# scipopt/SCIP-SDP

Measured on AMD Instinct MI355X. Metric: node-SDP solves/sec, dense block n x n with m vars (IPM iters/sec in iters_per_sec), higher is better.
Workload: dtype f64

## Files before the change

### include/hipsdp_units.h

```cpp
#ifndef HIPSDP_UNITS_H
#define HIPSDP_UNITS_H

#include "hipsdp.h"

#ifdef __cplusplus
extern "C" {
#endif

HIPSDP_API int  hipsdp_dgemm_selfcheck(int device, int M, int N, int K, int layB, int batch, int splitk, int flags, double beta,
   int* used_v2, long long* ndiff);
HIPSDP_API int  hipsdp_pass_at_unit(int device, int R, long long E, const double* A, const double* coef, double sa, const double* add, int split,
   double* out, int* chunks);
HIPSDP_API int  hipsdp_dgemm_selfcheck2(int device, int M, int N, int K, int layB, int batch, int splitk, int flags, double alpha, double beta,
   int reps, int* used, long long* ndiff, double* ms_tile, double* ms_fast);
HIPSDP_API int  hipsdp_gram_plan_info(int device, int M, long long K, int nslab, int* no, int* nd, int* nitems, double* span);
HIPSDP_API int  hipsdp_gram_selfcheck(int device, int M, long long K, int reps, int* used, double* maxdiff, long long* nrepro, double* ms_tile,
   double* ms_gram);
HIPSDP_API int  hipsdp_dgemm_selfcheck3(int device, int M, int N, int K, int layB, int batch, int splitk, int flags, double alpha, double beta,
   int reps, int* used, long long* ndiff, double* maxdiff, long long* nrepro, double* ms_tile, double* ms_fast);
HIPSDP_API int  hipsdp_tri_product_unit(int device, int mode, int M, int N, int K, int layB, int batch, int flags, const double* A,
   const double* B, double* Cio, int crows, int ldc, int* used);
HIPSDP_API int  hipsdp_tri_instance_force(int mode);
HIPSDP_API int  hipsdp_schur_identity_unit(int device, int m1, int n, const double* A, double ws_gbytes, int full_storage, double* Mx,
   double* flops);
HIPSDP_API int  hipsdp_schur_dense(int device, int m1, int n, const double* A, const double* X, const double* Zinv, double* Mx,
   double ws_gbytes);
HIPSDP_API int  hipsdp_schur_w(int device, int m1, int n, const double* A, const double* X, const double* Z, double* Mx);
HIPSDP_API int  hipsdp_schur_form_unit(int device, int form, int parts, int m1, int n, const double* A, const double* P, const double* Q,
   double ws_gbytes, double* Mx, int* used);
HIPSDP_API int  hipsdp_schur_small_unit(int device, int m1, int nblk, const int* ns, const double* const* A, const double* const* X,
   const double* const* Zinv, int q, const double* Dext, const double* x, const double* z, double* Mx, double* Lm, double* diagM, int* taken);
HIPSDP_API int  hipsdp_schur_shard_time(int device, int m1, int n, int nranks, int rank, int by_columns, int reps, double ws_gbytes, double* ms);
HIPSDP_API int  hipsdp_schur_var_share_time(int device, int m1, int n, int nranks, int rank, int cw, int reps, double* ms, double* a2a_bytes);
HIPSDP_API int  hipsdp_schur_sparse_unit(int device, int n, int m, long long nnz, const int* var, const int* row, const int* col,
   const double* val, const double* X, const double* Zinv, double* Mx);
HIPSDP_API int  hipsdp_schur_sparse_unit2(int device, int n, int m, long long nnz, const int* var, const int* row, const int* col,
   const double* val, const double* X, const double* Zinv, double* Mx, int kernel, int* took);
HIPSDP_API int  hipsdp_sparse_ops_unit(int device, int n, int m, long long nnz, const int* var, const int* row, const int* col,
   const double* val, const double* V, const double* coef, const double* base, double* outA, double* outAT);
HIPSDP_API int  hipsdp_mfma_peak(int device, double ms, double* tflops, double* ghz);
HIPSDP_API int  hipsdp_potrf(int device, int n, double* A, int* fail);
HIPSDP_API int  hipsdp_potrf_ex(int device, int n, double* A, int psd, int v1, double* dinv, int* regmask, int* fail);
HIPSDP_API int  hipsdp_potrs(int device, int n, const double* A, int nrhs, double* rhs);
HIPSDP_API int  hipsdp_potrs_seq(int device, int n, const double* A, int psd, int ncalls, const int* nrhs, const int* mode, double* rhs,
   int* regmask, int* fail);
HIPSDP_API int  hipsdp_potrf_small_unit(int device, int n, int pair, const double* base, const double* dir, double alpha, int set_flag,
   int want_gram, double* L, double* dinv, double* Mout, double* Linv, double* Gram, int* flag);
HIPSDP_API long long hipsdp_potrf_dinv_len(int n);
HIPSDP_API int  hipsdp_potrf_pair_unit(int device, int n, int pair, double* A, double* dinv, int* fail);
HIPSDP_API int  hipsdp_trial_pair_unit(int device, int n, int fused, int first, double alpha, double* io);
HIPSDP_API int  hipsdp_tail_after_solve2_unit(int device, int m, int fused, const double* rhs2, const double* u1, double* u2, double* wt,
   double* e2, double* e1);
HIPSDP_API int  hipsdp_tail_unpack3_unit(int device, int n, int fused, const double* pk, double* out);
HIPSDP_API int  hipsdp_tail_dz_unit(int device, int n, int fused, const double* pk, const double* P2, const double* Rd, double dtau, double eta,
   double* dZ);
HIPSDP_API int  hipsdp_tail_dirmat_unit(int device, int n, int fused, double s1, const double* Zinv, const double* X, const double* GZ, double* H,
   double* pk);
HIPSDP_API int  hipsdp_tail_sc_len(void);
HIPSDP_API int  hipsdp_tail_dir_unit(int device, int m, int n, int fused, const double* B, const double* H, const double* rhs2, const double* rp,
   const double* b, const double* u1, const double* u2, const double* par, double* sc, double* dy, double* dyt);
HIPSDP_API int  hipsdp_tail_dots_unit(int device, int m, int n, int fused, const double* a, const double* v, double* out);
HIPSDP_API int  hipsdp_trtri(int device, int n, const double* A, double* Linv);
HIPSDP_API int  hipsdp_lambda_min(int device, int n, const double* W, int steps, double* theta, double* resid);
HIPSDP_API int  hipsdp_lambda_min_scaled(int device, int n, const double* L, const double* D, int steps, double* theta, double* resid);
HIPSDP_API int  hipsdp_solve1_fits(int m, int q, int nblk, const int* ns);
HIPSDP_API int  hipsdp_solve1_class(int m, int nblk, const int* ns);
HIPSDP_API unsigned long long hipsdp_gram_gen_next(unsigned long long* counter);
HIPSDP_API int  hipsdp_gram_key_match_unit(int m_a, int nblk_a, const int* n_a, const int* form_a, const unsigned long long* gen_a,
   const long long* ws_a, int m_b, int nblk_b, const int* n_b, const int* form_b, const unsigned long long* gen_b, const long long* ws_b);
HIPSDP_API int  hipsdp_syev_many_unit(int device, int count, const int* ns, const double* A, double* lam, double* V, int* launches);
HIPSDP_API int  hipsdp_sparsecuts_unit(int device, int count, const int* ns, const double* Z, const double* v0, const double* maxeig,
   const int* sizes, const hipsdp_sparsecut_opts* opts, int* ncuts, double* eigvals, double* vecs, int* iters, int* flags);
HIPSDP_API int  hipsdp_sparsecuts_large_unit(int device, int n, const double* Z, const double* v0, double maxeig, int size,
   const hipsdp_sparsecut_opts* opts, int* ncuts, double* eigvals, double* vecs, int* iters, int* flags);
HIPSDP_API int  hipsdp_tridiag_unit(int device, int n, const double* A, double* d, double* e, double* Vrefl, double* tau);
HIPSDP_API int  hipsdp_tvec_unit(int device, int n, const double* d, const double* e, double* lam, double* Z);
HIPSDP_API int  hipsdp_sparse_dump_unit(hipsdp_solver* solver, int block, long long* counts, int* voff, int* vrow, int* vcol, double* vval,
   int* poff, int* prow, int* pcol, int* pvar, double* pval, int* foff, int* frow, int* fcol, double* fval, int* soff, int* srow, int* sent);
HIPSDP_API int  hipsdp_onevar_unit(int device, int n, int count, const double* Z, const double* A, const double* shift, const int* kind,
   const double* lb, const double* ub, double feastol, int maxevals, int* status, double* optval, double* lmin, double* grad, int* evals);
HIPSDP_API int  hipsdp_onevar_all_unit(int device, int count, const int* n, const double* Z, const double* A, const double* shift,
   const int* kind, const double* lb, const double* ub, double feastol, int maxevals, int mid_cap,
   int* status, double* optval, double* lmin, double* grad, int* evals);
HIPSDP_API int  hipsdp_onevar_large_unit(int device, int count, const int* n, const double* Z, const double* A, const double* shift,
   const int* kind, const double* lb, const double* ub, double feastol, int maxevals, int wg_cap, int chunk,
   int* status, double* optval, double* lmin, double* grad, int* evals, int* rounds);
HIPSDP_API int  hipsdp_objs_fanout_unit(int device, int count, int m, int q, int nblk, const int* ns, const double* B, const double* b_own,
   int have_start, const double* y, const double* x, const double* z, const double* XZ, int gap, double guard, long long* lane_len,
   long long* offs, double* lanes, int* launches);
HIPSDP_API int  hipsdp_small_dir_block_unit(int device, int n, double c, double s1, const double* X, const double* R, const double* E,
   const double* Zinv, int recorded, double* out, int* pending);
HIPSDP_API int  hipsdp_small_lp_rows_unit(int device, int q, int m1, const double* Dext, const double* v, int mode, double eta, double sigmu,
   const double* x, const double* z, const double* rd, const double* elp, int recorded, double* out1, double* out2, int* pending);
HIPSDP_API int  hipsdp_small_apply_A_unit(int device, int m1, int nblk, const int* n2, const double* A, const double* V, int q,
   const double* Dext, const double* vlp, int epi, double scal, const double* vin, int recorded, double* out, double* vout, int* pending);
HIPSDP_API int  hipsdp_small_elementwise_unit(int device, int n, const int* nn, const double* par, int use_elp, const double* in,
   const double* xs, int recorded, double* o_lp, double* o_mul, double* o_ext, double* ys, int* pending);
HIPSDP_API int  hipsdp_small_gemv_t_unit(int device, int R, long long E, long long lda, const double* A, const double* coef, double sa,
   int add_mode, const double* add, int recorded, double* out, int* pending);
HIPSDP_API int  hipsdp_reductions_unit(int device, int kind, int count, const int* len, const int* slot, const int* accumulate,
   const double* a, const double* b, const double* c, int nslots, const double* preset, int recorded, double* out, int* pending);
HIPSDP_API int  hipsdp_small_solve_unit(int device, int m, const double* M, int form, int nrhs, long long ld, double* rhs, double* u2,
   double* wt, int* pending, int* fail);
HIPSDP_API int  hipsdp_gemv_t3_unit(int device, int R, long long E, long long lda, const double* A, const double* c, int fused, double* out,
   int* took);
// ... 9 lines not shown
```

### scip-sdp_amd/binding.py

```python
import ctypes as C
import os
import numpy as np

_HERE = os.path.dirname(os.path.abspath(__file__))
LIBPATH = os.environ.get("HIPSDP_LIB", os.path.join(_HERE, "lib", "libhipsdp.so"))

STATUS_NAMES = {0: "optimal", 1: "dual_infeasible", 2: "dual_unbounded", 3: "both_infeasible", 4: "iterlimit",
                5: "numeric", 6: "timelimit", 7: "objlimit", -1: "unsolved"}


class Params(C.Structure):
    _fields_ = [("gaptol", C.c_double), ("feastol", C.c_double), ("infeastol", C.c_double), ("objlimit", C.c_double),
                ("timelimit", C.c_double), ("gamma", C.c_double), ("ws_gbytes", C.c_double), ("maxiter", C.c_int),
                ("verbose", C.c_int), ("lanczos_steps", C.c_int), ("settings", C.c_int), ("pabstol", C.c_double), ("preoptgap", C.c_double)]


class Info(C.Structure):
    _fields_ = [("status", C.c_int), ("iterations", C.c_int), ("pobj", C.c_double), ("dobj", C.c_double),
                ("pinf", C.c_double), ("dinf", C.c_double), ("dabs", C.c_double), ("gap", C.c_double), ("mu", C.c_double),
                ("tau", C.c_double), ("kappa", C.c_double), ("solve_seconds", C.c_double), ("schur_seconds", C.c_double),
                ("schur_flops", C.c_double), ("schur_calls", C.c_int), ("chol_fail", C.c_int), ("warm_started", C.c_int),
                ("settings_used", C.c_int), ("schur_flops_executed", C.c_double)]


# ... 866 lines not shown
    A = _f64(A)
    m1, n = A.shape[0], A.shape[1]
    P = _f64(P); Q = _f64(Q)
    assert A.shape == (m1, n, n) and P.shape == (n, n) and Q.shape == (n, n)
    Mx = np.zeros((m1, m1))
    used = (C.c_int * 3)(0, 0, 0)
    _chk(ulib().hipsdp_schur_form_unit(device, form, parts, m1, n, _dp(A), _dp(P), _dp(Q), C.c_double(ws_gbytes), _dp(Mx), used),
         "hipsdp_schur_form_unit")
    return Mx, tuple(used)


def schur_small_unit(As, Xs, Zinvs, Dext=None, x=None, z=None, fill=0.0, device=0):
    As = [_f64(a) for a in As]; Xs = [_f64(a) for a in Xs]; Zinvs = [_f64(a) for a in Zinvs]
    nblk, m1 = len(As), As[0].shape[0]
    ns = np.array([a.shape[1] for a in As], dtype=np.int32)
    for k in range(nblk):
        assert As[k].shape == (m1, ns[k], ns[k]) and Xs[k].shape == (ns[k], ns[k]) and Zinvs[k].shape == (ns[k], ns[k])
    q = 0 if Dext is None else int(np.shape(Dext)[0])
    if q > 0:
        Dext = _f64(Dext); x = _f64(x); z = _f64(z)
        assert Dext.shape == (q, m1) and x.shape == (q,) and z.shape == (q,)
    arr = C.POINTER(C.c_double) * nblk
    pA, pX, pZ = arr(*[_dp(a) for a in As]), arr(*[_dp(a) for a in Xs]), arr(*[_dp(a) for a in Zinvs])
    m = m1 - 1
    Mx = np.full((m1, m1), fill)
    Lm = np.full(max(m * m, 1), fill)
    dg = np.full(max(m, 1), fill)
    taken = C.c_int(-1)
    _chk(ulib().hipsdp_schur_small_unit(device, m1, nblk, _ip(ns), pA, pX, pZ, q, _dp(Dext) if q else None, _dp(x) if q else None,
                                        _dp(z) if q else None, _dp(Mx), _dp(Lm), _dp(dg), C.byref(taken)), "hipsdp_schur_small_unit")
    return taken.value, Mx, Lm[:m * m].reshape(m, m), dg[:m]


def gram_plan_info(M, K, nslab=64, device=0):
    no, nd, ni = C.c_int(0), C.c_int(0), C.c_int(0)
    sp = C.c_double(0.0)
    rc = ulib().hipsdp_gram_plan_info(device, M, C.c_longlong(K), nslab, C.byref(no), C.byref(nd), C.byref(ni), C.byref(sp))
    return (no.value, nd.value, ni.value, sp.value) if rc == 0 else None


def dgemm_selfcheck(M, N, K, layB=1, batch=1, splitk=1, flags=0, beta=0.0, device=0):
    used = C.c_int(0)
    nd = C.c_longlong(0)
    _chk(ulib().hipsdp_dgemm_selfcheck(device, M, N, K, layB, batch, splitk, flags, C.c_double(beta), C.byref(used), C.byref(nd)),
         "hipsdp_dgemm_selfcheck")
    return used.value, nd.value


def dgemm_selfcheck2(M, N, K, layB=1, batch=1, splitk=1, flags=0, alpha=1.0, beta=0.0, reps=0, device=0):
    used = C.c_int(0)
    nd = C.c_longlong(0)
    t0, t1 = C.c_double(0.0), C.c_double(0.0)
    _chk(ulib().hipsdp_dgemm_selfcheck2(device, M, N, K, layB, batch, splitk, flags, C.c_double(alpha), C.c_double(beta), reps,
                                       C.byref(used), C.byref(nd), C.byref(t0), C.byref(t1)), "hipsdp_dgemm_selfcheck2")
    return used.value, nd.value, t0.value, t1.value


def dgemm_selfcheck3(M, N, K, layB=1, batch=1, splitk=1, flags=0, alpha=1.0, beta=0.0, reps=0, device=0):
    used = C.c_int(0)
    nd, nr = C.c_longlong(0), C.c_longlong(0)
    md, t0, t1 = C.c_double(0.0), C.c_double(0.0), C.c_double(0.0)
    _chk(ulib().hipsdp_dgemm_selfcheck3(device, M, N, K, layB, batch, splitk, flags, C.c_double(alpha), C.c_double(beta), reps,
                                       C.byref(used), C.byref(nd), C.byref(md), C.byref(nr), C.byref(t0), C.byref(t1)), "hipsdp_dgemm_selfcheck3")
    return used.value, nd.value, md.value, nr.value, t0.value, t1.value


def tri_product_unit(A, B, flags, mode, layB=1, sentinel=None, pad_rows=0, pad_cols=0, device=0):
    A = _f64(A); B = _f64(B)
    M, K = A.shape
    batch = B.shape[0]
    N = B.shape[2] if layB == 1 else B.shape[1]
    assert B.shape == ((batch, K, N) if layB == 1 else (batch, N, K))
    Cio = np.full((batch, M + pad_rows, N + pad_cols), np.nan if sentinel is None else sentinel)
    used = (C.c_int * 2)(0, 0)
    _chk(ulib().hipsdp_tri_product_unit(device, mode, M, N, K, layB, batch, flags, _dp(A), _dp(B), _dp(Cio), M + pad_rows, N + pad_cols, used),
         "hipsdp_tri_product_unit")
    return Cio, tuple(used)


def tri_instance_force(mode):
    return ulib().hipsdp_tri_instance_force(mode)


def gram_selfcheck(M, K, reps=0, device=0):
    used = C.c_int(0)
    nr = C.c_longlong(0)
    md, t0, t1 = C.c_double(0.0), C.c_double(0.0), C.c_double(0.0)
    _chk(ulib().hipsdp_gram_selfcheck(device, M, C.c_longlong(K), reps, C.byref(used), C.byref(md), C.byref(nr), C.byref(t0), C.byref(t1)),
         "hipsdp_gram_selfcheck")
    return used.value, md.value, nr.value, t0.value, t1.value


def schur_identity_unit(A, Mx=None, ws_gbytes=0.0, full_storage=False, device=0):
    A = _f64(A)
    m1, n = A.shape[0], A.shape[1]
    Mx = np.zeros((m1, m1)) if Mx is None else _f64(Mx).copy()
    fl = C.c_double(0.0)
    _chk(ulib().hipsdp_schur_identity_unit(device, m1, n, _dp(A), C.c_double(ws_gbytes), int(full_storage), _dp(Mx), C.byref(fl)),
         "hipsdp_schur_identity_unit")
    return Mx, fl.value


def potrf(A, device=0):
    L = _f64(A).copy()
    fail = C.c_int(0)
    _chk(ulib().hipsdp_potrf(device, L.shape[0], _dp(L), C.byref(fail)), "hipsdp_potrf")
    return np.tril(L), fail.value


def potrf_ex(A, psd=False, v1=False, device=0):
    L = _f64(A).copy()
    n = L.shape[0]
    dinv = np.zeros(((n + 63) // 64) * 4096)
    mask = np.zeros(n, dtype=np.int32)
    fail = C.c_int(0)
    _chk(ulib().hipsdp_potrf_ex(device, n, _dp(L), int(psd), int(v1), _dp(dinv), _ip(mask), C.byref(fail)), "hipsdp_potrf_ex")
    return L, dinv, mask, fail.value


def potrs(A, rhs, device=0):
    A = _f64(A)
    r = _f64(rhs).copy()
    r2 = r.reshape(-1, A.shape[0])
    _chk(ulib().hipsdp_potrs(device, A.shape[0], _dp(A), r2.shape[0], _dp(r2)), "hipsdp_potrs")
    return r2.reshape(r.shape)


def potrs_seq(A, calls, psd=False, device=0):
    A = _f64(A)
    n = A.shape[0]
    nc = len(calls)
    slab = np.zeros((max(nc, 1), 4, n))
    nrhs = np.zeros(max(nc, 1), dtype=np.int32)
    mode = np.zeros(max(nc, 1), dtype=np.int32)
    for c, (md, r) in enumerate(calls):
        r = _f64(r).reshape(-1, n)
        nrhs[c], mode[c] = r.shape[0], md
        slab[c, :min(r.shape[0], 4)] = r[:4]
    mask = np.zeros(n, dtype=np.int32)
    fail = C.c_int(0)
    _chk(ulib().hipsdp_potrs_seq(device, n, _dp(A), int(psd), nc, _ip(nrhs), _ip(mode), _dp(slab), _ip(mask), C.byref(fail)),
         "hipsdp_potrs_seq")
    return [slab[c, :nrhs[c]].copy() for c in range(nc)], mask, fail.value


def potrf_small_unit(base, dir=None, alpha=0.0, pair=False, set_flag=False, want_gram=False, device=0):
    base = _f64(base)
    n = base.shape[-1]
    npb = 2 if pair else 1
    assert base.size == npb * n * n
    d = None if dir is None else _f64(dir)
    assert d is None or d.size == base.size
    shp = (2, n, n) if pair else (n, n)
    out = {"L": np.zeros(shp), "dinv": np.zeros((2, 64, 64) if pair else (64, 64)), "Mout": np.zeros(shp), "Linv": np.zeros(shp),
           "Gram": np.zeros(shp) if want_gram else None}
    flag = np.zeros(2, dtype=np.int32)
    _chk(ulib().hipsdp_potrf_small_unit(device, n, int(pair), _dp(base), None if d is None else _dp(d), C.c_double(alpha), int(set_flag),
                                        int(want_gram), _dp(out["L"]), _dp(out["dinv"]), _dp(out["Mout"]), _dp(out["Linv"]),
                                        None if not want_gram else _dp(out["Gram"]), _ip(flag)), "hipsdp_potrf_small_unit")
    out["flag"] = flag.copy() if pair else int(flag[0])
    return out


def potrf_pair_unit(A2, pair=True, device=0):
    L = _f64(A2).copy()
    n = L.shape[-1]
# ... 337 lines not shown
```

### scip-sdp_amd/csrc/hs_kernels.h

```cpp
#ifndef HS_KERNELS_H
#define HS_KERNELS_H

#include "hs_common.h"
#include "hs_cut_plan.h"
#include <vector>

int hs_fill(hipStream_t s, double* p, long long n, double v);
int hs_set_identity(hipStream_t s, double* A, int n, double v);
int hs_copy(hipStream_t s, double* dst, const double* src, long long n);
int hs_axpy(hipStream_t s, long long n, double a, const double* x, double* y);
int hs_scale_add(hipStream_t s, long long n, double a, const double* x, double b, const double* y, double* out);
struct hs_trial_job { double* V; const double* dV; double* Vs; double* L; };
int hs_trial_pair(hipStream_t s, long long n, double alpha, int first, const hs_trial_job* jobs);
int hs_mirror_lower(hipStream_t s, double* A, int n, long long lda);
int hs_symmetrize(hipStream_t s, double* A, int n);
int hs_transpose(hipStream_t s, int n, const double* src, double* dst);

int hs_gemv_n(hipStream_t s, int R, long long E, const double* A, long long lda, int nv, const double* const* V,
   double* out, long long ldo, double* ws, long long wsdoubles);
int hs_gemv_t(hipStream_t s, int R, long long E, const double* A, long long lda, const double* coef, double sa,
   const double* add, double* out);

int hs_gemv_t_chunks(int R, long long E);
int hs_gemv_t_ws(hipStream_t s, int R, long long E, const double* A, long long lda, const double* coef, double sa,
   const double* add, double* out, double* ws, long long wsdoubles);
int hs_gemv_t3(hipStream_t s, int R, long long E, const double* A, long long lda, const double* c0, const double* c1, const double* c2,
   double* o0, double* o1, double* o2);

void hs_red_batch_begin(hipStream_t s);
int hs_red_batch_end(void);
int hs_red_batch_end_publish(hipStream_t s, int n, const double* src, double* dst, unsigned long long seq, unsigned long long* flag);
void hs_red_batch_reset(void);
int hs_fill_scalar(hipStream_t s, double* p, double v);
int hs_red_batch_solve(hipStream_t s, int m, const double* dinv, const double* L, int nrhs, double* vec, long long ld);
struct hs_rb_finish { int m; double eta, rg, sigmu, tau, kappa, etk; const double* u1; const double* u2; double* dy; double* dyt; double* sc;
   int s0, bub, bh, wrp, bu1, dtau, dkappa, den; };
int hs_red_batch_finish(hipStream_t s, const void* fin, size_t bytes);
int hs_copy_scalar(hipStream_t s, double* dst, const double* src);
void hs_red_batch_hold(hipStream_t s);
int hs_red_batch_release(void);
int hs_red_batch_flush(void);
int hs_red_batch_pending(void);
int hs_red_batch_end_all(void);
int hs_make_ext(hipStream_t s, int m, double s0, double s1, const double* v, double* ext);
int hs_lp_rows_small(hipStream_t s, int q, int m1, const double* Dext, const double* v, int mode, double eta, double sigmu, const double* x,
   const double* z, const double* rd, const double* elp, double* out1, double* out2);
#define HS_AS_MAXBLK 8
struct hs_as_args { int nblk; int n2[HS_AS_MAXBLK]; const double* A[HS_AS_MAXBLK]; const double* V[HS_AS_MAXBLK]; };
int hs_apply_A_small(hipStream_t s, int m1, const hs_as_args* B, int q, const double* Dext, const double* vlp, double* out, int epi,
   double scal, const double* vin, double* vout);
int hs_axpy3(hipStream_t s, double a, long long n1, const double* x1, double* y1, long long n2, const double* x2, double* y2,
   long long n3, const double* x3, double* y3);
int hs_dot(hipStream_t s, long long n, const double* a, const double* b, double* out, int accumulate, double* ws);
#define HS_DOT_SLOT_DOUBLES 256
#define HS_DOT_SLOTS 4
#define HS_RED_WS_DOUBLES (HS_DOT_SLOTS * HS_DOT_SLOT_DOUBLES)
int hs_dot_deferred(hipStream_t s, long long n, const double* a, const double* b, double* out, int accumulate, double* ws, int slot);
int hs_absmax(hipStream_t s, long long n, const double* a, double* out, int accumulate, double* ws);
int hs_ratio_min(hipStream_t s, long long n, const double* x, const double* d, double* out, int accumulate, double* ws);

#define HS_SMALL_N 48
int hs_dir_block_small(hipStream_t s, int n, double c, const double* X, const double* R, const double* E, const double* Zinv,
   double s1, double* out);
int hs_dirmat(hipStream_t s, int n, double s1, const double* Zinv, const double* X, const double* GZ, double* H);
int hs_dirmat_pack(hipStream_t s, int n, double s1, const double* Zinv, const double* X, const double* GZ, double* H, double* pk);

int hs_lp_dir(hipStream_t s, int q, double sigmu, double eta, const double* x, const double* z, const double* rd_or_dz,
   const double* elp, double* out);
int hs_lp_scale_rows(hipStream_t s, int q, int cols, const double* x, const double* z, const double* D, double* S);
int hs_vec_mul(hipStream_t s, long long n, const double* a, const double* b, double* out);
int hs_lp_s0(hipStream_t s, int q, const double* x, const double* z, const double* beta, double* out, int accumulate, double* ws);

int hs_pack_rows(hipStream_t s, int m1, int n, long long Lp, const double* A, double* Apk);
int hs_packed_diag(hipStream_t s, int m1, int n, int ldd, long long Lp, const double* Apk, double* D);
int hs_sub_lower(hipStream_t s, int n, const double* S, double* C);
int hs_pack_weighted(hipStream_t s, int n, const double* V, double* pk);
int hs_unpack_sym(hipStream_t s, int n, const double* pk, double sa, const double* add, double* out);
int hs_unpack_sym3(hipStream_t s, int n, int cnt, const double* const* pk, double* const* out);
int hs_unpack_dz_combine(hipStream_t s, int n, const double* pk, const double* P2, const double* sc, int idtau, double eta, const double* Rd,
   double* dZ);
int hs_zero_upper(hipStream_t s, double* A, int n);

struct hs_schur_ws
{
   double*   T;
   double*   U;
   double*   K;
   double*   V;
   long long capT, capV;
   long long chunk_cols;
   long long n2;
   long long kws_len;
   int       full;
   double*   U2;
   double*   V2;
   void*     evP[2];
   void*     evX[2];
   void*     ev_g2;
   int       (*after_g1)(void*);
   void*     after_g1_arg;
};
int  hs_schur_ws_alloc(hs_schur_ws* w, int m1, long long n2max, double budget_gb);
void hs_schur_ws_free(hs_schur_ws* w);
int  hs_schur_U(hipStream_t s, int m1, int n, const double* A, const double* X, const double* Zinv, double* Mx,
   hs_schur_ws* w, int j_begin, int j_end);
int  hs_schur_W(hipStream_t s, int m1, int n, const double* A, const double* R, const double* G, double* Mx, hs_schur_ws* w);
int  hs_schur_W_identity(hipStream_t s, int m1, int n, const double* A, double* Mx, hs_schur_ws* w);
int  hs_schur_W_identity_range(hipStream_t s, int m1, int n, const double* A, long long k0, long long k1, double* Mx, hs_schur_ws* w);
int  hs_schur_W_identity_packed(hipStream_t s, int m1, int n, const double* Apk, long long Lp, double* Mx, hs_schur_ws* w);
int  hs_schur_identity_packed_fits(const hs_schur_ws* w, int m1, int n);

int  hs_schur_Urows(hipStream_t s, int m1, int n, const double* A, const double* X, const double* Zinv, double* Mx,
   hs_schur_ws* w, int r_begin, int r_end);
void hs_shard_rows(int m1, int nranks, int rank, int* chunk_rows, int* first_begin, int* second_begin);
int  hs_schur_Wcols(hipStream_t s, int m1, int n, const double* A, const double* R, const double* G, double* Mx, hs_schur_ws* w,
   int c0, int cw);
void hs_shard_cols(int m1, int n, int nranks, int rank, int* c_begin, int* c_width);
int  hs_schur_Wvar(hipStream_t s, void* comm, int rank, int nranks, int m1, int n, const double* A, const double* R, const double* G,
   double* Mx, hs_schur_ws* w, int c0, int cw);
int  hs_schur_ws_alloc_var(hs_schur_ws* w, int m1, int nranks, int n, int cwmax);
int  hs_schur_ws_alloc_var_overlap(hs_schur_ws* w);
int  hs_schur_Wvar_all(hipStream_t s, hipStream_t sc, void* comm, int rank, int nranks, int m1, int n, const double* A, const double* R,
   const double* G, double* Mx, hs_schur_ws* w, int cwmax, int overlap);
void hs_var_rows(int m1, int nranks, int rank, int* r0, int* r1);
void hs_var_wrows(int n, int nranks, int rank, int* q0, int* q1);
int  hs_alltoall(void* comm, const double* send, double* recv, const long long* cnt, hipStream_t stream);
int  hs_allreduce_sum(void* comm, double* buf, long long count, hipStream_t stream);
int  hs_mirror_upper(hipStream_t s, double* A, int n, long long lda);
int  hs_allgather_inplace(void* comm, double* buf, long long count_per_rank, int rank, hipStream_t stream);
int  hs_allgather(void* comm, const double* send, double* recv, long long count_per_rank, hipStream_t stream);

struct hs_sparse
{
   int        n, m;
   long long  nnz;
   int*       voff;
   int*       vrow;
   int*       vcol;
   double*    vval;
   long long  npos;
   int*       poff;
   int*       prow;
   int*       pcol;
   int*       pvar;
   double*    pval;
   long long  nfull, nslots;
   int*       foff;
   int*       frow;
   int*       fcol;
   double*    fval;
   int*       soff;
   int*       srow;
   int*       sent;
   double*    Tc;
   int        borrowed;
};
int  hs_sp_prefers_sparse(int n, int m, long long nnz);
int  hs_sp_build(hs_sparse** out, int n, int m, long long nnz, const int* var, const int* row, const int* col, const double* val);
void hs_sp_free(hs_sparse* sp);
long long hs_sp_nnz(const hs_sparse* sp);
int  hs_sp_apply_A(hipStream_t s, const hs_sparse* sp, const double* V, double* out_var1);
int  hs_sp_apply_AT(hipStream_t s, const hs_sparse* sp, const double* coef, double* out);
int  hs_sp_schur(hipStream_t s, const hs_sparse* sp, const double* X, const double* Zinv, double* Mx);
int  hs_sp_schur_ex(hipStream_t s, const hs_sparse* sp, const double* X, const double* Zinv, double* Mx, int kernel, int* took);
int  hs_sp_expand(hipStream_t s, const hs_sparse* sp, double* A);

struct hs_spm;
int  hs_spm_create(hs_spm** out, int N, int S);
void hs_spm_free(hs_spm* M);
int  hs_spm_size(const hs_spm* M);
int  hs_spm_slots(const hs_spm* M);
int  hs_spm_add(hs_spm* M, long long nnz, const int* slot, int oneslot, const int* row, const int* col, const double* val);
int  hs_spm_gather_sparse(hipStream_t s, hs_spm* M, int n, int m, int nactive, const int* act, const int* kept, hs_sparse** out,
   long long* launches, long long* readbacks);
int  hs_spm_gather_dense(hipStream_t s, hs_spm* M, int n, int nactive, const int* dact, const int* dinv, double* A, long long* launches);
struct hipsdp_solver;
int  hs_solver_sparse_block(struct hipsdp_solver* s, int block, const hs_sparse** sp);

struct hs_dir_tail_args { int m, q, K; const int* n; const double* const* B; const double* const* H; const double* beta; const double* hl;
   const double* rhs2; const double* rp; const double* b; double* u1; const double* u2; double* dy; double* dyt; double* sc; double* red_ws;
   const double* dinvm; const double* Lm; double eta, rg, sigmu, tau, kappa, etk; };
int hs_ipm_dir_tail(hipStream_t st, const hs_dir_tail_args* a, int tail, int fuse_solve);
int hs_ipm_after_solve2(hipStream_t st, int m, const double* rhs2, double* u2, double* wt, const double* u1, double* e2, double* e1, int fused);
int hs_ipm_dz_combine(hipStream_t st, long long n2, double* dZ, const double* P2, const double* sc, double eta, const double* Rd);
int hs_ipm_sc_dtau(void);
int hs_ipm_sc_len(int nblocks);

int hs_potrf(hipStream_t s, int n, double* A, double* dinv, int* flag, const double* diag0);
long long hs_potrf_dinv_len(int n);
int hs_potrf_psd(hipStream_t s, int n, double* A, double* dinv, int* flag, const double* diag0, int* regmask, int set_flag);
struct hs_potrf_job { double* A; double* dinv; int* flag; };
int hs_potrf_pair(hipStream_t s, int n, const hs_potrf_job* jobs);
int hs_trtri(hipStream_t s, int n, const double* L, const double* dinv, double* Linv, double* tmp);
int hs_potrf_small_ext_pair(hipStream_t s, int n, double* const* L, double* const* dinv, int* const* flag, const double* const* base,
   const double* const* dir, double alpha, double* const* Mout, double* const* Linv, double* const* Gram, int set_flag);
int hs_potrf_small_ext(hipStream_t s, int n, double* L, double* dinv, int* flag, const double* base, const double* dir, double alpha,
   double* Mout, double* Linv, double* Gram, int set_flag);
int hs_schur_small(hipStream_t s, int m1, int nblk, const int* n, const double* const* A, const double* const* X,
   const double* const* Zinv, int q, const double* Dext, const double* x, const double* z, double* Mx, double* Lm, double* diagM);
int hs_trsv(hipStream_t s, int n, const double* L, const double* dinv, int nrhs, double* rhs, long long ldr, int mode);
long long hs_trsv_sync_ws(int n);
int hs_trsv_sync_init(hipStream_t s, int n, int* sync_ws, int* epoch);
int hs_trsv_sync(hipStream_t s, int n, const double* L, const double* dinv, int nrhs, double* rhs, long long ldr, int mode,
   int* sync_ws, int* epoch);

int hs_lanczos_lmin(hipStream_t s, int n, const double* W, int maxsteps, double* res, double* ws);
long long hs_lanczos_ws(int n, int maxsteps);
#define HS_STEP_MAXJOBS 32
struct hs_step_jobs { int nblk; int n[HS_STEP_MAXJOBS]; const double* L0[HS_STEP_MAXJOBS]; const double* D0[HS_STEP_MAXJOBS];
   const double* L1[HS_STEP_MAXJOBS]; const double* D1[HS_STEP_MAXJOBS]; double* res0[HS_STEP_MAXJOBS]; double* res1[HS_STEP_MAXJOBS]; };
int hs_steplen_small_multi(hipStream_t s, const hs_step_jobs* P, int maxsteps);
int hs_lmin_exact_multi(hipStream_t st, const hs_step_jobs* P);
int hs_lanczos_scaled_small(hipStream_t s, int n, int maxsteps, const double* L0, const double* D0, const double* L1, const double* D1,
   double* res0, double* res1);
int hs_lmin_scaled_tiny(hipStream_t s, int n, const double* L0, const double* D0, const double* L1, const double* D1, double* res0,
   double* res1);
int hs_lanczos_lmin2(hipStream_t s, int n, const double* W0, const double* W1, int maxsteps, double* res0, double* res1,
   double* ws0, double* ws1, int* rot, unsigned long long* dsync, int nwipe);
long long hs_lanczos_sync_words(void);
int hs_lanczos_sync_reset(hipStream_t s, unsigned long long* dsync, int* rot);

long long hs_syev_small_scratch(int n);
int hs_syev_small_dev(hipStream_t st, int n, const double* A, double* lam, double* V, double* scratch);
struct hs_eig_job { int n; int pad; const double* in; double* ws; };
long long hs_syev_many_vecpos(int n);
int hs_syev_many_class(int n);
int hs_syev_small_many(hipStream_t st, int count, const hs_eig_job* hjobs, const hs_eig_job* jobs, int* launches);

int hs_psd_project_one(int device, int n, int nnz, const int* row, const int* col, const double* val, double minev,
   double epsilon, int mode, int cap, int* nnz_out, int* rowout, int* colout, double* valout);

#define HS_EC_DENSE  0
#define HS_EC_PACKED 1
#define HS_EC_SPARSE 2
struct hs_sp_view { long long nnz, npos; const int *voff, *vrow, *vcol; const double* vval; const int *poff, *prow, *pcol, *pvar; const double* pval; };
void hs_sp_get_view(const hs_sparse* sp, hs_sp_view* v);
struct hs_ec_job
{
   int n, form, blk, pad;
   long long ld;
   const double* A;
   hs_sp_view sp;
   double* Z;
   double* ws;
   long long vpos;
   long long vecoff;
};
int hs_ec_form_z(hipStream_t st, int count, int nmax, int m, const hs_ec_job* jobs, const double* y);
int hs_ec_cuts(hipStream_t st, int count, int nmax, int m, int nb, int maxcuts, double tol, const hs_ec_job* jobs, double* res);

#define HS_OV_MAXN 128
#define HS_OV_TAB 5
#define HS_OV_RES 6
struct hs_ov_par
{
   int n, count, maxevals, pad;
   double feastol, infinity;
   const hs_ec_job* blk;
   const double* Z; const double* A;
   const double* tab;
   double* slab;
   double* res;
};
long long hs_onevar_slab(int n, int count);
int hs_onevar_newton(hipStream_t st, const hs_ov_par* P);
// ... 441 lines not shown
```

### scip-sdp_amd/csrc/ipm.hip

```cpp
#include "hs_kernels.h"
#include "hs_gram_cache.h"
#include "hs_sp_master.h"
#include "../../include/hipsdp.h"
#include <rocprofiler-sdk-roctx/roctx.h>
#include <vector>
#include <atomic>
#include <utility>
#include <functional>
#include <chrono>
#include <algorithm>
#include <cmath>
#include <cassert>
#include <cstdio>
#include <cstdlib>
#include <cstring>

enum
{
   SC_AX0 = 0,
   SC_DOBJ,
   SC_XZ,
   SC_RP2,
   SC_RD2,
   SC_RDLPMAX,
   SC_HP2,
   SC_HD2,
   SC_S0,
   SC_BUB,
   SC_BH,
   SC_WRP,
   SC_BU1,
   SC_DTAU,
   SC_DKAPPA,
   SC_RATX,
   SC_RATZ,
   SC_DEN,
   SC_FIXED_END = 24
};
#define SC_BLK(k, i) (SC_FIXED_END + 8 * (k) + (i))

struct Block
{
   int     n;
   double* A;
   double* Aown;
   double* A0;
   double* A0sep;
   double* Apkown;
   double *X, *Z, *Rd, *Lz, *LzInv, *Zinv, *Lx, *LxInv, *B, *H, *G, *GZ, *dXa, *dZa, *dX, *dZ, *E, *W, *T1;
   double *dinvz, *dinvx;
   double *Xs, *Zs;
   double *T2, *W2;
   double *Xpre;
   double *P2;
   double *pk3;
   double *Apk;
   double *pkv;
   long long Lp;
   bool apk_valid;
   unsigned long long A_gen;
   bool a_escaped;
   bool derived_valid;
   bool sparse;
   bool sp_dirty;
   hs_sparse* sp;
   struct SpHost* sph;
   bool sp_gathered;
   int sp_master;
};

struct SpHost
{
   std::vector<int> var, row, col;
   std::vector<double> val;
};

enum { PH_RESID = 0, PH_FACTOR, PH_SCHUR, PH_MSOLVE, PH_PRED, PH_CORR, PH_UPDATE, PH_COUNT };
static const char* const g_phase_names[PH_COUNT] = {"residuals", "factorizations", "schur", "chol_M_solves", "predictor", "corrector",
   "update"};

struct PhaseClock
{
   bool on;
   int open;
   std::vector<hipEvent_t> pool;
   std::vector<std::pair<int, hipEvent_t> > marks;
   double ms[PH_COUNT];
};

struct CutWs
{
   double* dev = NULL; long long dev_len = 0;
   double* pin = NULL; long long pin_len = 0;
   char* tab = NULL; long long tab_len = 0;
   std::vector<hs_ec_job> jobs; std::vector<hs_eig_job> ejobs;

   static int regrow(void** p, long long* len, long long need, size_t unit, bool pinned)
   {
      if ( need <= *len )
         return HS_OK;
      if ( *p != NULL ) HS_HIP( pinned ? hipHostFree(*p) : hipFree(*p) );
      *p = NULL; *len = 0;
      HS_HIP( pinned ? hipHostMalloc(p, (size_t) need * unit, hipHostMallocDefault) : hipMalloc(p, (size_t) need * unit) );
      *len = need;
      return HS_OK;
   }
   int grow(long long dev_need, long long pin_need, size_t tab_bytes)
   {
      HS_CALL( regrow((void**) &dev, &dev_len, dev_need, sizeof(double), false) );
      HS_CALL( regrow((void**) &pin, &pin_len, pin_need, sizeof(double), true) );
      if ( (long long) tab_bytes > tab_len ) { jobs.clear(); ejobs.clear(); }
      return regrow((void**) &tab, &tab_len, (long long) tab_bytes, 1, false);
   }
   int upload(const std::vector<hs_ec_job>& j, const std::vector<hs_eig_job>& je)
   {
      if ( jobs.size() == j.size() && memcmp(jobs.data(), j.data(), j.size() * sizeof(hs_ec_job)) == 0 )
         return HS_OK;
      HS_HIP( hipMemcpy(tab, j.data(), j.size() * sizeof(hs_ec_job), hipMemcpyHostToDevice) );
      if ( !je.empty() )
         HS_HIP( hipMemcpy(tab + j.size() * sizeof(hs_ec_job), je.data(), je.size() * sizeof(hs_eig_job), hipMemcpyHostToDevice) );
      jobs = j; ejobs = je;
// ... 1369 lines not shown
         return HIPSDP_ERR_ARG;
   for (int r = 0; r < nkept; ++r)
      if ( kept[r] < 0 || kept[r] >= N )
         return HIPSDP_ERR_ARG;
   Block& B = s->blk[engine_block];
   a_written(s, B);
   long long g = ((long long) nactive * nkept * nkept + 255) / 256; if ( g > 65536 ) g = 65536;
   {
      void* dv = NULL;
      int* hidx = (int*) stage_take(s, (size_t) (nactive + nkept) * sizeof(int), &dv);
      if ( hidx != NULL )
      {
         memcpy(hidx, activevars, (size_t) nactive * sizeof(int));
         memcpy(hidx + nactive, kept, (size_t) nkept * sizeof(int));
         const int* didx = (const int*) dv;
         NodeCmd* q = ((long long) nactive * nkept * nkept <= NC_LIMIT) ? cmd_new(s) : NULL;
         if ( q != NULL )
         {
            q->op = NC_GATHER; q->i0 = nactive; q->i1 = nkept; q->i2 = N; q->idx = didx; q->src = s->master_A[master_block]; q->dst = B.A;
         }
         else
         {
            HS_CALL( flush_cmds(s) );
            hipLaunchKernelGGL(k_master_gather, dim3((unsigned) g), dim3(256), 0, s->stream, nactive, nkept, N, didx, didx + nactive,
               s->master_A[master_block], B.A);
            HS_LAUNCH_CHECK();
            s->stage_pending = true;
         }
      }
      else
      {
         int *dact, *dkept;
         HS_CALL( flush_cmds(s) );
         HS_CALL( dalloc(&dact, nactive) ); HS_CALL( dalloc(&dkept, nkept) );
         HS_HIP( hipMemcpyAsync(dact, activevars, (size_t) nactive * sizeof(int), hipMemcpyHostToDevice, s->stream) );
         HS_HIP( hipMemcpyAsync(dkept, kept, (size_t) nkept * sizeof(int), hipMemcpyHostToDevice, s->stream) );
         hipLaunchKernelGGL(k_master_gather, dim3((unsigned) g), dim3(256), 0, s->stream, nactive, nkept, N, dact, dkept,
            s->master_A[master_block], B.A);
         HS_LAUNCH_CHECK();
         HS_HIP( hipStreamSynchronize(s->stream) );
         dfree(dact); dfree(dkept);
      }
   }
   s->solved = false;
   return HIPSDP_OK;
}

extern "C" int hipsdp_set_block_dense(hipsdp_solver* s, int block, const double* A)
{
   if ( s == NULL || !s->shaped || block < 0 || block >= (int) s->blk.size() )
      return HIPSDP_ERR_ARG;
   HS_HIP( hipSetDevice(s->device) );
   HS_CALL( stage_sync(s) );
   Block& B = s->blk[block];
   if ( B.sparse )
   {
      set_err("hipsdp_set_block_dense: the block is kept as nonzeros (hipsdp_set_shape2 with a count): use hipsdp_add_entries");
      return HIPSDP_ERR_ARG;
   }
   const size_t n2b = (size_t) B.n * B.n * sizeof(double);
   a_written(s, B);
   if ( s->a_r1 > s->a_r0 )
      HS_HIP( hipMemcpy(B.Aown, A + (size_t) s->a_r0 * B.n * B.n, (size_t) (s->a_r1 - s->a_r0) * n2b, hipMemcpyHostToDevice) );
   if ( B.A0sep != NULL )
      HS_HIP( hipMemcpy(B.A0sep, A, n2b, hipMemcpyHostToDevice) );
   s->solved = false;
   return HIPSDP_OK;
}

extern "C" int hipsdp_set_lp(hipsdp_solver* s, const double* Dext)
{
   if ( s == NULL || !s->shaped ) return HIPSDP_ERR_ARG;
   HS_HIP( hipSetDevice(s->device) );
   if ( s->q > 0 )
      HS_CALL( stage_upload(s, s->Dext, Dext, (size_t) s->q * (s->m + 1) * sizeof(double)) );
   s->zero_D = false;
   s->solved = false;
   return HIPSDP_OK;
}

int hs_gen_dense(hipStream_t s, int n, int i0, int i1, long long seed, double* A);
static int ensure_packed(hipsdp_solver* s);
static int pass_A(hipsdp_solver* s, Block& B, const double* V, double* out, bool packed = false);
static int pass_AT(hipsdp_solver* s, Block& B, const double* coef, double sa, const double* add, double* out);

extern "C" int hipsdp_gen_planted(hipsdp_solver* s, int n, int m, long long seed, const double* Xstar, const double* Zstar,
   const double* ystar, double* b_out)
{
   if ( s == NULL || !s->shaped || s->blk.size() != 1 || s->blk[0].n != n || s->m != m || s->q != 0 || s->blk[0].sparse )
      return HIPSDP_ERR_ARG;
   HS_HIP( hipSetDevice(s->device) );
   HS_CALL( stage_sync(s) );
   Block& B = s->blk[0];
   const long long n2 = (long long) n * n;
   const int m1 = m + 1;
   hipStream_t st = s->stream;
   a_written(s, B);
   HS_CALL( hs_gen_dense(st, n, s->a_r0 > 1 ? s->a_r0 : 1, s->a_r1, seed, B.A) );
   HS_HIP( hipMemcpyAsync(B.Z, Zstar, (size_t) n2 * sizeof(double), hipMemcpyHostToDevice, st) );
   HS_HIP( hipMemcpyAsync(B.X, Xstar, (size_t) n2 * sizeof(double), hipMemcpyHostToDevice, st) );
   HS_HIP( hipMemsetAsync(s->yt, 0, sizeof(double), st) );
   HS_HIP( hipMemcpyAsync(s->yt + 1, ystar, (size_t) m * sizeof(double), hipMemcpyHostToDevice, st) );
   HS_HIP( hipMemsetAsync(B.A0, 0, (size_t) n2 * sizeof(double), st) );
   if ( s->shardA )
   {
      a_written(s, B);
      HS_CALL( ensure_packed(s) );
      HS_CALL( pass_AT(s, B, s->yt, -1.0, B.Z, B.T1) );
      HS_CALL( hs_symmetrize(st, B.T1, n) );
      HS_CALL( hs_copy(st, B.A0, B.T1, n2) );
      HS_CALL( pass_A(s, B, B.X, s->AX) );
   }
   else
   {
   HS_CALL( hs_gemv_t(st, m1, n2, B.A, n2, s->yt, -1.0, B.Z, B.T1) );
   HS_CALL( hs_symmetrize(st, B.T1, n) );
   HS_CALL( hs_copy(st, B.A, B.T1, n2) );
   const double* v = B.X;
   HS_CALL( hs_gemv_n(st, m1, n2, B.A, n2, 1, &v, s->AX, m1, s->gemv_ws, s->gemv_ws_len) );
   }
   HS_CALL( hs_copy(st, s->b, s->AX + 1, m) );
   HS_HIP( hipMemcpyAsync(b_out, s->b, (size_t) m * sizeof(double), hipMemcpyDeviceToHost, st) );
   HS_HIP( hipStreamSynchronize(st) );
   a_written(s, B);
   s->solved = false;
   return HIPSDP_OK;
}

void hs_gen_set_density(double density);

extern "C" int hipsdp_gen_planted_density(hipsdp_solver* s, int n, int m, long long seed, double density, const double* Xstar,
   const double* Zstar, const double* ystar, double* b_out)
{
   hs_gen_set_density(density);
   const int rc = hipsdp_gen_planted(s, n, m, seed, Xstar, Zstar, ystar, b_out);
   hs_gen_set_density(1.0);
   return rc;
}

extern "C" int hipsdp_get_block_dense(hipsdp_solver* s, int block, double* A)
{
   if ( s == NULL || !s->shaped || block < 0 || block >= (int) s->blk.size() )
      return HIPSDP_ERR_ARG;
   HS_HIP( hipSetDevice(s->device) );
   HS_CALL( stage_sync(s) );
   Block& B = s->blk[block];
   if ( B.sparse )
   {
      const size_t n2 = (size_t) B.n * B.n;
      memset(A, 0, (size_t) (s->m + 1) * n2 * sizeof(double));
      HS_HIP( hipMemcpy(A, B.A0, n2 * sizeof(double), hipMemcpyDeviceToHost) );
      if ( B.sp_gathered )
      {
         if ( B.sp == NULL )
            return HIPSDP_ERR_ARG;
         HS_HIP( hipStreamSynchronize(s->stream) );
         const size_t nz = (size_t) B.sp->nnz;
         std::vector<int> voff((size_t) s->m + 1), vrow(nz + 1), vcol(nz + 1);
         std::vector<double> vval(nz + 1);
         HS_HIP( hipMemcpy(voff.data(), B.sp->voff, voff.size() * sizeof(int), hipMemcpyDeviceToHost) );
         if ( nz > 0 )
         {
            HS_HIP( hipMemcpy(vrow.data(), B.sp->vrow, nz * sizeof(int), hipMemcpyDeviceToHost) );
            HS_HIP( hipMemcpy(vcol.data(), B.sp->vcol, nz * sizeof(int), hipMemcpyDeviceToHost) );
            HS_HIP( hipMemcpy(vval.data(), B.sp->vval, nz * sizeof(double), hipMemcpyDeviceToHost) );
         }
         for (int v = 1; v <= s->m; ++v)
// ... 135 lines not shown
      r[k][i] = x;
      __syncthreads();
      if ( i < m )
         rhs2[k * m + i] = x;
      if ( k == 0 )
      {
         if ( i == 0 )
            wt[0] = 1.0;
         if ( i < m )
         {
            u2[i] = r[1][i] - r[0][i];
            wt[1 + i] = -r[0][i];
         }
      }
      return;
   }
   __syncthreads();
   double acc = 0.0;
   if ( i < m )
      for (int j = 0; j <= i; ++j)
         acc += dinv[i * 64 + j] * r[k][j];
   t[k][i] = acc;
   __syncthreads();
   double res = 0.0;
   if ( i < m )
   {
      for (int j = 0; j <= i; ++j)
         res += L[(long long) i * m + j] * t[k][j];
      res = r[k][i] - res;
   }
   c[k][i] = res;
   __syncthreads();
   double cor = 0.0;
   if ( i < m )
      for (int j = 0; j <= i; ++j)
         cor += dinv[i * 64 + j] * c[k][j];
   __syncthreads();
   t[k][i] = acc + cor;
   __syncthreads();
   acc = 0.0;
   if ( i < m )
      for (int j = i; j < m; ++j)
         acc += dinv[j * 64 + i] * t[k][j];
   r[k][i] = acc;
   __syncthreads();
   res = 0.0;
   if ( i < m )
   {
      for (int j = i; j < m; ++j)
         res += L[(long long) j * m + i] * r[k][j];
      res = t[k][i] - res;
   }
   c[k][i] = res;
   __syncthreads();
   cor = 0.0;
   if ( i < m )
      for (int j = i; j < m; ++j)
         cor += dinv[j * 64 + i] * c[k][j];
   __syncthreads();
   r[k][i] = acc + cor;
   __syncthreads();
   if ( i < m )
      rhs2[k * m + i] = r[k][i];
   if ( k == 0 )
   {
      if ( i == 0 )
         wt[0] = 1.0;
      if ( i < m )
      {
         u2[i] = r[1][i] - r[0][i];
         wt[1 + i] = -r[0][i];
      }
   }
}

int hs_solve2_small(hipStream_t st, int m, const double* Mx, const double* b, const double* dinv, const double* L, double* rhs2, double* u2,
   double* wt, int subst)
{
   hipLaunchKernelGGL(k_solve2_small, dim3(1), dim3(128), 0, st, m, Mx, b, dinv, L, rhs2, u2, wt, subst);
   HS_LAUNCH_CHECK();
   return HS_OK;
}

__global__ void k_h(int m, double eta, const double* __restrict__ AH, const double* __restrict__ rp, double* __restrict__ h)
{
   const int i = blockIdx.x * blockDim.x + threadIdx.x;
   if ( i < m )
      h[i] = AH[1 + i] - eta * rp[i];
}

__global__ void k_finish_dir(int m, double eta, double rg, double sigmu, double tau, double kappa, double etk,
   const double* __restrict__ u1, const double* __restrict__ u2, double* __restrict__ dy, double* __restrict__ dyt,
   double* __restrict__ sc)
{
   const double den = sc[SC_S0] + kappa / tau + sc[SC_BUB];
   const double num = -eta * rg + (sigmu - tau * kappa - etk) / tau - sc[SC_BH] - eta * sc[SC_WRP] + sc[SC_BU1];
   const double dtau = num / den;
   const int i = blockIdx.x * blockDim.x + threadIdx.x;
   if ( i == 0 )
   {
      sc[SC_DTAU] = dtau;
      sc[SC_DKAPPA] = (sigmu - tau * kappa - etk - kappa * dtau) / tau;
      sc[SC_DEN] = den;
      dyt[0] = -dtau;
   }
   if ( i < m )
   {
      const double v = u1[i] - u2[i] * dtau;
      dy[i] = v;
      dyt[1 + i] = v;
   }
}

__global__ void k_dz_combine(long long n2, double* __restrict__ dZ, const double* __restrict__ P2, const double* __restrict__ sc, double eta,
   const double* __restrict__ Rd)
{
   const double dtau = sc[SC_DTAU];
   for (long long i = (long long) blockIdx.x * blockDim.x + threadIdx.x; i < n2; i += (long long) gridDim.x * blockDim.x)
      dZ[i] = (dZ[i] - dtau * P2[i]) + eta * Rd[i];
}

__global__ void k_cert(long long n2, double tau, const double* __restrict__ Rd, const double* __restrict__ A0, double* __restrict__ out)
{
   for (long long i = (long long) blockIdx.x * blockDim.x + threadIdx.x; i < n2; i += (long long) gridDim.x * blockDim.x)
      out[i] = Rd[i] + tau * A0[i];
}

static inline dim3 g1d(long long n) { long long g = (n + 255) / 256; if ( g < 1 ) g = 1; if ( g > 4096 ) g = 4096; return dim3((unsigned) g); }

int hs_ipm_dir_tail(hipStream_t st, const hs_dir_tail_args* a, int tail, int fuse_solve)
{
   const int m = a->m;
   hs_red_batch_begin(st);
   if ( fuse_solve )
      (void) hs_red_batch_solve(st, m, a->dinvm, a->Lm, 1, a->u1, m);
   HS_CALL( hs_fill_scalar(st, a->sc + SC_BH, 0.0) );
   for (int k = 0; k < a->K; ++k)
   {
      const long long n2 = (long long) a->n[k] * a->n[k];
      if ( tail )
         HS_CALL( hs_dot_deferred(st, n2, a->B[k], a->H[k], a->sc + SC_BH, 1, a->red_ws, k) );
      else
         HS_CALL( hs_dot(st, n2, a->B[k], a->H[k], a->sc + SC_BH, 1, a->red_ws) );
   }
   if ( a->q > 0 )
      HS_CALL( hs_dot(st, a->q, a->beta, a->hl, a->sc + SC_BH, 1, a->red_ws) );
   HS_CALL( hs_dot(st, m, a->rhs2, a->rp, a->sc + SC_WRP, 0, a->red_ws) );
   HS_CALL( hs_dot(st, m, a->b, a->u1, a->sc + SC_BU1, 0, a->red_ws) );
   bool finished = false;
   if ( fuse_solve || tail )
   {
      hs_rb_finish F = {m, a->eta, a->rg, a->sigmu, a->tau, a->kappa, a->etk, a->u1, a->u2, a->dy, a->dyt, a->sc,
         SC_S0, SC_BUB, SC_BH, SC_WRP, SC_BU1, SC_DTAU, SC_DKAPPA, SC_DEN};
      finished = hs_red_batch_finish(st, &F, sizeof(F)) == 1;
   }
   HS_CALL( hs_red_batch_end() );
   if ( !finished )
   {
      HS_CALL( hs_red_batch_flush() );
      hipLaunchKernelGGL(k_finish_dir, g1d(m > 0 ? m : 1), dim3(256), 0, st, m, a->eta, a->rg, a->sigmu, a->tau, a->kappa, a->etk,
         a->u1, a->u2, a->dy, a->dyt, a->sc);
      HS_LAUNCH_CHECK();
   }
   return HS_OK;
}

int hs_ipm_after_solve2(hipStream_t st, int m, const double* rhs2, double* u2, double* wt, const double* u1, double* e2, double* e1, int fused)
{
   if ( fused && e2 != NULL )
   {
      hipLaunchKernelGGL(k_after_solve2_ext, g1d(m + 1), dim3(256), 0, st, m, rhs2, u2, wt, 1.0, 1.0, e2, 0.0, 1.0, u1, e1);
      HS_LAUNCH_CHECK();
      return HS_OK;
   }
   hipLaunchKernelGGL(k_after_solve2, g1d(m + 1), dim3(256), 0, st, m, rhs2, u2, wt);
   HS_LAUNCH_CHECK();
   if ( e2 != NULL )
   {
      HS_CALL( hs_make_ext(st, m, 1.0, 1.0, u2, e2) );
      HS_CALL( hs_make_ext(st, m, 0.0, 1.0, u1, e1) );
   }
   return HS_OK;
}

int hs_ipm_dz_combine(hipStream_t st, long long n2, double* dZ, const double* P2, const double* sc, double eta, const double* Rd)
{
   HS_CALL( hs_red_batch_flush() );
   hipLaunchKernelGGL(k_dz_combine, g1d(n2), dim3(256), 0, st, n2, dZ, P2, sc, eta, Rd);
   HS_LAUNCH_CHECK();
   return HS_OK;
}

int hs_ipm_sc_dtau(void) { return SC_DTAU; }
int hs_ipm_sc_len(int nblocks) { return SC_FIXED_END + 8 * (nblocks > 0 ? nblocks : 1) + 8; }

static int gemm_on(hipStream_t st, int layA, int layB, int M, int N, int K, double alpha, const double* A, long long lda,
   const double* B, long long ldb, double beta, double* C, long long ldc, int flags = 0)
{
   (void) hs_red_batch_flush();
   hs_gemm_args g = {M, N, K, layA, layB, A, lda, 0, B, ldb, 0, C, ldc, 0, alpha, beta, 1, flags, 1, NULL};
   return hs_dgemm(st, &g);
}

static int gemm(hipsdp_solver* s, int layA, int layB, int M, int N, int K, double alpha, const double* A, long long lda,
   const double* B, long long ldb, double beta, double* C, long long ldc, int flags = 0)
{
   return gemm_on(s->stream, layA, layB, M, N, K, alpha, A, lda, B, ldb, beta, C, ldc, flags);
}

static int fork2(hipsdp_solver* s)
{
   if ( !s->use2 )
      return HS_OK;
   s->busy2 = true;
   HS_HIP( hipEventRecord(s->evFork, s->stream) );
   HS_HIP( hipStreamWaitEvent(s->stream2, s->evFork, 0) );
   return HS_OK;
}

static int join2(hipsdp_solver* s)
{
   if ( !s->use2 )
      return HS_OK;
   s->busy2 = false;
   HS_HIP( hipEventRecord(s->evJoin, s->stream2) );
   HS_HIP( hipStreamWaitEvent(s->stream, s->evJoin, 0) );
   return HS_OK;
}

static int ensure_schur_ws(hipsdp_solver* s)
{
   if ( s->sws.T != NULL )
      return HS_OK;
   {
      bool anydense = false;
      for (auto& B : s->blk) anydense = anydense || !B.sparse;
      if ( !anydense && !s->blk.empty() )
         return HS_OK;
   }
   const int m1 = s->m + 1;
   long long n2max = 1;
   for (auto& B : s->blk) { const long long n2 = (long long) B.n * B.n; if ( !B.sparse && n2 > n2max ) n2max = n2; }
   double budget = s->par.ws_gbytes > 0.0 ? s->par.ws_gbytes : 40.0;
   const char* env = getenv("HIPSDP_WS_GB");
   if ( env != NULL && atof(env) > 0.0 )
      budget = atof(env);
   else if ( s->par.ws_gbytes <= 0.0 && s->comm == NULL )
   {
      size_t fr = 0, tot = 0;
      if ( hipMemGetInfo(&fr, &tot) == hipSuccess && 0.75e-9 * (double) fr > budget )
         budget = 0.75e-9 * (double) fr;
   }
   const char* mode = getenv("HIPSDP_SCHUR");
   s->schur_mode_cols = false;
   s->schur_sim_shards = 0;
   if ( s->shardA )
   {
      int nmaxb = 1;
      for (auto& B : s->blk) if ( B.n > nmaxb ) nmaxb = B.n;
      static const bool var_overlap = !(getenv("HIPSDP_VAR_OVERLAP") != NULL && getenv("HIPSDP_VAR_OVERLAP")[0] == '0');
      const double per_col = (var_overlap ? 5.0 : 3.0) * 8.0 * (double) ((m1 + s->nranks - 1) / s->nranks + 1) * (double) nmaxb;
      long long cw = (long long) (budget * 1e9 / per_col);
      const char* ecw = getenv("HIPSDP_VAR_SLICE");
      if ( ecw != NULL && atoi(ecw) > 0 )
         cw = atoi(ecw);
      else if ( cw < nmaxb )
         cw = cw / 128 * 128 > 0 ? cw / 128 * 128 : 128;
      if ( cw > nmaxb ) cw = nmaxb;
      s->var_cw = (int) cw;
      HS_CALL( hs_schur_ws_alloc_var(&s->sws, m1, s->nranks, nmaxb, (int) cw) );
      s->var_overlap = false;
      if ( var_overlap && cw < nmaxb )
         s->var_overlap = (hs_schur_ws_alloc_var_overlap(&s->sws) == HS_OK);
      s->schur_mode_U = false; s->schur_mode_rows = false; s->schur_mode_forced = true;
      return HS_OK;
   }
// ... 209 lines not shown
   HS_HIP( hipStreamSynchronize(s->stream) );
   *sp = s->blk[block].sp;
   return HS_OK;
}

__global__ void k_sp_base(long long n2, const double* __restrict__ c, const double* __restrict__ A0, double sa, const double* __restrict__ add,
   double* __restrict__ out)
{
   const double c0 = c[0];
   for (long long e = (long long) blockIdx.x * blockDim.x + threadIdx.x; e < n2; e += (long long) gridDim.x * blockDim.x)
      out[e] = c0 * A0[e] + (add != NULL ? sa * add[e] : 0.0);
}

__global__ void __launch_bounds__(1024) k_sp_dot0(long long n, const double* __restrict__ a, const double* __restrict__ b, double* __restrict__ out)
{
   __shared__ double part[16];
   double acc = 0.0;
   for (long long e = threadIdx.x; e < n; e += 1024)
      acc += a[e] * b[e];
#pragma unroll
   for (int off = 32; off > 0; off >>= 1)
      acc += __shfl_xor(acc, off, 64);
   if ( (threadIdx.x & 63) == 0 )
      part[threadIdx.x >> 6] = acc;
   __syncthreads();
   if ( threadIdx.x == 0 )
   {
      double t = 0.0;
      for (int w = 0; w < 16; ++w)
         t += part[w];
      out[0] = t;
   }
}

__global__ void k_add_col0(int m1, const double* __restrict__ v, double* __restrict__ Mx)
{
   for (int i = blockIdx.x * blockDim.x + threadIdx.x; i < m1; i += gridDim.x * blockDim.x)
      Mx[(long long) i * m1] += v[i];
}

static int pass_A(hipsdp_solver* s, Block& B, const double* V, double* out, bool packed)
{
   const int m1 = s->m + 1;
   if ( B.sparse )
   {
      HS_CALL( hs_gemv_n(s->stream, 1, (long long) B.n * B.n, B.A0, (long long) B.n * B.n, 1, &V, out, 1, s->gemv_ws, s->gemv_ws_len) );
      return hs_sp_apply_A(s->stream, B.sp, V, out + 1);
   }
   if ( passes_sharded(s, B) )
   {
      int c, r0, r1;
      pass_rows(s, &c, &r0, &r1);
      if ( s->passg == NULL )
         HS_CALL( dalloc(&s->passg, (long long) c * s->nranks) );
      double* mine = s->passg + (long long) s->rank * c;
      if ( B.Apk != NULL )
      {
         HS_CALL( hs_pack_weighted(s->stream, B.n, V, B.pkv) );
         const double* v = B.pkv;
         if ( r1 > r0 )
            HS_CALL( hs_gemv_n(s->stream, r1 - r0, B.Lp, B.Apk + (long long) r0 * B.Lp, B.Lp, 1, &v, mine, r1 - r0, s->gemv_ws, s->gemv_ws_len) );
      }
      else if ( r1 > r0 )
      {
         const long long n2 = (long long) B.n * B.n;
         HS_CALL( hs_gemv_n(s->stream, r1 - r0, n2, B.A + (long long) r0 * n2, n2, 1, &V, mine, r1 - r0, s->gemv_ws, s->gemv_ws_len) );
      }
      hs_comm_phase(1);
      const int rcg = hs_allgather_inplace(s->comm, s->passg, c, s->rank, s->stream);
      hs_comm_phase(2);
      HS_CALL( rcg );
      return hs_copy(s->stream, out, s->passg, m1);
   }
   if ( B.Apk != NULL )
   {
      if ( !packed )
         HS_CALL( hs_pack_weighted(s->stream, B.n, V, B.pkv) );
      const double* v = B.pkv;
      return hs_gemv_n(s->stream, m1, B.Lp, B.Apk, B.Lp, 1, &v, out, m1, s->gemv_ws, s->gemv_ws_len);
   }
   return hs_gemv_n(s->stream, m1, (long long) B.n * B.n, B.A, (long long) B.n * B.n, 1, &V, out, m1, s->gemv_ws, s->gemv_ws_len);
}

static int pass_AT(hipsdp_solver* s, Block& B, const double* coef, double sa, const double* add, double* out)
{
   const int m1 = s->m + 1;
   const long long n2 = (long long) B.n * B.n;
   if ( B.sparse )
   {
      hipLaunchKernelGGL(k_sp_base, g1d(n2), dim3(256), 0, s->stream, n2, coef, B.A0, sa, add, out);
      HS_LAUNCH_CHECK();
      return hs_sp_apply_AT(s->stream, B.sp, coef, out);
   }
   if ( passes_sharded(s, B) )
   {
      int c, r0, r1;
      pass_rows(s, &c, &r0, &r1);
      if ( B.Apk != NULL )
      {
         HS_CALL( hs_gemv_t(s->stream, r1 - r0, B.Lp, B.Apk + (long long) r0 * B.Lp, B.Lp, coef + r0, 0.0, NULL, B.pkv + B.Lp) );
         hs_comm_phase(1);
         const int rcr = hs_allreduce_sum(s->comm, B.pkv + B.Lp, B.Lp, s->stream);
         hs_comm_phase(2);
         HS_CALL( rcr );
         return hs_unpack_sym(s->stream, B.n, B.pkv + B.Lp, sa, add, out);
      }
      HS_CALL( hs_gemv_t(s->stream, r1 - r0, n2, B.A + (long long) r0 * n2, n2, coef + r0, s->rank == 0 ? sa : 0.0,
            s->rank == 0 ? add : NULL, out) );
      hs_comm_phase(1);
      const int rcr = hs_allreduce_sum(s->comm, out, n2, s->stream);
      hs_comm_phase(2);
      return rcr;
   }
   if ( B.Apk != NULL )
   {
      HS_CALL( hs_gemv_t_ws(s->stream, m1, B.Lp, B.Apk, B.Lp, coef, 0.0, NULL, B.pkv + B.Lp, s->gemvt_ws, s->gemvt_ws_len) );
      return hs_unpack_sym(s->stream, B.n, B.pkv + B.Lp, sa, add, out);
   }
   return hs_gemv_t_ws(s->stream, m1, n2, B.A, n2, coef, sa, add, out, s->gemvt_ws, s->gemvt_ws_len);
}

#define AS_MAXBLK HS_AS_MAXBLK

static bool small_problem(const hipsdp_solver* s)
{
   if ( s->blk.size() > AS_MAXBLK || s->q > 4096 || s->m + 1 > 4096 || s->shardA )
      return false;
   long long tot = 0;
   for (auto& B : s->blk)
   {
      if ( B.Apk != NULL || B.sparse || B.A == NULL )
         return false;
      tot += (long long) B.n * B.n;
   }
   return tot <= 8192;
}

static bool batch_regions(const hipsdp_solver* s)
{
   static int on = -1;
   if ( on < 0 )
   {
      const char* env = getenv("HIPSDP_BATCH");
      on = (env != NULL && env[0] == '0') ? 0 : 1;
   }
   return on != 0 && s->comm == NULL && small_problem(s);
}

struct BatchRegion
{
   bool on;
   BatchRegion(hipsdp_solver* s, bool want) : on(want) { if ( on ) hs_red_batch_hold(s->stream); }
   int close() { if ( !on ) return HS_OK; on = false; return hs_red_batch_release(); }
   ~BatchRegion() { if ( on ) (void) hs_red_batch_release(); }
};

static bool general_tail(const hipsdp_solver* s)
{
   if ( s->comm != NULL || s->m <= 64 || s->blk.empty() || batch_regions(s) )
      return false;
   for (auto& B : s->blk)
      if ( B.n <= 64 )
         return false;
   return true;
}

static bool pack_with_dirmat(const hipsdp_solver* s, const Block& B)
{
   return general_tail(s) && B.Apk != NULL && !B.sparse;
}

static int apply_A_small(hipsdp_solver* s, double* const* Vk, const double* vlp, double* out, int epi, double scal,
   const double* vin, double* vout)
{
   if ( !small_problem(s) )
      return 0;
   for (auto& Bk : s->blk)
      if ( Bk.A == NULL )
         return 0;
   hs_as_args B;
   B.nblk = (int) s->blk.size();
   for (int k = 0; k < AS_MAXBLK; ++k)
   {
      B.n2[k] = 0; B.A[k] = NULL; B.V[k] = NULL;
   }
   for (size_t k = 0; k < s->blk.size(); ++k)
   {
      B.n2[k] = s->blk[k].n * s->blk[k].n;
      B.A[k] = s->blk[k].A;
      B.V[k] = Vk[k];
   }
   const int rc = hs_apply_A_small(s->stream, s->m + 1, &B, s->q, s->Dext, vlp, out, epi, scal, vin, vout);
   if ( rc != HS_OK )
      return -rc;
   return 1;
}

static int apply_A(hipsdp_solver* s, double* const* Vk, const double* vlp, double* out, bool packed = false)
{
   const int m1 = s->m + 1;
   bool first = true;
   for (size_t k = 0; k < s->blk.size(); ++k)
   {
      Block& B = s->blk[k];
      const double* v = Vk[k];
      double* dst = first ? out : s->tmpe;
      HS_CALL( pass_A(s, B, v, dst, packed && pack_with_dirmat(s, B)) );
      if ( !first )
         HS_CALL( hs_axpy(s->stream, m1, 1.0, s->tmpe, out) );
      first = false;
   }
   if ( first )
      HS_CALL( hs_fill(s->stream, out, m1, 0.0) );
   if ( s->q > 0 )
      HS_CALL( hs_gemv_t(s->stream, s->q, m1, s->Dext, m1, vlp, 1.0, out, out) );
   return HS_OK;
}

struct QueueSwap
{
   hipsdp_solver* s;
   explicit QueueSwap(hipsdp_solver* s_) : s(s_) { std::swap(s->stream, s->stream2); }
   ~QueueSwap() { std::swap(s->stream, s->stream2); }
};

static const int SOLVE_MODE = 3 | 4;

static int direction(hipsdp_solver* s, double sigma, double eta, double mu, double rg, bool useE, double etk, int part = 0,
   bool u1_solved = false, int split = 0)
{
   const int m = s->m, m1 = s->m + 1, q = s->q;
   const double sigmu = sigma * mu;
   std::vector<double*> Hs;
   int fusedA = 0;
   BatchRegion region(s, part == 0 && batch_regions(s));
   if ( part != 2 )
   {
   for (auto& B : s->blk)
   {
      const int n = B.n;
      const long long n2 = (long long) n * n;
      if ( n <= HS_SMALL_N )
         HS_CALL( hs_dir_block_small(s->stream, n, eta, B.X, B.Rd, useE ? B.E : NULL, B.Zinv, sigmu, B.H) );
      else
      {
         if ( useE )
            HS_CALL( hs_copy(s->stream, B.G, B.E, n2) );
         HS_CALL( gemm(s, HS_KC, HS_MC, n, n, n, eta, B.X, n, B.Rd, n, useE ? 1.0 : 0.0, B.G, n) );
         HS_CALL( gemm(s, HS_KC, HS_MC, n, n, n, 1.0, B.G, n, B.Zinv, n, 0.0, B.GZ, n) );
         if ( pack_with_dirmat(s, B) )
            HS_CALL( hs_dirmat_pack(s->stream, n, sigmu, B.Zinv, B.X, B.GZ, B.H, B.pkv) );
         else
            HS_CALL( hs_dirmat(s->stream, n, sigmu, B.Zinv, B.X, B.GZ, B.H) );
      }
      Hs.push_back(B.H);
   }
   if ( q > 0 )
      HS_CALL( hs_lp_dir(s->stream, q, sigmu, eta, s->x, s->z, s->rd, useE ? s->elp : NULL, s->hl) );
   fusedA = part == 1 ? 0 : apply_A_small(s, Hs.data(), s->hl, s->AH, 1, eta, s->rp, s->u1);
   if ( fusedA < 0 )
      return -fusedA;
   if ( fusedA == 0 )
      HS_CALL( apply_A(s, Hs.data(), s->hl, s->AH, true) );
   if ( fusedA == 0 && m > 0 )
   {
      HS_CALL( hs_red_batch_flush() );
      hipLaunchKernelGGL(k_h, g1d(m), dim3(256), 0, s->stream, m, eta, s->AH, s->rp, s->u1);
      HS_LAUNCH_CHECK();
   }
   if ( part == 1 )
      return HS_OK;
   }
   const bool fuse_solve = (fusedA == 1) && m > 0 && m <= 64;
   if ( m > 0 && !fuse_solve && !u1_solved )
   {
      HS_CALL( hs_red_batch_flush() );
      HS_CALL( hs_trsv_sync(s->stream, m, s->Lm, s->dinvm, 1, s->u1, m, SOLVE_MODE, s->trsv_ws, &s->trsv_epoch) );
   }
   {
      std::vector<int> bn;
      std::vector<const double*> bB, bH;
      for (auto& B : s->blk)
      {
         bn.push_back(B.n); bB.push_back(B.B); bH.push_back(B.H);
      }
      const hs_dir_tail_args ta = {m, q, (int) s->blk.size(), bn.data(), bB.data(), bH.data(), s->beta, s->hl, s->rhs2, s->rp, s->b, s->u1, s->u2,
         s->dy, s->dyt, s->sc, s->red_ws, s->dinvm, s->Lm, eta, rg, sigmu, s->tau, s->kappa, etk};
      HS_CALL( hs_ipm_dir_tail(s->stream, &ta, general_tail(s) ? 1 : 0, fuse_solve ? 1 : 0) );
   }
   for (auto& B : s->blk)
   {
      const int n = B.n;
      const long long n2 = (long long) n * n;
      if ( split == 0 )
         HS_CALL( pass_AT(s, B, s->dyt, eta, B.Rd, B.dZ) );
      else
      {
         bool combined = false;
         if ( split == 1 )
         {
            if ( &B == &s->blk[0] )
            {
               HS_CALL( hs_make_ext(s->stream, m, 0.0, 1.0, s->u1, s->cvec + m1) );
               HS_LAUNCH_CHECK();
            }
            if ( pack_with_dirmat(s, B) )
            {
               HS_CALL( hs_gemv_t_ws(s->stream, m1, B.Lp, B.Apk, B.Lp, s->cvec + m1, 0.0, NULL, B.pkv + B.Lp, s->gemvt_ws, s->gemvt_ws_len) );
               HS_CALL( hs_unpack_dz_combine(s->stream, n, B.pkv + B.Lp, B.P2, s->sc, SC_DTAU, eta, B.Rd, B.dZ) );
               combined = true;
            }
            else
               HS_CALL( pass_AT(s, B, s->cvec + m1, 0.0, NULL, B.dZ) );
         }
         if ( !combined )
            HS_CALL( hs_ipm_dz_combine(s->stream, n2, B.dZ, B.P2, s->sc, eta, B.Rd) );
      }
      if ( n <= HS_SMALL_N )
         HS_CALL( hs_dir_block_small(s->stream, n, 1.0, B.X, B.dZ, useE ? B.E : NULL, B.Zinv, sigmu, B.dX) );
      else
      {
         if ( useE )
            HS_CALL( hs_copy(s->stream, B.G, B.E, n2) );
         HS_CALL( gemm(s, HS_KC, HS_MC, n, n, n, 1.0, B.X, n, B.dZ, n, useE ? 1.0 : 0.0, B.G, n) );
         HS_CALL( gemm(s, HS_KC, HS_MC, n, n, n, 1.0, B.G, n, B.Zinv, n, 0.0, B.GZ, n) );
         HS_CALL( hs_dirmat(s->stream, n, sigmu, B.Zinv, B.X, B.GZ, B.dX) );
      }
   }
   if ( q > 0 )
   {
      if ( small_problem(s) )
      {
         HS_CALL( hs_lp_rows_small(s->stream, q, m1, s->Dext, s->dyt, 1, eta, sigmu, s->x, s->z,
            s->rd, useE ? s->elp : NULL, s->dz, s->dx) );
      }
      else
      {
         const double* v = s->dyt;
         HS_CALL( hs_gemv_n(s->stream, q, m1, s->Dext, m1, 1, &v, s->tmpq, q, s->gemv_ws, s->gemv_ws_len) );
         HS_CALL( hs_scale_add(s->stream, q, 1.0, s->tmpq, eta, s->rd, s->dz) );
         HS_CALL( hs_lp_dir(s->stream, q, sigmu, 1.0, s->x, s->z, s->dz, useE ? s->elp : NULL, s->dx) );
      }
   }
   return region.close();
}

static int steplen_enqueue(hipsdp_solver* s)
{
   int k = 0;
   hipStream_t st = s->stream, st2 = s->use2 ? s->stream2 : s->stream;
   HS_CALL( fork2(s) );
   for (auto& B : s->blk)
   {
      const int n = B.n;
      if ( n <= 64 )
         continue;
      HS_CALL( gemm_on(st, HS_KC, HS_MC, n, n, n, 1.0, B.LxInv, n, B.dX, n, 0.0, B.T1, n) );
      HS_CALL( gemm_on(st, HS_KC, HS_KC, n, n, n, 1.0, B.T1, n, B.LxInv, n, 0.0, B.W, n) );
      HS_CALL( gemm_on(st2, HS_KC, HS_MC, n, n, n, 1.0, B.LzInv, n, B.dZ, n, 0.0, B.T2, n) );
      HS_CALL( gemm_on(st2, HS_KC, HS_KC, n, n, n, 1.0, B.T2, n, B.LzInv, n, 0.0, B.W2, n) );
   }
   HS_CALL( join2(s) );
   int nmax_blk = 0;
   for (auto& B : s->blk)
      if ( B.n > nmax_blk ) nmax_blk = B.n;
   for (int cls = 0; cls < 2; ++cls)
   {
      hs_step_jobs J;
      J.nblk = 0;
      int kk = 0;
      for (auto& B : s->blk)
      {
         const bool mine = (cls == 0) ? (B.n <= 16) : (B.n > 16 && B.n <= 64);
         if ( mine )
         {
            const int j = J.nblk++;
            J.n[j] = B.n; J.L0[j] = B.LxInv; J.D0[j] = B.dX; J.L1[j] = B.LzInv; J.D1[j] = B.dZ;
            J.res0[j] = s->sc + SC_BLK(kk, 1); J.res1[j] = s->sc + SC_BLK(kk, 4);
            if ( J.nblk == HS_STEP_MAXJOBS )
            {
               HS_CALL( hs_steplen_small_multi(st, &J, s->par.lanczos_steps) );
               J.nblk = 0;
            }
         }
         ++kk;
      }
      HS_CALL( hs_steplen_small_multi(st, &J, s->par.lanczos_steps) );
   }
   for (auto& B : s->blk)
   {
      if ( B.n > 64 )
         HS_CALL( hs_lanczos_lmin2(st, B.n, B.W, B.W2, s->par.lanczos_steps, s->sc + SC_BLK(k, 1), s->sc + SC_BLK(k, 4), s->lan_ws,
               s->lan_ws2, s->lan_rot, s->lan_sync, nmax_blk) );
      ++k;
   }
   hs_red_batch_begin(s->stream);
   HS_CALL( hs_ratio_min(s->stream, s->q, s->x, s->dx, s->sc + SC_RATX, 0, s->red_ws) );
   HS_CALL( hs_ratio_min(s->stream, s->q, s->z, s->dz, s->sc + SC_RATZ, 0, s->red_ws) );
   return HS_OK;
}

static double steplen_host(hipsdp_solver* s, const HostScalars& h)
{
   double a = 1e300;
   for (size_t k = 0; k < s->blk.size(); ++k)
   {
      for (int which = 0; which < 2; ++which)
      {
         const double theta = h.v[SC_BLK(k, which ? 4 : 1)];
         const double resid = h.v[SC_BLK(k, which ? 5 : 2)];
         const double lo = theta - resid;
         if ( lo < 0.0 )
            a = fmin(a, -1.0 / lo);
      }
   }
   a = fmin(a, fmin(h.v[SC_RATX], h.v[SC_RATZ]));
   const double dtau = h.v[SC_DTAU], dkap = h.v[SC_DKAPPA];
   if ( dtau < 0.0 ) a = fmin(a, -s->tau / dtau);
   if ( dkap < 0.0 ) a = fmin(a, -s->kappa / dkap);
   return a;
}

static bool replicate_small(const hipsdp_solver* s)
{
// ... 438 lines not shown
   for (auto& B : s->blk)
      B.derived_valid = false;
   s->s1_last = 1;
   s->s1_sol_host = true;
   return HS_OK;
}

static int solve1_try(hipsdp_solver* s, hipsdp_info* info, bool* done)
{
   *done = false;
   S1Prep pp;
   bool offered = false;
   HS_CALL( solve1_prepare(s, &pp, &offered) );
   if ( !offered )
      return HS_OK;
   HS_CALL( hs_solve1_launch(s->stream, &pp.a) );
   HS_CALL( solve1_wait(pp.host, pp.a.seq, s->stream) );
   return solve1_finish(s, &pp, info, done);
}

static int solve_begin(hipsdp_solver* s, const hipsdp_params* params, hipsdp_info* info)
{
   g_err[0] = 0;
   if ( s == NULL || !s->shaped || info == NULL )
      return HIPSDP_ERR_ARG;
   if ( s->shardA && s->comm == NULL )
   {
      set_err("hipsdp_solve: the matrices of this problem are sharded by variable, the communicator is gone");
      return HIPSDP_ERR_ARG;
   }
   HS_HIP( hipSetDevice(s->device) );
   if ( params != NULL )
      s->par = *params;
   else
      hipsdp_default_params(&s->par);
   {
      if ( s->par.lanczos_steps <= 0 )
      {
         int nmin = 1 << 30;
         for (auto& B : s->blk) if ( B.n < nmin ) nmin = B.n;
         s->par.lanczos_steps = (!s->blk.empty() && nmin > 64) ? 16 : 24;
      }
      if ( s->par.settings < 0 ) s->par.settings = 0;
      if ( s->par.settings > 2 ) s->par.settings = 2;
      s->par.lanczos_steps <<= s->par.settings;
      bool lan_used = false;
      for (auto& B : s->blk)
         if ( B.n > 64 ) lan_used = true;
      if ( s->lan_sync != NULL && lan_used )
      {
         HS_CALL( hs_lanczos_sync_reset(s->stream, s->lan_sync, s->lan_rot) );
      }
      if ( s->trsv_ws != NULL && s->m > 2 * 64 )
         HS_CALL( hs_trsv_sync_init(s->stream, s->m, s->trsv_ws, &s->trsv_epoch) );
      if ( s->par.lanczos_steps < 4 ) s->par.lanczos_steps = 4;
      if ( s->par.lanczos_steps > 250 ) s->par.lanczos_steps = 250;
   }
   return HIPSDP_OK;
}

static void solve_reset(hipsdp_solver* s, hipsdp_info* info)
{
   hs_comm_phase(2);
   for (int p = 0; p < PH_COUNT; ++p) s->pc.ms[p] = 0.0;
   memset(info, 0, sizeof(*info));
   info->status = HIPSDP_STATUS_UNSOLVED;
   hs_red_batch_reset();
   s->pre_valid = false;
   s->clk_n = 0;
   s->clk_ghz = 0.0;
}

static int after_g1_x_inverse(void* arg)
{
   hipsdp_solver* s = static_cast<hipsdp_solver*>(arg);
   HS_CALL( fork2(s) );
   for (auto& B : s->blk)
      HS_CALL( hs_trtri(s->stream2, B.n, B.Lx, B.dinvx, B.LxInv, B.T1) );
   HS_HIP( hipEventRecord(s->evJoin, s->stream2) );
   s->sws.ev_g2 = (void*) s->evJoin;
   return HS_OK;
}

struct GeneralSolve
{
   hipsdp_solver* const s;
   hipsdp_info* const info;
   const std::chrono::steady_clock::time_point t_begin;
   const hipsdp_params& par = s->par;
   const hipStream_t st = s->stream;
   const int m = s->m, m1 = s->m + 1, q = s->q, K = (int) s->blk.size();
   const int settings = par.settings;
   const double gamma_eff = settings == 0 ? par.gamma : fmin(par.gamma, settings == 1 ? 0.9 : 0.75);
   const int stall_lim = settings == 0 ? 3 : (settings == 1 ? 5 : 8);
   const int nobest_lim = settings == 0 ? 6 : (settings == 1 ? 10 : 15);
   const double sigma_floor = settings == 0 ? 1e-8 : (settings == 1 ? 1e-4 : 1e-2);
   const bool no_identity_start = getenv("HIPSDP_NO_IDENTITY_START") != NULL && getenv("HIPSDP_NO_IDENTITY_START")[0] == '1';
   const bool optimistic = (s->comm == NULL) && getenv("HIPSDP_NO_OPTIMISTIC") == NULL;
   const char* const overstep = getenv("HIPSDP_TEST_OVERSTEP");

   double N1 = 0.0, normb = 0.0, normC = 0.0;
   bool small_all = false;
   int setf = 0;
   bool defer_ok = false;
   hipStream_t st2 = NULL;

   int it = 0, status = HIPSDP_STATUS_ITERLIM;
   bool stop = false;
   bool identity_start = false;
   bool factors_valid = false;
   bool residuals_ready = false;
   bool want_cert = false;
   bool rd_have = false;
   bool rd_pending = false;
   double rd_scale = 1.0;
   bool zchain_queued = false, xchain_queued = false;

   int certwait = 0, nstall = 0, sincebest = 0;
   double lastmu = 1e300, alpha_last = 1.0, bestmerit = 1e300;

   HostScalars hs;
   int hflags[3] = {0, 0, 0};
   double mu = 0, pinf = 0, dinf = 0, dabs = 0, gap = 0, pobj = 0, dobj = 0, rg = 0;
   double schur_ms = 0.0;
   bool defer_join = false, gram_only_used = false, schur_small = false;
   bool gram_cached = false;
   bool predH_queued = false, predH_joined = false, split_dz = false;
   double dta = 0, dka = 0, sigma = 0, eta = 0, amax = 0, alpha = 0, dt = 0, dk = 0;
   double tau0 = 0, kappa0 = 0, applied = 0;

   int halt(int why) { status = why; stop = true; return HS_OK; }

   int factor(hipStream_t qf, int n, double* L, double* dinv, const double* M, int f)
   {
      HS_CALL( hs_copy(qf, L, M, (long long) n * n) );
      return hs_potrf(qf, n, L, dinv, s->flags + f, NULL);
   }

   int z_chain(Block& B, hipStream_t qz)
   {
      const int n = B.n;
      if ( !factors_valid )
         HS_CALL( factor(qz, n, B.Lz, B.dinvz, B.Z, 0) );
      HS_CALL( hs_trtri(qz, n, B.Lz, B.dinvz, B.LzInv, B.T2) );
      HS_CALL( gemm_on(qz, HS_MC, HS_MC, n, n, n, 1.0, B.LzInv, n, B.LzInv, n, 0.0, B.Zinv, n, HS_GEMM_LOWER) );
      return hs_mirror_lower(qz, B.Zinv, n, n);
   }

   int x_chain(Block& B, bool inverse)
   {
      const int n = B.n;
      if ( !factors_valid )
         HS_CALL( factor(st, n, B.Lx, B.dinvx, B.X, 1) );
      HS_CALL( hs_zero_upper(st, B.Lx, n) );
      return inverse ? hs_trtri(st, n, B.Lx, B.dinvx, B.LxInv, B.T1) : HS_OK;
   }

   int queue_z_chains()
   {
      HS_CALL( fork2(s) );
      for (auto& B : s->blk)
         if ( B.n > 64 )
            HS_CALL( z_chain(B, st2) );
      zchain_queued = true;
      return HS_OK;
   }

   int read_back(int* flags3)
   {
      const std::function<int()> x_chains = [this]() -> int
      {
         for (auto& B : s->blk)
            if ( B.n > 64 )
               HS_CALL( x_chain(B, true) );
         xchain_queued = true;
         return HS_OK;
      };
      const bool with_x = zchain_queued && !xchain_queued && s->comm == NULL && !(factors_valid && defer_ok);
      return read_scalars(s, hs, flags3, with_x ? &x_chains : NULL);
   }

   void swap_trial()
   {
      for (auto& B : s->blk)
         if ( B.n <= 64 )
         {
            std::swap(B.X, B.Xs);
            std::swap(B.Z, B.Zs);
         }
   }

   int apply_step()
   {
      HS_CALL( hs_axpy3(st, alpha - applied, m, s->dy, s->y, q, s->dx, s->x, q, s->dz, s->z) );
      applied = alpha;
      s->tau = tau0 + alpha * dt;
      s->kappa = kappa0 + alpha * dk;
      return HS_OK;
   }

   int give_up(bool undo)
   {
      if ( par.verbose )
         printf("hipsdp: no step length down to %g keeps X and Z positive definite\n", alpha);
      if ( undo )
      {
         HS_CALL( hs_axpy3(st, -applied, m, s->dy, s->y, q, s->dx, s->x, q, s->dz, s->z) );
         s->tau = tau0;
         s->kappa = kappa0;
      }
      for (auto& B : s->blk)
      {
// ... 624 lines not shown
            else
               HS_CALL( hs_trsv_sync(st, m, s->Lm, s->dinvm, 2, s->rhs2, m, SOLVE_MODE, s->trsv_ws, &s->trsv_epoch) );
         }
      }
      split_dz = predH_joined && s->comm == NULL;
      for (auto& B : s->blk)
         if ( B.Apk == NULL )
            split_dz = false;
      const bool tail = general_tail(s);
      if ( m == 0 || m > 64 )
         HS_CALL( hs_ipm_after_solve2(st, m, s->rhs2, s->u2, s->wt, s->u1, (split_dz && tail) ? s->cvec : NULL, s->cvec + m1, 1) );
      hs_red_batch_begin(st);
      HS_CALL( hs_fill_scalar(st, s->sc + SC_S0, 0.0) );
      if ( split_dz && !tail )
      {
         HS_CALL( hs_make_ext(st, m, 1.0, 1.0, s->u2, s->cvec) );
         HS_CALL( hs_make_ext(st, m, 0.0, 1.0, s->u1, s->cvec + m1) );
         HS_LAUNCH_CHECK();
      }
      int slot = 0;
      for (auto& B : s->blk)
      {
         const int n = B.n;
         const long long n2 = (long long) n * n;
         bool swept = false;
         if ( split_dz )
         {
            if ( B.P2 == NULL )
            {
               HS_CALL( dalloc(&B.P2, n2) );
               HS_CALL( dalloc(&B.pk3, 3 * B.Lp) );
            }
            const int r3 = hs_gemv_t3(st, m1, B.Lp, B.Apk, B.Lp, s->wt, s->cvec, s->cvec + m1, B.pk3, B.pk3 + B.Lp, B.pk3 + 2 * B.Lp);
            if ( r3 < 0 )
               return -r3;
            if ( r3 == 1 )
            {
               if ( tail )
               {
                  const double* pk[3] = {B.pk3, B.pk3 + B.Lp, B.pk3 + 2 * B.Lp};
                  double* un[3] = {B.B, B.P2, B.dZ};
                  HS_CALL( hs_unpack_sym3(st, n, 3, pk, un) );
               }
               else
               {
                  HS_CALL( hs_unpack_sym(st, n, B.pk3, 0.0, NULL, B.B) );
                  HS_CALL( hs_unpack_sym(st, n, B.pk3 + B.Lp, 0.0, NULL, B.P2) );
                  HS_CALL( hs_unpack_sym(st, n, B.pk3 + 2 * B.Lp, 0.0, NULL, B.dZ) );
               }
               swept = true;
            }
            else
            {
               HS_CALL( pass_AT(s, B, s->cvec, 0.0, NULL, B.P2) );
               HS_CALL( pass_AT(s, B, s->cvec + m1, 0.0, NULL, B.dZ) );
            }
         }
         if ( !swept )
            HS_CALL( pass_AT(s, B, s->wt, 0.0, NULL, B.B) );
         HS_CALL( gemm(s, HS_KC, HS_MC, n, n, n, 1.0, B.X, n, B.B, n, 0.0, B.T1, n) );
         HS_CALL( gemm(s, HS_KC, HS_MC, n, n, n, 1.0, B.T1, n, B.Zinv, n, 0.0, B.W, n) );
         if ( tail )
            HS_CALL( hs_dot_deferred(st, n2, B.B, B.W, s->sc + SC_S0, 1, s->red_ws, slot++) );
         else
            HS_CALL( hs_dot(st, n2, B.B, B.W, s->sc + SC_S0, 1, s->red_ws) );
      }
      if ( q > 0 )
      {
         const double* v = s->wt;
         HS_CALL( hs_gemv_n(st, q, m1, s->Dext, m1, 1, &v, s->beta, q, s->gemv_ws, s->gemv_ws_len) );
         HS_CALL( hs_lp_s0(st, q, s->x, s->z, s->beta, s->sc + SC_S0, 1, s->red_ws) );
      }
      HS_CALL( hs_dot(st, m, s->b, s->rhs2 + m, s->sc + SC_BUB, 0, s->red_ws) );
      return hs_red_batch_end();
   }

   int predictor()
   {
      phase_mark(s, PH_PRED);
      if ( predH_queued && !predH_joined )
         HS_CALL( join2(s) );
      HS_CALL( direction(s, 0.0, 1.0, mu, rg, false, 0.0, predH_queued ? 2 : 0, predH_joined, split_dz ? 2 : 0) );
      HS_CALL( steplen_enqueue(s) );
      HS_CALL( read_scalars(s, hs, hflags) );
      float ms = 0.f;
      if ( hipEventElapsedTime(&ms, s->ev0, s->ev1) == hipSuccess )
         schur_ms += ms;
      info->schur_calls++;
      for (auto& B : s->blk)
         if ( !gram_cached )
            info->schur_flops += (gram_only_used && !B.sparse ? 0.0 : 4.0 * m1 * (double) B.n * B.n * B.n) + (double) m1 * m1 * (double) B.n * B.n;
      if ( hflags[0] != 0 || hflags[1] != 0 || hflags[2] != 0 )
      {
         if ( par.verbose )
            printf("hipsdp: Cholesky failure flags Z=%d X=%d M=%d\n", hflags[0], hflags[1], hflags[2]);
         return halt(HIPSDP_STATUS_NUMERIC);
      }
      const double aa = fmin(1.0, steplen_host(s, hs));
      dta = hs.v[SC_DTAU];
      dka = hs.v[SC_DKAPPA];
      if ( !std::isfinite(aa) || !std::isfinite(dta) )
      {
         if ( par.verbose )
            printf("hipsdp: predictor not finite (alpha %g dtau %g)\n", aa, dta);
         return halt(HIPSDP_STATUS_NUMERIC);
      }
      sigma = (1.0 - aa) * (1.0 - aa) * (1.0 - aa);
      sigma = fmin(1.0, fmax(sigma_floor, sigma));
      eta = 1.0 - sigma;
      return HS_OK;
   }

   int corrector()
   {
      phase_mark(s, PH_CORR);
      for (auto& B : s->blk)
         HS_CALL( gemm(s, HS_KC, HS_MC, B.n, B.n, B.n, 1.0, B.dX, B.n, B.dZ, B.n, 0.0, B.E, B.n) );
      {
         BatchRegion region(s, batch_regions(s));
         if ( q > 0 )
            HS_CALL( hs_vec_mul(st, q, s->dx, s->dz, s->elp) );
         HS_CALL( direction(s, sigma, eta, mu, rg, true, dta * dka, 0, false, split_dz ? 1 : 0) );
         HS_CALL( region.close() );
      }
      HS_CALL( steplen_enqueue(s) );
      HS_CALL( read_scalars(s, hs, NULL) );
      amax = steplen_host(s, hs);
      alpha = fmin(1.0, gamma_eff * amax);
      dt = hs.v[SC_DTAU];
      dk = hs.v[SC_DKAPPA];
      if ( !std::isfinite(alpha) || !std::isfinite(dt) || !std::isfinite(dk) )
      {
         if ( par.verbose )
            printf("hipsdp: corrector not finite (alpha %g dtau %g dkappa %g)\n", alpha, dt, dk);
         return halt(HIPSDP_STATUS_NUMERIC);
      }
      return HS_OK;
   }

   int update()
   {
      phase_mark(s, PH_UPDATE);
      tau0 = s->tau;
      kappa0 = s->kappa;
      applied = 0.0;
      return (small_all && K > 0) ? step_small() : step_general();
   }

   int step_small()
   {
      for (int attempt = 0; attempt < 8; ++attempt)
      {
         if ( !setf )
            HS_HIP( hipMemsetAsync(s->flags, 0, 8 * sizeof(int), st) );
         for (auto& B : s->blk)
         {
            double* L2[2] = {B.Lx, B.Lz};
            double* di2[2] = {B.dinvx, B.dinvz};
            int* fl2[2] = {s->flags + 1, s->flags + 0};
            const double* ba2[2] = {B.X, B.Z};
            const double* dr2[2] = {B.dX, B.dZ};
            double* mo2[2] = {B.Xs, B.Zs};
            double* li2[2] = {B.LxInv, B.LzInv};
            double* gr2[2] = {NULL, B.n <= 32 ? B.Zinv : NULL};
            HS_CALL( hs_potrf_small_ext_pair(st, B.n, L2, di2, fl2, ba2, dr2, alpha, mo2, li2, gr2, setf) );
         }
         swap_trial();
         if ( batch_regions(s) )
            hs_red_batch_hold(st);
         HS_CALL( apply_step() );
         HS_CALL( enqueue_residuals() );
         HS_CALL( read_scalars(s, hs, hflags) );
         if ( hflags[0] == 0 && hflags[1] == 0 )
         {
            for (auto& B : s->blk)
               B.derived_valid = true;
            factors_valid = true;
            residuals_ready = true;
            alpha_last = alpha;
            return HS_OK;
         }
         swap_trial();
         alpha *= 0.5;
         info->chol_fail++;
      }
      return give_up(true);
   }

   int step_general()
   {
      if ( it == 2 && overstep != NULL )
         alpha = amax * atof(overstep);
      for (int attempt = 0; attempt < 8; ++attempt)
      {
         HS_HIP( hipMemsetAsync(s->flags, 0, 8 * sizeof(int), st) );
         bool large = false, small = false;
         for (auto& B : s->blk)
            (B.n > 64 ? large : small) = true;
         if ( large && s->busy2 )
            HS_CALL( join2(s) );
         for (auto& B : s->blk)
         {
            if ( B.n <= 64 )
               continue;
            const hs_trial_job tj[2] = {{B.X, B.dX, B.Xs, B.Lx}, {B.Z, B.dZ, B.Zs, B.Lz}};
            HS_CALL( hs_trial_pair(st, (long long) B.n * B.n, alpha, attempt == 0 ? 1 : 0, tj) );
            const hs_potrf_job pj[2] = {{B.Lx, B.dinvx, s->flags + 1}, {B.Lz, B.dinvz, s->flags + 0}};
            HS_CALL( hs_potrf_pair(st, B.n, pj) );
         }
         if ( small )
         {
            HS_CALL( fork2(s) );
            for (auto& B : s->blk)
            {
               const int n = B.n;
               if ( n > 64 )
                  continue;
               HS_CALL( hs_potrf_small_ext(st, n, B.Lx, B.dinvx, s->flags + 1, B.X, B.dX, alpha, B.Xs, B.LxInv, NULL, setf) );
               HS_CALL( hs_potrf_small_ext(st2, n, B.Lz, B.dinvz, s->flags + 0, B.Z, B.dZ, alpha, B.Zs, B.LzInv, n <= 32 ? B.Zinv : NULL, setf) );
            }
            HS_CALL( join2(s) );
         }
         if ( K == 0 )
            break;
         if ( optimistic )
         {
            swap_trial();
            HS_CALL( apply_step() );
            factors_valid = true;
            if ( s->use2 && !zchain_queued )
               HS_CALL( queue_z_chains() );
            if ( attempt == 0 )
            {
               rd_have = !small_problem(s);
               rd_pending = rd_have;
               rd_scale = 1.0 - alpha * eta;
            }
            HS_CALL( enqueue_residuals() );
            HS_CALL( read_back(hflags) );
            if ( hflags[0] == 0 && hflags[1] == 0 )
               break;
            swap_trial();
            factors_valid = zchain_queued = xchain_queued = false;
            rd_have = rd_pending = false;
         }
         else
         {
            if ( s->comm == NULL )
               HS_CALL( publish_and_wait(s, s->nsc, 2) );
            else
            {
               HS_CALL( hs_bcast_ints(s->comm, s->flags, 3, st) );
               HS_HIP( hipMemcpyAsync(s->hsc + s->nsc, s->flags, 4 * sizeof(int), hipMemcpyDeviceToHost, st) );
               HS_HIP( hipStreamSynchronize(st) );
            }
            memcpy(hflags, s->hsc + s->nsc, 3 * sizeof(int));
            if ( hflags[0] == 0 && hflags[1] == 0 )
               break;
         }
         alpha *= 0.5;
         info->chol_fail++;
      }
      if ( K > 0 && (hflags[0] != 0 || hflags[1] != 0) )
         return give_up(optimistic && applied != 0.0);
      if ( !optimistic )
         swap_trial();
      for (auto& B : s->blk)
         if ( B.n <= 64 )
            B.derived_valid = true;
      factors_valid = (K > 0);
      alpha_last = alpha;
      if ( optimistic && K > 0 )
      {
         residuals_ready = true;
         return HS_OK;
      }
      HS_CALL( hs_axpy3(st, alpha, m, s->dy, s->y, q, s->dx, s->x, q, s->dz, s->z) );
      s->tau += alpha * dt;
      s->kappa += alpha * dk;
      rd_have = !small_problem(s);
      rd_pending = rd_have;
      rd_scale = 1.0 - alpha * eta;
      return HS_OK;
   }

   int run()
   {
      HS_CALL( start() );
      for (it = 0; it <= par.maxiter; ++it)
      {
         if ( !residuals_ready )
            HS_CALL( residual_pass() );
         residuals_ready = false;
         HS_CALL( terminate() );
         if ( stop )
            break;
         HS_CALL( factorize() );
         HS_CALL( assemble() );
         HS_CALL( solve_m() );
         HS_CALL( predictor() );
         if ( !stop )
            HS_CALL( corrector() );
         if ( !stop )
            HS_CALL( update() );
         if ( stop )
            break;
      }
      return HS_OK;
   }

   int finish()
   {
      HS_HIP( hipStreamSynchronize(st) );
      if ( s->clk_on && s->clk_n > 0 )
      {
         if ( s->clk_stream != NULL )
            HS_HIP( hipStreamSynchronize(s->clk_stream) );
         std::vector<unsigned long long> h((size_t) 4 * s->clk_n);
         HS_HIP( hipMemcpy(h.data(), s->clk_buf, h.size() * sizeof(unsigned long long), hipMemcpyDeviceToHost) );
         double dc = 0.0, dw = 0.0;
         for (int a = 0; a < s->clk_n; ++a)
// ... 1245 lines not shown
```

### scip-sdp_amd/csrc/kernels.hip

```cpp
#include "hs_kernels.h"
#include <string.h>
#include <stdio.h>
#include <stdlib.h>

static int hs_rec_dir_block_small(hipStream_t s, int n, double c, const double* X, const double* R, const double* E, const double* Zinv,
   double s1, double* out);
static int hs_rec_lp_dir(hipStream_t s, int q, double sigmu, double eta, const double* x, const double* z, const double* r, const double* elp,
   double* out);
static int hs_rec_vec_mul(hipStream_t s, long long n, const double* a, const double* b, double* out);
static int hs_rec_axpy3(hipStream_t s, double a, long long n1, const double* x1, double* y1, long long n2, const double* x2, double* y2,
   long long n3, const double* x3, double* y3);
static int hs_rec_gemv_t(hipStream_t s, int R, long long E, const double* A, long long lda, const double* coef, double sa, const double* add,
   double* out);

struct __attribute__((aligned(16))) dbl2 { double x, y; };
__device__ __forceinline__ dbl2 load_stream2(const double* p)
{
   typedef double gv2 __attribute__((ext_vector_type(2)));
   const gv2 t = __builtin_nontemporal_load(reinterpret_cast<const gv2*>(p));
   dbl2 r; r.x = t.x; r.y = t.y;
   return r;
}

static inline int hs_launch_ok(void)
{
   return hipGetLastError() == hipSuccess ? HS_OK : HS_ERR_HIP;
}


__global__ void k_fill(double* p, long long n, double v)
{
   for (long long i = (long long) blockIdx.x * blockDim.x + threadIdx.x; i < n; i += (long long) gridDim.x * blockDim.x)
      p[i] = v;
}

__global__ void k_identity(double* A, int n, double v)
{
   const long long total = (long long) n * n;
   for (long long i = (long long) blockIdx.x * blockDim.x + threadIdx.x; i < total; i += (long long) gridDim.x * blockDim.x)
   {
      const int r = (int) (i / n);
      const int c = (int) (i - (long long) r * n);
      A[i] = (r == c) ? v : 0.0;
   }
}

__global__ void k_scale_add(long long n, double a, const double* __restrict__ x, double b, const double* __restrict__ y,
   double* __restrict__ out)
{
   for (long long i = (long long) blockIdx.x * blockDim.x + threadIdx.x; i < n; i += (long long) gridDim.x * blockDim.x)
   {
      double v = a * x[i];
      if ( y != NULL )
         v += b * y[i];
      out[i] = v;
   }
}

__global__ void k_mirror_lower(double* A, int n, long long lda)
{
   const long long total = (long long) n * n;
   for (long long i = (long long) blockIdx.x * blockDim.x + threadIdx.x; i < total; i += (long long) gridDim.x * blockDim.x)
   {
      const int r = (int) (i / n);
      const int c = (int) (i - (long long) r * n);
      if ( r < c )
         A[(long long) r * lda + c] = A[(long long) c * lda + r];
   }
}

__global__ void k_mirror_upper(double* A, int n, long long lda)
{
   const long long total = (long long) n * n;
   for (long long i = (long long) blockIdx.x * blockDim.x + threadIdx.x; i < total; i += (long long) gridDim.x * blockDim.x)
   {
      const int r = (int) (i / n);
      const int c = (int) (i - (long long) r * n);
      if ( r > c )
         A[(long long) r * lda + c] = A[(long long) c * lda + r];
   }
}

__global__ void k_pack_rows(int m1, int n, long long Lp, const double* __restrict__ A, double* __restrict__ Apk)
{
   const long long n2 = (long long) n * n;
   const long long total = (long long) m1 * n2;
   for (long long e = (long long) blockIdx.x * blockDim.x + threadIdx.x; e < total; e += (long long) gridDim.x * blockDim.x)
   {
      const long long i = e / n2;
      const long long rc = e - i * n2;
      const int r = (int) (rc / n), c = (int) (rc - (long long) r * n);
      if ( c <= r )
         Apk[i * Lp + (long long) r * (r + 1) / 2 + c] = A[e];
   }
}

__global__ void k_packed_diag(int m1, int n, int ldd, long long Lp, const double* __restrict__ Apk, double* __restrict__ D)
{
   const long long total = (long long) m1 * ldd;
   for (long long e = (long long) blockIdx.x * blockDim.x + threadIdx.x; e < total; e += (long long) gridDim.x * blockDim.x)
   {
      const long long i = e / ldd;
      const int r = (int) (e - i * ldd);
      D[e] = r < n ? Apk[i * Lp + (long long) r * (r + 3) / 2] : 0.0;
   }
}

__global__ void k_sub_lower(int n, const double* __restrict__ S, double* __restrict__ C)
{
   const long long total = (long long) n * n;
   for (long long e = (long long) blockIdx.x * blockDim.x + threadIdx.x; e < total; e += (long long) gridDim.x * blockDim.x)
   {
      const int r = (int) (e / n), c = (int) (e - (long long) r * n);
      if ( c <= r )
         C[e] -= S[e];
   }
}

__global__ void k_pack_weighted(int n, const double* __restrict__ V, double* __restrict__ pk)
{
   const long long total = (long long) n * n;
   for (long long e = (long long) blockIdx.x * blockDim.x + threadIdx.x; e < total; e += (long long) gridDim.x * blockDim.x)
   {
      const int r = (int) (e / n), c = (int) (e - (long long) (e / n) * n);
      if ( c <= r )
         pk[(long long) r * (r + 1) / 2 + c] = (r == c ? 1.0 : 2.0) * V[e];
   }
}

__global__ void k_unpack_sym(int n, const double* __restrict__ pk, double sa, const double* __restrict__ add, double* __restrict__ out)
{
   const long long total = (long long) n * n;
   for (long long e = (long long) blockIdx.x * blockDim.x + threadIdx.x; e < total; e += (long long) gridDim.x * blockDim.x)
   {
      const int r0 = (int) (e / n), c0 = (int) (e - (long long) (e / n) * n);
      const int r = r0 > c0 ? r0 : c0, c = r0 > c0 ? c0 : r0;
      double v = pk[(long long) r * (r + 1) / 2 + c];
      if ( add != NULL )
         v += sa * add[e];
      out[e] = v;
   }
}

struct unpack3_args { const double* pk[3]; double* out[3]; };
__global__ void k_unpack_sym3(int n, unpack3_args U)
{
   const double* __restrict__ pk = U.pk[blockIdx.y];
   double* __restrict__ out = U.out[blockIdx.y];
   const long long total = (long long) n * n;
   for (long long e = (long long) blockIdx.x * blockDim.x + threadIdx.x; e < total; e += (long long) gridDim.x * blockDim.x)
   {
      const int r0 = (int) (e / n), c0 = (int) (e - (long long) (e / n) * n);
      const int r = r0 > c0 ? r0 : c0, c = r0 > c0 ? c0 : r0;
      out[e] = pk[(long long) r * (r + 1) / 2 + c];
   }
}

__global__ void k_unpack_dz_combine(int n, const double* __restrict__ pk, const double* __restrict__ P2, const double* __restrict__ sc, int idtau,
   double eta, const double* __restrict__ Rd, double* __restrict__ dZ)
{
   const double dtau = sc[idtau];
   const long long total = (long long) n * n;
   for (long long e = (long long) blockIdx.x * blockDim.x + threadIdx.x; e < total; e += (long long) gridDim.x * blockDim.x)
   {
      const int r0 = (int) (e / n), c0 = (int) (e - (long long) (e / n) * n);
      const int r = r0 > c0 ? r0 : c0, c = r0 > c0 ? c0 : r0;
      const double p1 = pk[(long long) r * (r + 1) / 2 + c];
      dZ[e] = (p1 - dtau * P2[e]) + eta * Rd[e];
   }
}

__global__ void k_dirmat_pack(int n, double s1, const double* __restrict__ Zinv, const double* __restrict__ X,
   const double* __restrict__ GZ, double* __restrict__ H, double* __restrict__ pk)
{
   const long long total = (long long) n * n;
   for (long long i = (long long) blockIdx.x * blockDim.x + threadIdx.x; i < total; i += (long long) gridDim.x * blockDim.x)
   {
      const int r = (int) (i / n);
      const int c = (int) (i - (long long) r * n);
      const double g = 0.5 * (GZ[i] + GZ[(long long) c * n + r]);
      const double h = s1 * Zinv[i] - X[i] - g;
      H[i] = h;
      if ( c <= r )
         pk[(long long) r * (r + 1) / 2 + c] = (r == c ? 1.0 : 2.0) * h;
   }
}

__global__ void k_zero_upper(double* A, int n)
{
   const long long total = (long long) n * n;
   for (long long i = (long long) blockIdx.x * blockDim.x + threadIdx.x; i < total; i += (long long) gridDim.x * blockDim.x)
   {
      const int r = (int) (i / n);
      const int c = (int) (i - (long long) r * n);
      if ( r < c )
         A[i] = 0.0;
   }
}

__global__ void k_symmetrize(double* A, int n)
{
   const long long total = (long long) n * n;
   for (long long i = (long long) blockIdx.x * blockDim.x + threadIdx.x; i < total; i += (long long) gridDim.x * blockDim.x)
   {
      const int r = (int) (i / n);
      const int c = (int) (i - (long long) r * n);
      if ( r > c )
      {
         const double v = 0.5 * (A[(long long) r * n + c] + A[(long long) c * n + r]);
         A[(long long) r * n + c] = v;
         A[(long long) c * n + r] = v;
      }
   }
}

__global__ void k_dirmat(int n, double s1, const double* __restrict__ Zinv, const double* __restrict__ X,
   const double* __restrict__ GZ, double* __restrict__ H)
{
   const long long total = (long long) n * n;
   for (long long i = (long long) blockIdx.x * blockDim.x + threadIdx.x; i < total; i += (long long) gridDim.x * blockDim.x)
   {
      const int r = (int) (i / n);
      const int c = (int) (i - (long long) r * n);
      const double g = 0.5 * (GZ[i] + GZ[(long long) c * n + r]);
      H[i] = s1 * Zinv[i] - X[i] - g;
   }
}

__global__ void k_lp_dir(int q, double sigmu, double eta, const double* __restrict__ x, const double* __restrict__ z,
   const double* __restrict__ r, const double* __restrict__ elp, double* __restrict__ out)
{
   const int i = blockIdx.x * blockDim.x + threadIdx.x;
   if ( i < q )
   {
      double t = eta * x[i] * r[i];
      if ( elp != NULL )
         t += elp[i];
      out[i] = sigmu / z[i] - x[i] - t / z[i];
   }
}

__global__ void k_lp_scale_rows(int q, int cols, const double* __restrict__ x, const double* __restrict__ z,
   const double* __restrict__ D, double* __restrict__ S)
{
   const long long total = (long long) q * cols;
   for (long long i = (long long) blockIdx.x * blockDim.x + threadIdx.x; i < total; i += (long long) gridDim.x * blockDim.x)
   {
      const int r = (int) (i / cols);
      S[i] = (x[r] / z[r]) * D[i];
   }
}

__global__ void k_vec_mul(long long n, const double* __restrict__ a, const double* __restrict__ b, double* __restrict__ out)
{
   for (long long i = (long long) blockIdx.x * blockDim.x + threadIdx.x; i < n; i += (long long) gridDim.x * blockDim.x)
      out[i] = a[i] * b[i];
}

static inline int grid_for(long long n, int block, int cap)
{
   long long g = (n + block - 1) / block;
   if ( g > cap ) g = cap;
   if ( g < 1 ) g = 1;
   return (int) g;
}

int hs_fill(hipStream_t s, double* p, long long n, double v)
{
   (void) hs_red_batch_flush();
   if ( n <= 0 ) return HS_OK;
   hipLaunchKernelGGL(k_fill, dim3(grid_for(n, 256, 2048)), dim3(256), 0, s, p, n, v);
   HS_LAUNCH_CHECK();
   return HS_OK;
}

int hs_set_identity(hipStream_t s, double* A, int n, double v)
{
   (void) hs_red_batch_flush();
   if ( n <= 0 ) return HS_OK;
   hipLaunchKernelGGL(k_identity, dim3(grid_for((long long) n * n, 256, 2048)), dim3(256), 0, s, A, n, v);
   HS_LAUNCH_CHECK();
   return HS_OK;
}

__global__ void k_copy(long long n, const double* __restrict__ src, double* __restrict__ dst)
{
   for (long long i = (long long) blockIdx.x * blockDim.x + threadIdx.x; i < n; i += (long long) gridDim.x * blockDim.x)
      dst[i] = src[i];
}

long long hs_objs_lane_layout(int m, int q, int nblk, const int* n, int gap, long long* off)
{
   long long t = 0;
   int i = 0;
   auto put = [&](long long len) { off[i++] = t; t += ((len + 1) & ~1LL) + gap; };
   put(m); put(m); put(q); put(q);
   for (int k = 0; k < nblk; ++k)
   {
      put((long long) n[k] * n[k]);
      put((long long) n[k] * n[k]);
   }
   return t;
}

__global__ void __launch_bounds__(256) k_objs_fanout(const hs_fan_plan P, double* __restrict__ lanes, long long lane_stride, int nlanes)
{
   typedef double fan_v2 __attribute__((ext_vector_type(2)));
   const hs_fan_seg& S = P.seg[blockIdx.y];
   const long long nv = S.len >> 1;
   for (long long j = blockIdx.x; j < nlanes; j += gridDim.x)
   {
      const double* __restrict__ src = (j == 0) ? S.src0 : S.src + (j - 1) * S.stride;
      double* __restrict__ dst = lanes + j * lane_stride + S.dst;
      for (long long e = threadIdx.x; e < nv; e += 256)
// ... 9 lines not shown
      return HS_OK;
   if ( plan->nseg > HS_FAN_MAXSEG || (lane_stride & 1) || (reinterpret_cast<size_t>(lanes) & 15) )
      return HS_ERR_ARG;
   for (int i = 0; i < plan->nseg; ++i)
   {
      const hs_fan_seg& S = plan->seg[i];
      if ( S.len <= 0 || (S.dst & 1) || (S.stride & 1) || (reinterpret_cast<size_t>(S.src0) & 15) || (reinterpret_cast<size_t>(S.src) & 15) )
         return HS_ERR_ARG;
   }
   const int gx = nlanes < (1 << 20) ? nlanes : (1 << 20);
   hipLaunchKernelGGL(k_objs_fanout, dim3(gx, plan->nseg), dim3(256), 0, st, *plan, lanes, lane_stride, nlanes);
   HS_LAUNCH_CHECK();
   return HS_OK;
}

int hs_copy(hipStream_t s, double* dst, const double* src, long long n)
{
   (void) hs_red_batch_flush();
   if ( n <= 0 ) return HS_OK;
   if ( n <= (1LL << 16) )
   {
      hipLaunchKernelGGL(k_copy, dim3(grid_for(n, 256, 256)), dim3(256), 0, s, n, src, dst);
      HS_LAUNCH_CHECK();
      return HS_OK;
   }
   HS_HIP( hipMemcpyAsync(dst, src, (size_t) n * sizeof(double), hipMemcpyDeviceToDevice, s) );
   return HS_OK;
}

__global__ void k_axpy3(double a, long long n1, const double* __restrict__ x1, double* __restrict__ y1, long long n2,
   const double* __restrict__ x2, double* __restrict__ y2, long long n3, const double* __restrict__ x3, double* __restrict__ y3)
{
   const long long total = n1 + n2 + n3;
   for (long long i = (long long) blockIdx.x * blockDim.x + threadIdx.x; i < total; i += (long long) gridDim.x * blockDim.x)
   {
      if ( i < n1 )
         y1[i] += a * x1[i];
      else if ( i < n1 + n2 )
         y2[i - n1] += a * x2[i - n1];
      else
         y3[i - n1 - n2] += a * x3[i - n1 - n2];
   }
}

int hs_axpy3(hipStream_t s, double a, long long n1, const double* x1, double* y1, long long n2, const double* x2, double* y2,
   long long n3, const double* x3, double* y3)
{
   if ( n1 < 0 ) n1 = 0;
   if ( n2 < 0 ) n2 = 0;
   if ( n3 < 0 ) n3 = 0;
   if ( n1 + n2 + n3 == 0 ) return HS_OK;
   if ( hs_rec_axpy3(s, a, n1, x1, y1, n2, x2, y2, n3, x3, y3) )
      return HS_OK;
   hipLaunchKernelGGL(k_axpy3, dim3(grid_for(n1 + n2 + n3, 256, 2048)), dim3(256), 0, s, a, n1, x1, y1, n2, x2, y2, n3, x3, y3);
   HS_LAUNCH_CHECK();
   return HS_OK;
}

int hs_scale_add(hipStream_t s, long long n, double a, const double* x, double b, const double* y, double* out)
{
   (void) hs_red_batch_flush();
   if ( n <= 0 ) return HS_OK;
   hipLaunchKernelGGL(k_scale_add, dim3(grid_for(n, 256, 2048)), dim3(256), 0, s, n, a, x, b, y, out);
   HS_LAUNCH_CHECK();
   return HS_OK;
}

__global__ void k_trial_pair(long long n, double a, double b, int first, hs_trial_job J0, hs_trial_job J1)
{
   const hs_trial_job J = blockIdx.y ? J1 : J0;
   const double* base = first ? J.V : J.Vs;
   for (long long i = (long long) blockIdx.x * blockDim.x + threadIdx.x; i < n; i += (long long) gridDim.x * blockDim.x)
   {
      const double y = base[i];
      double v = a * J.dV[i];
      v += b * y;
      if ( first )
         J.Vs[i] = y;
      J.V[i] = v;
      J.L[i] = v;
   }
}

int hs_trial_pair(hipStream_t s, long long n, double alpha, int first, const hs_trial_job* jobs)
{
   (void) hs_red_batch_flush();
   if ( n <= 0 ) return HS_OK;
   hipLaunchKernelGGL(k_trial_pair, dim3(grid_for(n, 256, 2048), 2), dim3(256), 0, s, n, alpha, 1.0, first, jobs[0], jobs[1]);
   HS_LAUNCH_CHECK();
   return HS_OK;
}

int hs_axpy(hipStream_t s, long long n, double a, const double* x, double* y)
{
   (void) hs_red_batch_flush();
   return hs_scale_add(s, n, a, x, 1.0, y, y);
}

int hs_mirror_lower(hipStream_t s, double* A, int n, long long lda)
{
   (void) hs_red_batch_flush();
   if ( n <= 1 ) return HS_OK;
   hipLaunchKernelGGL(k_mirror_lower, dim3(grid_for((long long) n * n, 256, 2048)), dim3(256), 0, s, A, n, lda);
   HS_LAUNCH_CHECK();
   return HS_OK;
}

int hs_mirror_upper(hipStream_t s, double* A, int n, long long lda)
{
   (void) hs_red_batch_flush();
   if ( n <= 1 ) return HS_OK;
   hipLaunchKernelGGL(k_mirror_upper, dim3(grid_for((long long) n * n, 256, 2048)), dim3(256), 0, s, A, n, lda);
   HS_LAUNCH_CHECK();
   return HS_OK;
}

int hs_pack_rows(hipStream_t s, int m1, int n, long long Lp, const double* A, double* Apk)
{
   (void) hs_red_batch_flush();
   HS_HIP( hipMemsetAsync(Apk, 0, (size_t) m1 * (size_t) Lp * sizeof(double), s) );
   hipLaunchKernelGGL(k_pack_rows, dim3(grid_for((long long) m1 * n * n, 256, 65536)), dim3(256), 0, s, m1, n, Lp, A, Apk);
   HS_LAUNCH_CHECK();
   return HS_OK;
}

int hs_packed_diag(hipStream_t s, int m1, int n, int ldd, long long Lp, const double* Apk, double* D)
{
   (void) hs_red_batch_flush();
   if ( ldd < n )
      return HS_ERR_ARG;
   hipLaunchKernelGGL(k_packed_diag, dim3(grid_for((long long) m1 * ldd, 256, 2048)), dim3(256), 0, s, m1, n, ldd, Lp, Apk, D);
   HS_LAUNCH_CHECK();
   return HS_OK;
}

int hs_sub_lower(hipStream_t s, int n, const double* S, double* C)
{
   (void) hs_red_batch_flush();
   hipLaunchKernelGGL(k_sub_lower, dim3(grid_for((long long) n * n, 256, 2048)), dim3(256), 0, s, n, S, C);
   HS_LAUNCH_CHECK();
   return HS_OK;
}

int hs_pack_weighted(hipStream_t s, int n, const double* V, double* pk)
{
   (void) hs_red_batch_flush();
   hipLaunchKernelGGL(k_pack_weighted, dim3(grid_for((long long) n * n, 256, 2048)), dim3(256), 0, s, n, V, pk);
   HS_LAUNCH_CHECK();
   return HS_OK;
}

int hs_unpack_sym(hipStream_t s, int n, const double* pk, double sa, const double* add, double* out)
{
   (void) hs_red_batch_flush();
   hipLaunchKernelGGL(k_unpack_sym, dim3(grid_for((long long) n * n, 256, 2048)), dim3(256), 0, s, n, pk, sa, add, out);
   HS_LAUNCH_CHECK();
   return HS_OK;
}

int hs_unpack_sym3(hipStream_t s, int n, int cnt, const double* const* pk, double* const* out)
{
   (void) hs_red_batch_flush();
   if ( cnt < 1 || cnt > 3 )
      return HS_ERR_ARG;
   unpack3_args U = {{NULL, NULL, NULL}, {NULL, NULL, NULL}};
   for (int k = 0; k < cnt; ++k)
   {
      U.pk[k] = pk[k]; U.out[k] = out[k];
   }
   hipLaunchKernelGGL(k_unpack_sym3, dim3(grid_for((long long) n * n, 256, 2048), cnt), dim3(256), 0, s, n, U);
   HS_LAUNCH_CHECK();
   return HS_OK;
}

int hs_unpack_dz_combine(hipStream_t s, int n, const double* pk, const double* P2, const double* sc, int idtau, double eta, const double* Rd,
   double* dZ)
{
   (void) hs_red_batch_flush();
   hipLaunchKernelGGL(k_unpack_dz_combine, dim3(grid_for((long long) n * n, 256, 2048)), dim3(256), 0, s, n, pk, P2, sc, idtau, eta, Rd, dZ);
   HS_LAUNCH_CHECK();
   return HS_OK;
}

int hs_zero_upper(hipStream_t s, double* A, int n)
{
   (void) hs_red_batch_flush();
   if ( n <= 1 ) return HS_OK;
   hipLaunchKernelGGL(k_zero_upper, dim3(grid_for((long long) n * n, 256, 2048)), dim3(256), 0, s, A, n);
   HS_LAUNCH_CHECK();
   return HS_OK;
}

__global__ void __launch_bounds__(256) k_transpose(int n, const double* __restrict__ src, double* __restrict__ dst)
{
   __shared__ double tile[32][33];
   const int bx = blockIdx.x * 32, by = blockIdx.y * 32;
   const int tx = threadIdx.x & 31, ty = threadIdx.x >> 5;
   for (int r = ty; r < 32; r += 8)
      if ( by + r < n && bx + tx < n )
         tile[r][tx] = src[(long long) (by + r) * n + bx + tx];
   __syncthreads();
   for (int r = ty; r < 32; r += 8)
      if ( bx + r < n && by + tx < n )
         dst[(long long) (bx + r) * n + by + tx] = tile[tx][r];
}

int hs_transpose(hipStream_t s, int n, const double* src, double* dst)
{
   (void) hs_red_batch_flush();
   if ( n <= 0 ) return HS_OK;
   const int t = (n + 31) / 32;
   hipLaunchKernelGGL(k_transpose, dim3(t, t), dim3(256), 0, s, n, src, dst);
   HS_LAUNCH_CHECK();
   return HS_OK;
}

int hs_symmetrize(hipStream_t s, double* A, int n)
{
   (void) hs_red_batch_flush();
   if ( n <= 1 ) return HS_OK;
   hipLaunchKernelGGL(k_symmetrize, dim3(grid_for((long long) n * n, 256, 2048)), dim3(256), 0, s, A, n);
   HS_LAUNCH_CHECK();
   return HS_OK;
}

#include "hs_lds_product.h"

__device__ void d_dir_block_small(int n, double c, const double* __restrict__ X, const double* __restrict__ R,
   const double* __restrict__ E, const double* __restrict__ Zinv, double s1, double* __restrict__ out, double* db_smem)
{
   const int ld = n + 1;
   double* sx = db_smem;
   double* sr = sx + n * ld;
   double* sz = sr + n * ld;
   double* sg = sz + n * ld;
   const int tid = threadIdx.x;
   const int n2 = n * n;
   if ( n2 <= 256 )
   {
      const int e = tid;
      const bool in = e < n2;
      const int r = in ? e / n : 0, cc = in ? e - r * n : 0;
      const double evv = (in && E != NULL) ? E[e] : 0.0;
      if ( in )
      {
         sx[r * ld + cc] = X[e];
         sr[r * ld + cc] = R[e];
         sz[r * ld + cc] = Zinv[e];
      }
      __syncthreads();
      if ( in )
      {
         double acc = 0.0;
         for (int k = 0; k < n; ++k)
            acc = fma(sx[r * ld + k], sr[k * ld + cc], acc);
         double g = acc * c;
         if ( E != NULL )
            g = __dadd_rn(g, evv);
// ... 9 lines not shown
      __syncthreads();
      if ( in )
         sr[r * ld + cc] = gz;
      __syncthreads();
      if ( in )
         out[e] = s1 * sz[r * ld + cc] - sx[r * ld + cc] - 0.5 * (sr[r * ld + cc] + sr[cc * ld + r]);
      return;
   }
   double ev[DB_PR][DB_PC];
   {
      const int tc = (n + DB_PC - 1) / DB_PC;
      const int pr = tid / tc, pc = tid - pr * tc;
#pragma unroll
      for (int i = 0; i < DB_PR; ++i)
#pragma unroll
         for (int j = 0; j < DB_PC; ++j)
         {
            const int r = min(DB_PR * pr + i, n - 1), cc = min(DB_PC * pc + j, n - 1);
            ev[i][j] = (E != NULL) ? E[r * n + cc] : 0.0;
         }
      const int ueff = (n2 + 255) >> 8;
      double xv[DB_U], rv[DB_U], zv[DB_U];
#pragma unroll
      for (int u = 0; u < DB_U; ++u)
         if ( u < ueff )
         {
            const int e = min(tid + 256 * u, n2 - 1);
            xv[u] = X[e];
            rv[u] = R[e];
            zv[u] = Zinv[e];
         }
#pragma unroll
      for (int u = 0; u < DB_U; ++u)
      {
         const int e = tid + 256 * u;
         if ( u < ueff && e < n2 )
         {
            const int r = e / n, cc = e - r * n;
            sx[r * ld + cc] = xv[u];
            sr[r * ld + cc] = rv[u];
            sz[r * ld + cc] = zv[u];
         }
      }
   }
   __syncthreads();
   db_product(n, ld, sx, sr, [&](int i, int j, int r, int cc, double acc)
   {
      double g = acc * c;
      if ( E != NULL )
         g = __dadd_rn(g, ev[i][j]);
      sg[r * ld + cc] = g;
   });
   __syncthreads();
   db_product(n, ld, sg, sz, [&](int, int, int r, int cc, double acc) { sr[r * ld + cc] = acc; });
   __syncthreads();
   for (int e = tid; e < n2; e += 256)
   {
      const int r = e / n, cc = e - r * n;
      out[e] = s1 * sz[r * ld + cc] - sx[r * ld + cc] - 0.5 * (sr[r * ld + cc] + sr[cc * ld + r]);
   }
}

__global__ void __launch_bounds__(256) k_dir_block_small(int n, double c, const double* __restrict__ X, const double* __restrict__ R,
   const double* __restrict__ E, const double* __restrict__ Zinv, double s1, double* __restrict__ out)
{
   extern __shared__ double db_smem_k[];
   d_dir_block_small(n, c, X, R, E, Zinv, s1, out, db_smem_k);
}

int hs_dir_block_small(hipStream_t s, int n, double c, const double* X, const double* R, const double* E, const double* Zinv,
   double s1, double* out)
{
   if ( n <= 0 ) return HS_OK;
   if ( n > HS_SMALL_N ) return HS_ERR_ARG;
   if ( hs_rec_dir_block_small(s, n, c, X, R, E, Zinv, s1, out) )
      return HS_OK;
   static hs_attr_mask attr_done;
   HS_CALL( hs_func_max_lds(reinterpret_cast<const void*>(&k_dir_block_small), 4 * HS_SMALL_N * (HS_SMALL_N + 1) * (int) sizeof(double), &attr_done) );
   hipLaunchKernelGGL(k_dir_block_small, dim3(1), dim3(256), (size_t) 4 * n * (n + 1) * sizeof(double), s, n, c, X, R, E, Zinv, s1, out);
   HS_LAUNCH_CHECK();
   return HS_OK;
}

int hs_dirmat(hipStream_t s, int n, double s1, const double* Zinv, const double* X, const double* GZ, double* H)
{
   (void) hs_red_batch_flush();
   if ( n <= 0 ) return HS_OK;
   hipLaunchKernelGGL(k_dirmat, dim3(grid_for((long long) n * n, 256, 2048)), dim3(256), 0, s, n, s1, Zinv, X, GZ, H);
   HS_LAUNCH_CHECK();
   return HS_OK;
}

int hs_dirmat_pack(hipStream_t s, int n, double s1, const double* Zinv, const double* X, const double* GZ, double* H, double* pk)
{
   (void) hs_red_batch_flush();
   hipLaunchKernelGGL(k_dirmat_pack, dim3(grid_for((long long) n * n, 256, 2048)), dim3(256), 0, s, n, s1, Zinv, X, GZ, H, pk);
   HS_LAUNCH_CHECK();
   return HS_OK;
}

int hs_lp_dir(hipStream_t s, int q, double sigmu, double eta, const double* x, const double* z, const double* r,
   const double* elp, double* out)
{
   if ( q <= 0 ) return HS_OK;
   if ( hs_rec_lp_dir(s, q, sigmu, eta, x, z, r, elp, out) )
      return HS_OK;
   hipLaunchKernelGGL(k_lp_dir, dim3((q + 255) / 256), dim3(256), 0, s, q, sigmu, eta, x, z, r, elp, out);
   HS_LAUNCH_CHECK();
   return HS_OK;
}

int hs_lp_scale_rows(hipStream_t s, int q, int cols, const double* x, const double* z, const double* D, double* S)
{
   (void) hs_red_batch_flush();
   if ( q <= 0 ) return HS_OK;
   hipLaunchKernelGGL(k_lp_scale_rows, dim3(grid_for((long long) q * cols, 256, 2048)), dim3(256), 0, s, q, cols, x, z, D, S);
   HS_LAUNCH_CHECK();
   return HS_OK;
}

int hs_vec_mul(hipStream_t s, long long n, const double* a, const double* b, double* out)
{
   if ( n <= 0 ) return HS_OK;
   if ( hs_rec_vec_mul(s, n, a, b, out) )
      return HS_OK;
   hipLaunchKernelGGL(k_vec_mul, dim3(grid_for(n, 256, 2048)), dim3(256), 0, s, n, a, b, out);
   HS_LAUNCH_CHECK();
   return HS_OK;
}


struct OpSum { __device__ static double id() { return 0.0; } __device__ static double f(double a, double b) { return a + b; } };
struct OpMax { __device__ static double id() { return 0.0; } __device__ static double f(double a, double b) { return a > b ? a : b; } };
struct OpMin { __device__ static double id() { return 1e300; } __device__ static double f(double a, double b) { return a < b ? a : b; } };

template<class OP>
__device__ __forceinline__ double wave_reduce(double v)
{
#pragma unroll
   for (int off = 32; off > 0; off >>= 1)
      v = OP::f(v, __shfl_down(v, off, 64));
   return v;
}

template<class OP>
__device__ __forceinline__ double block_reduce_256(double v, double* sh)
{
   v = wave_reduce<OP>(v);
   const int lane = threadIdx.x & 63;
   const int wave = threadIdx.x >> 6;
   if ( lane == 0 )
      sh[wave] = v;
   __syncthreads();
   double r = OP::id();
   if ( threadIdx.x == 0 )
   {
      r = sh[0];
      for (int w = 1; w < (int) (blockDim.x >> 6); ++w)
         r = OP::f(r, sh[w]);
   }
   __syncthreads();
   return r;
}


#define RED_DOT      0
#define RED_ABSMAX   1
#define RED_RATIOMIN 2
#define RED_LPS0     3
#define RED_STAGE_N  2048

template<int KIND> struct RedTraits;
template<> struct RedTraits<RED_DOT>      { typedef OpSum OP; };
template<> struct RedTraits<RED_ABSMAX>   { typedef OpMax OP; };
template<> struct RedTraits<RED_RATIOMIN> { typedef OpMin OP; };
template<> struct RedTraits<RED_LPS0>     { typedef OpSum OP; };

template<int KIND>
__device__ __forceinline__ double red_elem(long long i, const double* a, const double* b, const double* c)
{
   if ( KIND == RED_DOT )
      return a[i] * b[i];
   if ( KIND == RED_ABSMAX )
      return fabs(a[i]);
   if ( KIND == RED_RATIOMIN )
   {
      const double d = b[i];
      return d < 0.0 ? -a[i] / d : 1e300;
   }
   return (a[i] / b[i]) * c[i] * c[i];
}

template<int KIND>
__global__ void __launch_bounds__(256) k_reduce_stage1(long long n, const double* __restrict__ a, const double* __restrict__ b,
   const double* __restrict__ c, double* __restrict__ part, double* __restrict__ out, int accumulate, int direct)
{
   typedef typename RedTraits<KIND>::OP OP;
   __shared__ double sh[4];
   double v = OP::id();
   for (long long i = (long long) blockIdx.x * blockDim.x + threadIdx.x; i < n; i += (long long) gridDim.x * blockDim.x)
      v = OP::f(v, red_elem<KIND>(i, a, b, c));
   v = block_reduce_256<OP>(v, sh);
   if ( threadIdx.x == 0 )
   {
      if ( direct )
         *out = accumulate ? OP::f(*out, v) : v;
      else
         part[blockIdx.x] = v;
   }
}

template<int KIND>
__global__ void __launch_bounds__(256) k_reduce_stage2(int nparts, const double* __restrict__ part, double* __restrict__ out,
   int accumulate)
{
   typedef typename RedTraits<KIND>::OP OP;
   __shared__ double sh[4];
   double v = OP::id();
   for (int i = threadIdx.x; i < nparts; i += blockDim.x)
      v = OP::f(v, part[i]);
   v = block_reduce_256<OP>(v, sh);
   if ( threadIdx.x == 0 )
      *out = accumulate ? OP::f(*out, v) : v;
}

#define RB_MAX   24
#define RB_MAXN  16384
#define RB_ROWS  64
#define RB_MATS  32
#define RB_MAXWORK 16384
#define RB_FILL  100
#define RB_COPY1 101
#define RB_SOLVE 102
#define RB_FINISH 103
#define RB_STAGE2 105
#define RB_DIRBLK  110
#define RB_LPDIR   111
#define RB_VECMUL  112
#define RB_AXPY3   113
#define RB_MAKEEXT 114
#define RB_GEMVT   115
#define RB_LPROWS  116
#define RB_APPLYA  117

struct rb_desc { int kind; int accumulate; int i[6]; double d[4]; const void* p[10]; };
struct rb_finish { int m; double eta, rg, sigmu, tau, kappa, etk; const double* u1; const double* u2; double* dy; double* dyt; double* sc;
   int s0, bub, bh, wrp, bu1, dtau, dkappa, den; };
struct rb_args { int cnt; rb_desc d[RB_MAX]; rb_finish fin; int pub_n; const double* pub_src; double* pub_dst;
   unsigned long long pub_seq; unsigned long long* pub_flag;
   unsigned long long* dbg; };
static_assert(sizeof(rb_args) <= 4096, "the records travel as kernel arguments");
static thread_local struct { bool open; hipStream_t s; int hold; size_t smem; rb_args args; } g_rb = {false, NULL, 0, 0, {0, {}}};

#define RB_STAGES (RB_MAXN / RED_STAGE_N)
static_assert(RB_STAGES * RED_STAGE_N == RB_MAXN && RB_STAGES <= 256, "rb_run keeps one partial result per first-stage workgroup");

template<int KIND>
__device__ __forceinline__ double rb_run(const rb_desc& D, double* sh, double* part)
{
   typedef typename RedTraits<KIND>::OP OP;
   const double* a = (const double*) D.p[0];
   const double* b = (const double*) D.p[1];
   const double* c = (const double*) D.p[2];
   double* out = (double*) D.p[3];
   const int n = D.i[0];
   const int g = (n + RED_STAGE_N - 1) / RED_STAGE_N;
   double v = OP::id();
   if ( g <= 1 )
   {
      for (long long i = threadIdx.x; i < n; i += 256)
         v = OP::f(v, red_elem<KIND>(i, a, b, c));
      v = block_reduce_256<OP>(v, sh);
   }
   else
   {
      double w[RB_STAGES];
#pragma unroll
      for (int k = 0; k < RB_STAGES; ++k)
         w[k] = OP::id();
      for (int base = threadIdx.x; base < n; base += 256 * g)
      {
#pragma unroll
         for (int k = 0; k < RB_STAGES; ++k)
         {
            const int i = base + 256 * k;
            if ( k < g && i < n )
               w[k] = OP::f(w[k], red_elem<KIND>(i, a, b, c));
         }
      }
#pragma unroll
      for (int k = 0; k < RB_STAGES; ++k)
      {
         if ( k < g )
         {
            const double r = block_reduce_256<OP>(w[k], sh);
            if ( threadIdx.x == 0 )
               part[k] = r;
         }
      }
      __syncthreads();
      if ( (int) threadIdx.x < g )
         v = OP::f(v, part[threadIdx.x]);
      v = block_reduce_256<OP>(v, sh);
   }
   if ( threadIdx.x == 0 )
      *out = D.accumulate ? OP::f(*out, v) : v;
   return v;
}

__device__ __forceinline__ double d_tree64(double (&p)[64])
{
#pragma unroll
   for (int off = 32; off > 0; off >>= 1)
#pragma unroll
      for (int l = 0; l < off; ++l)
         p[l] += p[l + off];
   return p[0];
}

template<int KIND>
__device__ __forceinline__ void rb_run_wave(const rb_desc& D)
{
   typedef typename RedTraits<KIND>::OP OP;
   const double* a = (const double*) D.p[0];
   const double* b = (const double*) D.p[1];
   const double* c = (const double*) D.p[2];
   double* out = (double*) D.p[3];
   const int lane = threadIdx.x & 63;
   double v[4];
#pragma unroll
   for (int g = 0; g < 4; ++g)
   {
      double x = OP::id();
      for (long long i = 64 * g + lane; i < D.i[0]; i += 256)
         x = OP::f(x, red_elem<KIND>(i, a, b, c));
      v[g] = x;
   }
#pragma unroll
   for (int g = 0; g < 4; ++g)
      v[g] = wave_reduce<OP>(v[g]);
   if ( lane == 0 )
   {
      double r = v[0];
      r = OP::f(r, v[1]); r = OP::f(r, v[2]); r = OP::f(r, v[3]);
      *out = D.accumulate ? OP::f(*out, r) : r;
   }
}

__global__ void __launch_bounds__(256) k_red_batch(rb_args A)
{
   extern __shared__ double rb_dyn[];
   __shared__ double sh[4];
   __shared__ double sh_part[RB_STAGES];
   for (int t = 0; t < A.cnt; ++t)
   {
      {
         int g = 0;
         while ( g < 4 && t + g < A.cnt && A.d[t + g].kind <= RED_LPS0 && A.d[t + g].i[0] <= 1024 )
         {
            bool fresh = true;
            for (int h = 0; h < g; ++h)
               fresh = fresh && A.d[t + h].p[3] != A.d[t + g].p[3];
            if ( !fresh )
               break;
            ++g;
         }
         if ( g > 1 )
         {
            const unsigned long long tg_begin = (A.dbg != NULL) ? wall_clock64() : 0ULL;
            const int w = threadIdx.x >> 6;
            if ( w < g )
            {
               const rb_desc& G = A.d[t + w];
               switch ( G.kind )
               {
               case RED_DOT:      rb_run_wave<RED_DOT>(G); break;
               case RED_ABSMAX:   rb_run_wave<RED_ABSMAX>(G); break;
               case RED_RATIOMIN: rb_run_wave<RED_RATIOMIN>(G); break;
               default:           rb_run_wave<RED_LPS0>(G); break;
               }
            }
            __threadfence_block();
            __syncthreads();
            if ( A.dbg != NULL && threadIdx.x == 0 )
            {
               atomicAdd(A.dbg + 2 * 8, wall_clock64() - tg_begin);
               atomicAdd(A.dbg + 2 * 8 + 1, 1ULL);
            }
            t += g - 1;
            continue;
         }
      }
      const rb_desc& D = A.d[t];
      const unsigned long long t_begin = (A.dbg != NULL) ? wall_clock64() : 0ULL;
      const unsigned long long c_begin = (A.dbg != NULL) ? clock64() : 0ULL;
      switch ( D.kind )
      {
      case RED_DOT:      rb_run<RED_DOT>(D, sh, sh_part); break;
      case RED_ABSMAX:   rb_run<RED_ABSMAX>(D, sh, sh_part); break;
      case RED_RATIOMIN: rb_run<RED_RATIOMIN>(D, sh, sh_part); break;
      case RED_LPS0:     rb_run<RED_LPS0>(D, sh, sh_part); break;
      case RB_FILL:      if ( threadIdx.x == 0 ) *(double*) D.p[3] = D.d[0]; break;
      case RB_COPY1:     if ( threadIdx.x == 0 ) *(double*) D.p[3] = *(const double*) D.p[0]; break;
      case RB_STAGE2:
      {
         const double* part = (const double*) D.p[0];
         double* out = (double*) D.p[3];
         double v = OpSum::id();
         for (int i = threadIdx.x; i < D.i[0]; i += 256)
            v = OpSum::f(v, part[i]);
         v = block_reduce_256<OpSum>(v, sh);
         if ( threadIdx.x == 0 )
            *out = D.accumulate ? OpSum::f(*out, v) : v;
         break;
      }
      case RB_DIRBLK:
         d_dir_block_small(D.i[0], D.d[0], (const double*) D.p[0], (const double*) D.p[1], (const double*) D.p[2], (const double*) D.p[3],
            D.d[1], (double*) D.p[4], rb_dyn);
         break;
      case RB_LPDIR:
      {
         const double* x = (const double*) D.p[0]; const double* z = (const double*) D.p[1]; const double* r = (const double*) D.p[2];
         const double* elp = (const double*) D.p[3]; double* out = (double*) D.p[4];
         const double sigmu = D.d[0], eta = D.d[1];
         for (int i = threadIdx.x; i < D.i[0]; i += 256)
         {
            double t = eta * x[i] * r[i];
            if ( elp != NULL )
               t += elp[i];
// ... 142 lines not shown
         const double* A1 = (const double*) D.p[2]; const double* V1 = (const double*) D.p[3];
         const double* Dext = (const double*) D.p[4]; const double* vlp = (const double*) D.p[5];
         for (int base = 0; base < m1; base += RB_MATS)
         {
            const int nm = min(RB_MATS, m1 - base);
            const int t = threadIdx.x;
            if ( nblk == 1 && n2a <= 256 && q <= 256 )
            {
               const bool hs = t < n2a, hl = t < q;
               const double v0 = hs ? V0[t] : 0.0, vl = hl ? vlp[t] : 0.0;
               const double* ap = A0 + (hs ? t : 0);
               const double* dp = Dext + (long long) (hl ? t : 0) * m1;
               for (int ii = 0; ii < nm; ii += 8)
               {
                  double xa[8], xd[8];
#pragma unroll
                  for (int u = 0; u < 8; ++u)
                  {
                     const int i = base + min(ii + u, nm - 1);
                     xa[u] = ap[(long long) i * n2a];
                     xd[u] = hl ? dp[i] : 0.0;
                  }
#pragma unroll
                  for (int u = 0; u < 8; ++u)
                     if ( ii + u < nm )
                     {
                        double a = 0.0;
                        if ( hs )
                           a += xa[u] * v0;
                        if ( hl )
                           a += xd[u] * vl;
                        rb_dyn[((ii + u) * 4 + (t >> 6)) * 65 + (t & 63)] = a;
                     }
               }
            }
            else
            for (int ii = 0; ii < nm; ++ii)
            {
               const int i = base + ii;
               double a = 0.0;
               {
                  const double* ap = A0 + (long long) i * n2a;
                  for (int e = t; e < n2a; e += 256)
                     a += ap[e] * V0[e];
               }
               if ( nblk > 1 )
               {
                  const double* ap = A1 + (long long) i * n2b;
                  for (int e = t; e < n2b; e += 256)
                     a += ap[e] * V1[e];
               }
               for (int r = t; r < q; r += 256)
                  a += Dext[(long long) r * m1 + i] * vlp[r];
               rb_dyn[(ii * 4 + (t >> 6)) * 65 + (t & 63)] = a;
            }
            __syncthreads();
            for (int jj = threadIdx.x; jj < 4 * ((nm + 15) / 16) * 16; jj += 256)
            {
               const int ii = min(jj >> 2, nm - 1), g = jj & 3;
               double pl[64];
#pragma unroll
               for (int l = 0; l < 64; ++l)
                  pl[l] = rb_dyn[(ii * 4 + g) * 65 + l];
               const double sg = d_tree64(pl);
               const double s1v = __shfl_down(sg, 1, 64), s2v = __shfl_down(sg, 2, 64), s3v = __shfl_down(sg, 3, 64);
               const double v = ((sg + s1v) + s2v) + s3v;
               const int i = base + (jj >> 2);
               if ( g == 0 && (jj >> 2) < nm )
               {
                  out[i] = v;
                  if ( i >= 1 )
                  {
                     if ( epi == 1 )
                        vout[i - 1] = v - scal * vin[i - 1];
                     else if ( epi == 2 )
                        vout[i - 1] = vin[i - 1] * scal - v;
                  }
               }
            }
            __syncthreads();
         }
         break;
      }
      case RB_SOLVE:
      {
         __shared__ double sL[64 * 65];
         __shared__ double tv[64], tw[64], tr[64], ldg[64];
         const int m = D.i[0];
         const long long stride = (long long) D.d[0];
         const double* Da = (const double*) D.p[0];
         const double* Db = (const double*) D.p[1];
         const int row = threadIdx.x >> 2, part = threadIdx.x & 3;
         if ( D.i[1] )
         {
            for (int e = threadIdx.x; e < m * m; e += 256)
            {
               const int i = e / m, j = e - i * m;
               if ( j <= i )
                  sL[i * 65 + j] = Db[(long long) i * m + j];
            }
            __syncthreads();
            const int wv = threadIdx.x >> 6, ln = threadIdx.x & 63;
            for (int k = wv; k < D.accumulate; k += 4)
            {
               double* vec = (double*) D.p[3] + k * stride;
               const double x = hs_wl_msolve(sL, m, ln, ln < m ? vec[ln] : 0.0);
               if ( ln < m )
                  vec[ln] = x;
            }
            __syncthreads();
            break;
         }
         for (int e = threadIdx.x; e < m * m; e += 256)
         {
            const int i = e / m, j = e - i * m;
            if ( j <= i )
               sL[i * 65 + j] = Da[i * 64 + j];
            if ( j < i )
               sL[j * 65 + i] = Db[(long long) i * m + j];
            if ( j == i )
               ldg[i] = Db[(long long) i * m + i];
         }
         for (int k = 0; k < D.accumulate; ++k)
         {
            double* vec = (double*) D.p[3] + k * stride;
            if ( threadIdx.x < m )
               tv[threadIdx.x] = vec[threadIdx.x];
            __syncthreads();
            double x0 = 0.0;
            {
               double acc = 0.0;
               if ( row < m )
               {
#pragma unroll 4
                  for (int j = part; j <= row; j += 4)
                     acc += sL[row * 65 + j] * tv[j];
               }
               acc += __shfl_xor(acc, 1, 64);
               acc += __shfl_xor(acc, 2, 64);
               x0 = acc;
               if ( row < m && part == 0 )
                  tw[row] = acc;
            }
            __syncthreads();
            {
               double acc = 0.0;
               if ( row < m )
               {
#pragma unroll 4
                  for (int j = part; j < row; j += 4)
                     acc += sL[j * 65 + row] * tw[j];
               }
               acc += __shfl_xor(acc, 1, 64);
               acc += __shfl_xor(acc, 2, 64);
               if ( row < m && part == 0 )
                  tr[row] = tv[row] - (acc + ldg[row] * x0);
            }
            __syncthreads();
            {
               double acc = 0.0;
               if ( row < m )
               {
#pragma unroll 4
                  for (int j = part; j <= row; j += 4)
                     acc += sL[row * 65 + j] * tr[j];
               }
               acc += __shfl_xor(acc, 1, 64);
               acc += __shfl_xor(acc, 2, 64);
               if ( row < m && part == 0 )
                  tw[row] = x0 + acc;
            }
            __syncthreads();
            {
               double acc = 0.0;
               if ( row < m )
               {
#pragma unroll 4
                  for (int i = row + part; i < m; i += 4)
                     acc += sL[i * 65 + row] * tw[i];
               }
               acc += __shfl_xor(acc, 1, 64);
               acc += __shfl_xor(acc, 2, 64);
               x0 = acc;
               if ( row < m && part == 0 )
                  tv[row] = acc;
            }
            __syncthreads();
            {
               double acc = 0.0;
               if ( row < m )
               {
#pragma unroll 4
                  for (int i = row + 1 + part; i < m; i += 4)
                     acc += sL[row * 65 + i] * tv[i];
               }
               acc += __shfl_xor(acc, 1, 64);
               acc += __shfl_xor(acc, 2, 64);
               if ( row < m && part == 0 )
                  tr[row] = tw[row] - (acc + ldg[row] * x0);
            }
            __syncthreads();
            {
               double acc = 0.0;
               if ( row < m )
               {
#pragma unroll 4
                  for (int i = row + part; i < m; i += 4)
                     acc += sL[i * 65 + row] * tr[i];
               }
               acc += __shfl_xor(acc, 1, 64);
               acc += __shfl_xor(acc, 2, 64);
               if ( row < m && part == 0 )
                  vec[row] = x0 + acc;
            }
            __syncthreads();
         }
         break;
      }
      default:
      {
         const rb_finish& F = A.fin;
         const double den = F.sc[F.s0] + F.kappa / F.tau + F.sc[F.bub];
         const double num = -F.eta * F.rg + (F.sigmu - F.tau * F.kappa - F.etk) / F.tau - F.sc[F.bh] - F.eta * F.sc[F.wrp] + F.sc[F.bu1];
         const double dtau = num / den;
         __syncthreads();
         if ( threadIdx.x == 0 )
         {
            F.sc[F.dtau] = dtau;
            F.sc[F.dkappa] = (F.sigmu - F.tau * F.kappa - F.etk - F.kappa * dtau) / F.tau;
            F.sc[F.den] = den;
            F.dyt[0] = -dtau;
         }
         for (int i = threadIdx.x; i < F.m; i += 256)
         {
            const double v = F.u1[i] - F.u2[i] * dtau;
            F.dy[i] = v;
            F.dyt[1 + i] = v;
         }
         break;
      }
      }
      __threadfence_block();
      __syncthreads();
      if ( A.dbg != NULL && threadIdx.x == 0 )
      {
         const unsigned long long dt = wall_clock64() - t_begin;
         atomicAdd(A.dbg + 2 * (D.kind & 31), dt);
         atomicAdd(A.dbg + 2 * (D.kind & 31) + 1, 1ULL);
         atomicAdd(A.dbg + 64, dt);
         atomicAdd(A.dbg + 65, (unsigned long long) clock64() - c_begin);
      }
   }
   if ( A.pub_n > 0 )
   {
      for (int i = threadIdx.x; i < A.pub_n; i += 256)
         __builtin_nontemporal_store(A.pub_src[i], A.pub_dst + i);
      __threadfence_system();
      __syncthreads();
      if ( threadIdx.x == 0 )
         __hip_atomic_store(A.pub_flag, A.pub_seq, __ATOMIC_RELEASE, __HIP_MEMORY_SCOPE_SYSTEM);
   }
}

static unsigned long long* g_rb_dbg = NULL;
static void rb_dbg_report(void)
{
   unsigned long long h[66];
   if ( g_rb_dbg == NULL || hipMemcpy(h, g_rb_dbg, sizeof(h), hipMemcpyDeviceToHost) != hipSuccess )
      return;
   if ( h[64] > 0 )
      fprintf(stderr, "batch records: shader clock while they ran %.0f MHz\n", (double) h[65] / ((double) h[64] * 0.01));
   for (int k = 0; k < 32; ++k)
      if ( h[2 * k + 1] > 0 )
         fprintf(stderr, "batch records of kind %%32 = %2d: %10llu records, %8.3f us each\n", k, h[2 * k + 1],
            (double) h[2 * k] / (double) h[2 * k + 1] * 0.01);
}
static unsigned long long* rb_dbg_buffer(void)
{
   static int on = -1;
   if ( on < 0 )
   {
      const char* env = getenv("HIPSDP_BATCH_TIMES");
      on = (env != NULL && env[0] == '1') ? 1 : 0;
      if ( on && hipMalloc((void**) &g_rb_dbg, 66 * sizeof(unsigned long long)) == hipSuccess
         && hipMemset(g_rb_dbg, 0, 66 * sizeof(unsigned long long)) == hipSuccess )
         atexit(rb_dbg_report);
      else
         g_rb_dbg = NULL;
   }
   return g_rb_dbg;
}

static int rb_flush(void)
{
   if ( g_rb.args.cnt > 0 || g_rb.args.pub_n > 0 )
   {
      if ( g_rb.smem > 0 )
      {
         static hs_attr_mask attr_done;
         HS_CALL( hs_func_max_lds(reinterpret_cast<const void*>(&k_red_batch), 4 * HS_SMALL_N * (HS_SMALL_N + 1) * (int) sizeof(double), &attr_done) );
         static_assert(4 * HS_SMALL_N * (HS_SMALL_N + 1) >= RB_MATS * 4 * 65 && RB_MATS * 4 * 65 >= RB_ROWS * 65, "dynamic LDS of the batch kernel");
      }
      g_rb.args.dbg = rb_dbg_buffer();
      hipLaunchKernelGGL(k_red_batch, dim3(1), dim3(256), g_rb.smem, g_rb.s, g_rb.args);
      g_rb.args.cnt = 0;
      g_rb.args.pub_n = 0;
      g_rb.smem = 0;
      HS_LAUNCH_CHECK();
   }
   return HS_OK;
}

// ... 70 lines not shown
   if ( !g_rb.open )
      g_rb.args.cnt = 0;
   g_rb.open = false;
   return rb_flush();
}

static int rb_record(hipStream_t s, int kind, long long n, const double* a, const double* b, const double* c, double* out,
   int accumulate, double v)
{
   if ( !g_rb.open )
      return 0;
   if ( s != g_rb.s || n > RB_MAXN )
   {
      (void) rb_flush();
      return 0;
   }
   if ( g_rb.args.cnt == RB_MAX )
      (void) rb_flush();
   rb_desc& D = g_rb.args.d[g_rb.args.cnt++];
   memset(&D, 0, sizeof(D));
   D.kind = kind; D.accumulate = accumulate; D.i[0] = (int) n; D.p[0] = a; D.p[1] = b; D.p[2] = c; D.p[3] = out; D.d[0] = v;
   return 1;
}

static rb_desc* rb_record_ext(hipStream_t s, int kind, size_t smem)
{
   if ( !g_rb.open || g_rb.hold == 0 )
      return NULL;
   if ( s != g_rb.s )
   {
      (void) rb_flush();
      return NULL;
   }
   if ( g_rb.args.cnt == RB_MAX )
      (void) rb_flush();
   rb_desc& D = g_rb.args.d[g_rb.args.cnt++];
   memset(&D, 0, sizeof(D));
   D.kind = kind;
   if ( smem > g_rb.smem )
      g_rb.smem = smem;
   return &D;
}

int hs_fill_scalar(hipStream_t s, double* p, double v)
{
   if ( rb_record(s, RB_FILL, 1, NULL, NULL, NULL, p, 0, v) )
      return HS_OK;
   return hs_fill(s, p, 1, v);
}

int hs_copy_scalar(hipStream_t s, double* dst, const double* src)
{
   if ( rb_record(s, RB_COPY1, 1, src, NULL, NULL, dst, 0, 0.0) )
      return HS_OK;
   return hs_copy(s, dst, src, 1);
}

int hs_small_solve_by_substitution(void)
{
   const char* e = getenv("HIPSDP_SMALL_SOLVE");
   return (e != NULL && e[0] == 's') ? 1 : 0;
}

int hs_red_batch_solve(hipStream_t s, int m, const double* dinv, const double* L, int nrhs, double* vec, long long ld)
{
   if ( m > 64 )
      return 0;
   if ( !rb_record(s, RB_SOLVE, m, dinv, L, NULL, vec, nrhs, (double) ld) )
      return 0;
   g_rb.args.d[g_rb.args.cnt - 1].i[1] = hs_small_solve_by_substitution();
   return 1;
}

int hs_red_batch_finish(hipStream_t s, const void* fin, size_t bytes)
{
   if ( !g_rb.open || s != g_rb.s || bytes != sizeof(rb_finish) )
      return 0;
   if ( g_rb.args.cnt == RB_MAX )
      (void) rb_flush();
   memcpy(&g_rb.args.fin, fin, sizeof(rb_finish));
   rb_desc& D = g_rb.args.d[g_rb.args.cnt++];
   memset(&D, 0, sizeof(D));
   D.kind = RB_FINISH;
   return 1;
}

static int rb_decline(void)
{
   if ( g_rb.open && g_rb.hold > 0 )
      (void) rb_flush();
   return 0;
}

static int hs_rec_dir_block_small(hipStream_t s, int n, double c, const double* X, const double* R, const double* E, const double* Zinv,
   double s1, double* out)
{
   rb_desc* D = rb_record_ext(s, RB_DIRBLK, (size_t) 4 * n * (n + 1) * sizeof(double));
   if ( D == NULL )
      return 0;
   D->i[0] = n; D->d[0] = c; D->d[1] = s1; D->p[0] = X; D->p[1] = R; D->p[2] = E; D->p[3] = Zinv; D->p[4] = out;
   return 1;
}

static int hs_rec_lp_dir(hipStream_t s, int q, double sigmu, double eta, const double* x, const double* z, const double* r, const double* elp,
   double* out)
{
   if ( q > RB_MAXN )
      return rb_decline();
   rb_desc* D = rb_record_ext(s, RB_LPDIR, 0);
   if ( D == NULL )
      return 0;
   D->i[0] = q; D->d[0] = sigmu; D->d[1] = eta; D->p[0] = x; D->p[1] = z; D->p[2] = r; D->p[3] = elp; D->p[4] = out;
   return 1;
}

static int hs_rec_vec_mul(hipStream_t s, long long n, const double* a, const double* b, double* out)
{
   if ( n > RB_MAXN )
      return rb_decline();
   rb_desc* D = rb_record_ext(s, RB_VECMUL, 0);
   if ( D == NULL )
      return 0;
   D->i[0] = (int) n; D->p[0] = a; D->p[1] = b; D->p[2] = out;
   return 1;
}

static int hs_rec_axpy3(hipStream_t s, double a, long long n1, const double* x1, double* y1, long long n2, const double* x2, double* y2,
   long long n3, const double* x3, double* y3)
{
   if ( n1 > RB_MAXN || n2 > RB_MAXN || n3 > RB_MAXN )
      return rb_decline();
   rb_desc* D = rb_record_ext(s, RB_AXPY3, 0);
   if ( D == NULL )
      return 0;
   D->d[0] = a; D->i[0] = (int) n1; D->i[1] = (int) n2; D->i[2] = (int) n3;
   D->p[0] = x1; D->p[1] = y1; D->p[2] = x2; D->p[3] = y2; D->p[4] = x3; D->p[5] = y3;
   return 1;
}

static int hs_rec_gemv_t(hipStream_t s, int R, long long E, const double* A, long long lda, const double* coef, double sa, const double* add,
   double* out)
{
   if ( E > RB_MAXN || lda > 0x7fffffffLL || (long long) R * E > RB_MAXWORK )
      return rb_decline();
   rb_desc* D = rb_record_ext(s, RB_GEMVT, 0);
   if ( D == NULL )
      return 0;
   D->i[0] = R; D->i[1] = (int) E; D->i[2] = (int) lda; D->d[0] = sa; D->p[0] = A; D->p[1] = coef; D->p[2] = add; D->p[3] = out;
   return 1;
}

__global__ void k_make_ext(int m, double s0, double s1, const double* __restrict__ v, double* __restrict__ ext)
{
   const int i = blockIdx.x * blockDim.x + threadIdx.x;
   if ( i == 0 )
      ext[0] = s0;
   if ( i < m )
      ext[1 + i] = s1 * v[i];
}

int hs_make_ext(hipStream_t s, int m, double s0, double s1, const double* v, double* ext)
{
   if ( m <= RB_MAXN )
   {
      rb_desc* D = rb_record_ext(s, RB_MAKEEXT, 0);
      if ( D != NULL )
// ... 622 lines not shown
```

### scip-sdp_amd/csrc/units.hip

```cpp
#include "hs_kernels.h"
#include "hs_gram_cache.h"
#include "../../include/hipsdp.h"
#include "../../include/hipsdp_units.h"
#include <vector>
#include <algorithm>
#include <cstring>
#include <cstdlib>

namespace {

struct DevBuf
{
   double* p;
   DevBuf() : p(NULL) {}
   ~DevBuf() { if ( p ) (void) hipFree(p); }
   int alloc(long long n) { if ( n <= 0 ) n = 1; hipError_t e = hipMalloc((void**) &p, (size_t) n * sizeof(double)); if ( e != hipSuccess ) { hs_record_hip_error(e, "hipMalloc", __FILE__, __LINE__); return e == hipErrorOutOfMemory ? HS_ERR_NOMEM : HS_ERR_HIP; } return HS_OK; }
   int up(const double* h, long long n) { if ( n <= 0 ) return HS_OK; hipError_t e = hipMemcpy(p, h, (size_t) n * sizeof(double), hipMemcpyHostToDevice); if ( e != hipSuccess ) { hs_record_hip_error(e, "H2D", __FILE__, __LINE__); return HS_ERR_HIP; } return HS_OK; }
   int down(double* h, long long n) { if ( n <= 0 ) return HS_OK; hipError_t e = hipMemcpy(h, p, (size_t) n * sizeof(double), hipMemcpyDeviceToHost); if ( e != hipSuccess ) { hs_record_hip_error(e, "D2H", __FILE__, __LINE__); return HS_ERR_HIP; } return HS_OK; }
};

int pick_device(int device)
{
   int nd = 0;
   if ( hipGetDeviceCount(&nd) != hipSuccess || nd <= 0 )
// ... 940 lines not shown
   HS_CALL( rc );
   return dO.down(out, 3 * n2);
}

extern "C" int hipsdp_tail_dz_unit(int device, int n, int fused, const double* pk, const double* P2, const double* Rd, double dtau, double eta,
   double* dZ)
{
   if ( n < 1 || (fused != 0 && fused != 1) || pk == NULL || P2 == NULL || Rd == NULL || dZ == NULL )
      return HIPSDP_ERR_ARG;
   HS_CALL( pick_device(device) );
   const long long n2 = (long long) n * n, Lp = packed_len(n);
   const int nsc = hs_ipm_sc_len(1);
   DevBuf dP, dP2, dR, dZd, dS;
   HS_CALL( dP.alloc(Lp) ); HS_CALL( dP2.alloc(n2) ); HS_CALL( dR.alloc(n2) ); HS_CALL( dZd.alloc(n2) ); HS_CALL( dS.alloc(nsc) );
   HS_CALL( nan_fill(dZd, n2) );
   std::vector<double> sc((size_t) nsc, 0.0);
   sc[hs_ipm_sc_dtau()] = dtau;
   HS_CALL( dS.up(sc.data(), nsc) ); HS_CALL( dP.up(pk, Lp) ); HS_CALL( dP2.up(P2, n2) ); HS_CALL( dR.up(Rd, n2) );
   int rc;
   if ( fused )
      rc = hs_unpack_dz_combine(0, n, dP.p, dP2.p, dS.p, hs_ipm_sc_dtau(), eta, dR.p, dZd.p);
   else
   {
      rc = hs_unpack_sym(0, n, dP.p, 0.0, NULL, dZd.p);
      if ( rc == HS_OK ) rc = hs_ipm_dz_combine(0, n2, dZd.p, dP2.p, dS.p, eta, dR.p);
   }
   if ( rc == HS_OK && hipDeviceSynchronize() != hipSuccess ) rc = HS_ERR_HIP;
   HS_CALL( rc );
   return dZd.down(dZ, n2);
}

extern "C" int hipsdp_tail_dirmat_unit(int device, int n, int fused, double s1, const double* Zinv, const double* X, const double* GZ, double* H,
   double* pk)
{
   if ( n < 1 || (fused != 0 && fused != 1) || Zinv == NULL || X == NULL || GZ == NULL || H == NULL || pk == NULL )
      return HIPSDP_ERR_ARG;
   HS_CALL( pick_device(device) );
   const long long n2 = (long long) n * n, Lp = packed_len(n);
   DevBuf dZ, dX, dG, dH, dP;
   HS_CALL( dZ.alloc(n2) ); HS_CALL( dX.alloc(n2) ); HS_CALL( dG.alloc(n2) ); HS_CALL( dH.alloc(n2) ); HS_CALL( dP.alloc(Lp) );
   HS_CALL( nan_fill(dH, n2) ); HS_CALL( nan_fill(dP, Lp) );
   HS_CALL( dZ.up(Zinv, n2) ); HS_CALL( dX.up(X, n2) ); HS_CALL( dG.up(GZ, n2) );
   int rc;
   if ( fused )
      rc = hs_dirmat_pack(0, n, s1, dZ.p, dX.p, dG.p, dH.p, dP.p);
   else
   {
      rc = hs_dirmat(0, n, s1, dZ.p, dX.p, dG.p, dH.p);
      if ( rc == HS_OK ) rc = hs_pack_weighted(0, n, dH.p, dP.p);
   }
   if ( rc == HS_OK && hipDeviceSynchronize() != hipSuccess ) rc = HS_ERR_HIP;
   HS_CALL( rc );
   HS_CALL( dH.down(H, n2) );
   return dP.down(pk, Lp);
}

extern "C" int hipsdp_tail_sc_len(void) { return hs_ipm_sc_len(1); }
extern "C" int hipsdp_tail_dir_unit(int device, int m, int n, int fused, const double* B, const double* H, const double* rhs2, const double* rp,
   const double* b, const double* u1, const double* u2, const double* par, double* sc, double* dy, double* dyt)
{
   if ( m < 1 || n < 1 || (fused != 0 && fused != 1) || B == NULL || H == NULL || rhs2 == NULL || rp == NULL || b == NULL || u1 == NULL
         || u2 == NULL || par == NULL || sc == NULL || dy == NULL || dyt == NULL )
      return HIPSDP_ERR_ARG;
   HS_CALL( pick_device(device) );
   const long long n2 = (long long) n * n;
   const int nsc = hs_ipm_sc_len(1);
   DevBuf dB, dH, dR, dRp, db, dU1, dU2, dS, dY, dYt, dW;
   HS_CALL( dB.alloc(n2) ); HS_CALL( dH.alloc(n2) ); HS_CALL( dR.alloc(m) ); HS_CALL( dRp.alloc(m) ); HS_CALL( db.alloc(m) );
   HS_CALL( dU1.alloc(m) ); HS_CALL( dU2.alloc(m) ); HS_CALL( dS.alloc(nsc) ); HS_CALL( dY.alloc(m) ); HS_CALL( dYt.alloc(m + 1) );
   HS_CALL( dW.alloc(HS_RED_WS_DOUBLES) );
   HS_CALL( nan_fill(dY, m) ); HS_CALL( nan_fill(dYt, m + 1) ); HS_CALL( nan_fill(dW, HS_RED_WS_DOUBLES) );
   HS_CALL( dB.up(B, n2) ); HS_CALL( dH.up(H, n2) ); HS_CALL( dR.up(rhs2, m) ); HS_CALL( dRp.up(rp, m) ); HS_CALL( db.up(b, m) );
   HS_CALL( dU1.up(u1, m) ); HS_CALL( dU2.up(u2, m) ); HS_CALL( dS.up(sc, nsc) );
   const double* pB = dB.p; const double* pH = dH.p;
   const hs_dir_tail_args ta = {m, 0, 1, &n, &pB, &pH, NULL, NULL, dR.p, dRp.p, db.p, dU1.p, dU2.p, dY.p, dYt.p, dS.p, dW.p, NULL, NULL,
      par[0], par[1], par[2], par[3], par[4], par[5]};
   hs_red_batch_reset();
   int rc = hs_ipm_dir_tail(0, &ta, fused, 0);
   if ( rc == HS_OK && hipDeviceSynchronize() != hipSuccess ) rc = HS_ERR_HIP;
   hs_red_batch_reset();
   HS_CALL( rc );
   HS_CALL( dS.down(sc, nsc) ); HS_CALL( dY.down(dy, m) );
   return dYt.down(dyt, m + 1);
}

extern "C" int hipsdp_tail_dots_unit(int device, int m, int n, int fused, const double* a, const double* v, double* out)
{
   if ( m < 1 || n < 1 || (fused != 0 && fused != 1) || a == NULL || v == NULL || out == NULL )
      return HIPSDP_ERR_ARG;
   HS_CALL( pick_device(device) );
   const long long n2 = (long long) n * n;
   DevBuf dA, dV, dO, dW;
   HS_CALL( dA.alloc(3 * n2) ); HS_CALL( dV.alloc(2 * m) ); HS_CALL( dO.alloc(3) ); HS_CALL( dW.alloc(HS_RED_WS_DOUBLES) );
   HS_CALL( nan_fill(dO, 3) ); HS_CALL( nan_fill(dW, HS_RED_WS_DOUBLES) );
   HS_CALL( dA.up(a, 3 * n2) ); HS_CALL( dV.up(v, 2 * m) );
   const double* a0 = dA.p; const double* a1 = dA.p + n2; const double* a2 = dA.p + 2 * n2;
   hs_red_batch_reset();
   hs_red_batch_begin(0);
   int rc = hs_fill_scalar(0, dO.p, 0.0);
   if ( fused )
   {
      if ( rc == HS_OK ) rc = hs_dot_deferred(0, n2, a0, a1, dO.p, 1, dW.p, 0);
      if ( rc == HS_OK ) rc = hs_dot_deferred(0, n2, a2, a2, dO.p + 1, 0, dW.p, 1);
      if ( rc == HS_OK ) rc = hs_dot_deferred(0, n2, a0, a2, dO.p, 1, dW.p, 2);
   }
   else
   {
      if ( rc == HS_OK ) rc = hs_dot(0, n2, a0, a1, dO.p, 1, dW.p);
      if ( rc == HS_OK ) rc = hs_dot(0, n2, a2, a2, dO.p + 1, 0, dW.p);
      if ( rc == HS_OK ) rc = hs_dot(0, n2, a0, a2, dO.p, 1, dW.p);
   }
   if ( rc == HS_OK ) rc = hs_dot(0, m, dV.p, dV.p + m, dO.p + 2, 0, dW.p);
   if ( rc == HS_OK ) rc = hs_red_batch_end();
   if ( rc == HS_OK && hipDeviceSynchronize() != hipSuccess ) rc = HS_ERR_HIP;
   hs_red_batch_reset();
   HS_CALL( rc );
   return dO.down(out, 3);
}

extern "C" int hipsdp_trtri(int device, int n, const double* A, double* Linv)
{
   HS_CALL( pick_device(device) );
   const long long n2 = (long long) n * n;
   DevBuf dA, dD, dL, dT;
   int* dflag = NULL;
   HS_CALL( dA.alloc(n2) ); HS_CALL( dD.alloc(hs_potrf_dinv_len(n)) ); HS_CALL( dL.alloc(n2) ); HS_CALL( dT.alloc(n2) );
   HS_HIP( hipMalloc((void**) &dflag, sizeof(int)) );
   HS_HIP( hipMemset(dflag, 0, sizeof(int)) );
   HS_CALL( dA.up(A, n2) );
   int rc = hs_potrf(0, n, dA.p, dD.p, dflag, NULL);
   if ( rc == HS_OK ) rc = hs_trtri(0, n, dA.p, dD.p, dL.p, dT.p);
   if ( rc == HS_OK && hipDeviceSynchronize() != hipSuccess ) rc = HS_ERR_HIP;
   int hflag = 0;
   if ( rc == HS_OK && hipMemcpy(&hflag, dflag, sizeof(int), hipMemcpyDeviceToHost) != hipSuccess ) rc = HS_ERR_HIP;
   (void) hipFree(dflag);
   HS_CALL( rc );
   HS_CALL( dL.down(Linv, n2) );
   return hflag == 0 ? HIPSDP_OK : HIPSDP_ERR_NUMERIC;
}

extern "C" int hipsdp_lambda_min(int device, int n, const double* W, int steps, double* theta, double* resid)
{
   HS_CALL( pick_device(device) );
   if ( n <= 0 ) return HIPSDP_ERR_ARG;
   if ( steps <= 0 ) steps = n < 250 ? n : 250;
   if ( steps > 250 ) steps = 250;
   const long long n2 = (long long) n * n;
   DevBuf dW, dR, dS;
   HS_CALL( dW.alloc(n2) ); HS_CALL( dR.alloc(8) ); HS_CALL( dS.alloc(hs_lanczos_ws(n, steps)) );
   HS_CALL( dW.up(W, n2) );
   HS_CALL( hs_lanczos_lmin(0, n, dW.p, steps, dR.p, dS.p) );
   HS_HIP( hipDeviceSynchronize() );
   double h[3];
   HS_CALL( dR.down(h, 3) );
   *theta = h[0];
   if ( resid != NULL ) *resid = h[1];
   return HIPSDP_OK;
}

extern "C" int hipsdp_lambda_min_scaled(int device, int n, const double* L, const double* D, int steps, double* theta, double* resid)
{
   HS_CALL( pick_device(device) );
   if ( n <= 0 || n > 64 || theta == NULL ) return HIPSDP_ERR_ARG;
   const long long n2 = (long long) n * n;
   DevBuf dL, dD, dR;
   HS_CALL( dL.alloc(n2) ); HS_CALL( dD.alloc(n2) ); HS_CALL( dR.alloc(16) );
// ... 1068 lines not shown
```

Baseline: 13.53.

## Compute predictor step-length and sigma decisions on device to avoid host round-trip

Adds a device-side decision record, computed in the batched reduction kernel, that holds the predictor step length, sigma, eta, sigma*mu and the tau-kappa product. Kernels now accept values given either as immediates or as device pointers (hs_dval), so the corrector direction can read these values without a host readback and sync. The intent is to remove a device-to-host synchronization per IPM iteration. In exchange it adds an extra elementwise kernel, forces batch flushes in some paths, and supports only a restricted set of configurations; a host-decisions force switch keeps the old path available.

```diff
diff --git a/include/hipsdp_units.h b/include/hipsdp_units.h
--- a/include/hipsdp_units.h
+++ b/include/hipsdp_units.h
@@ -21,6 +21,10 @@
 HIPSDP_API int  hipsdp_tri_product_unit(int device, int mode, int M, int N, int K, int layB, int batch, int flags, const double* A,
    const double* B, double* Cio, int crows, int ldc, int* used);
 HIPSDP_API int  hipsdp_tri_instance_force(int mode);
+HIPSDP_API int  hipsdp_host_decisions_force(int on);
+HIPSDP_API int  hipsdp_decide_sc_len(int nblk);
+HIPSDP_API int  hipsdp_decide_pred_layout(int* layout);
+HIPSDP_API int  hipsdp_decide_pred_unit(int device, int nblk, const double* par, const double* sc, double* dec);
 HIPSDP_API int  hipsdp_schur_identity_unit(int device, int m1, int n, const double* A, double ws_gbytes, int full_storage, double* Mx,
    double* flops);
 HIPSDP_API int  hipsdp_schur_dense(int device, int m1, int n, const double* A, const double* X, const double* Zinv, double* Mx,
diff --git a/scip-sdp_amd/binding.py b/scip-sdp_amd/binding.py
--- a/scip-sdp_amd/binding.py
+++ b/scip-sdp_amd/binding.py
@@ -972,6 +972,25 @@
     return ulib().hipsdp_tri_instance_force(mode)
 
 
+def host_decisions_force(on):
+    return ulib().hipsdp_host_decisions_force(on)
+
+
+def decide_pred_layout():
+    lay = (C.c_int * 6)()
+    _chk(ulib().hipsdp_decide_pred_layout(lay), "hipsdp_decide_pred_layout")
+    return tuple(lay)
+
+
+def decide_pred_unit(nblk, tau, kappa, sigma_floor, mu, sc, device=0):
+    sc = _f64(sc)
+    assert sc.shape == (ulib().hipsdp_decide_sc_len(nblk),)
+    par = _f64([tau, kappa, sigma_floor, mu])
+    dec = np.zeros(6)
+    _chk(ulib().hipsdp_decide_pred_unit(device, nblk, _dp(par), _dp(sc), _dp(dec)), "hipsdp_decide_pred_unit")
+    return dec
+
+
 def gram_selfcheck(M, K, reps=0, device=0):
     used = C.c_int(0)
     nr = C.c_longlong(0)
diff --git a/scip-sdp_amd/csrc/hs_kernels.h b/scip-sdp_amd/csrc/hs_kernels.h
--- a/scip-sdp_amd/csrc/hs_kernels.h
+++ b/scip-sdp_amd/csrc/hs_kernels.h
@@ -4,12 +4,24 @@
 #include "hs_common.h"
 #include "hs_cut_plan.h"
 #include <vector>
+
+struct hs_dval
+{
+   double v; const double* p;
+   hs_dval(double x) : v(x), p(NULL) {}
+   explicit hs_dval(const double* slot) : v(0.0), p(slot) {}
+};
+#ifdef __HIPCC__
+__device__ __forceinline__ double hs_dget(const hs_dval& a) { return a.p != NULL ? *a.p : a.v; }
+#endif
 
 int hs_fill(hipStream_t s, double* p, long long n, double v);
 int hs_set_identity(hipStream_t s, double* A, int n, double v);
 int hs_copy(hipStream_t s, double* dst, const double* src, long long n);
 int hs_axpy(hipStream_t s, long long n, double a, const double* x, double* y);
 int hs_scale_add(hipStream_t s, long long n, double a, const double* x, double b, const double* y, double* out);
+int hs_scale_add_d(hipStream_t s, long long n, double a, const double* x, hs_dval b, const double* y, double* out);
+int hs_scaled_plus(hipStream_t s, long long n, hs_dval c, const double* t, const double* e, double* out);
 struct hs_trial_job { double* V; const double* dV; double* Vs; double* L; };
 int hs_trial_pair(hipStream_t s, long long n, double alpha, int first, const hs_trial_job* jobs);
 int hs_mirror_lower(hipStream_t s, double* A, int n, long long lda);
@@ -34,7 +46,10 @@
 int hs_fill_scalar(hipStream_t s, double* p, double v);
 int hs_red_batch_solve(hipStream_t s, int m, const double* dinv, const double* L, int nrhs, double* vec, long long ld);
 struct hs_rb_finish { int m; double eta, rg, sigmu, tau, kappa, etk; const double* u1; const double* u2; double* dy; double* dyt; double* sc;
-   int s0, bub, bh, wrp, bu1, dtau, dkappa, den; };
+   int s0, bub, bh, wrp, bu1, dtau, dkappa, den; const double* dec; };
+enum { HS_DEC_AA = 0, HS_DEC_SIGMA, HS_DEC_ETA, HS_DEC_SIGMU, HS_DEC_ETK, HS_DEC_BAD, HS_DEC_LEN };
+struct hs_decide_pred { int nblk, blk0, ratx, ratz, dtau, dkappa; double tau, kappa, sigma_floor, mu; const double* sc; double* dec; };
+int hs_red_batch_decide_pred(hipStream_t s, const hs_decide_pred* a);
 int hs_red_batch_finish(hipStream_t s, const void* fin, size_t bytes);
 int hs_copy_scalar(hipStream_t s, double* dst, const double* src);
 void hs_red_batch_hold(hipStream_t s);
@@ -62,10 +77,10 @@
 #define HS_SMALL_N 48
 int hs_dir_block_small(hipStream_t s, int n, double c, const double* X, const double* R, const double* E, const double* Zinv,
    double s1, double* out);
-int hs_dirmat(hipStream_t s, int n, double s1, const double* Zinv, const double* X, const double* GZ, double* H);
-int hs_dirmat_pack(hipStream_t s, int n, double s1, const double* Zinv, const double* X, const double* GZ, double* H, double* pk);
-
-int hs_lp_dir(hipStream_t s, int q, double sigmu, double eta, const double* x, const double* z, const double* rd_or_dz,
+int hs_dirmat(hipStream_t s, int n, hs_dval s1, const double* Zinv, const double* X, const double* GZ, double* H);
+int hs_dirmat_pack(hipStream_t s, int n, hs_dval s1, const double* Zinv, const double* X, const double* GZ, double* H, double* pk);
+
+int hs_lp_dir(hipStream_t s, int q, hs_dval sigmu, hs_dval eta, const double* x, const double* z, const double* rd_or_dz,
    const double* elp, double* out);
 int hs_lp_scale_rows(hipStream_t s, int q, int cols, const double* x, const double* z, const double* D, double* S);
 int hs_vec_mul(hipStream_t s, long long n, const double* a, const double* b, double* out);
@@ -75,9 +90,9 @@
 int hs_packed_diag(hipStream_t s, int m1, int n, int ldd, long long Lp, const double* Apk, double* D);
 int hs_sub_lower(hipStream_t s, int n, const double* S, double* C);
 int hs_pack_weighted(hipStream_t s, int n, const double* V, double* pk);
-int hs_unpack_sym(hipStream_t s, int n, const double* pk, double sa, const double* add, double* out);
+int hs_unpack_sym(hipStream_t s, int n, const double* pk, hs_dval sa, const double* add, double* out);
 int hs_unpack_sym3(hipStream_t s, int n, int cnt, const double* const* pk, double* const* out);
-int hs_unpack_dz_combine(hipStream_t s, int n, const double* pk, const double* P2, const double* sc, int idtau, double eta, const double* Rd,
+int hs_unpack_dz_combine(hipStream_t s, int n, const double* pk, const double* P2, const double* sc, int idtau, hs_dval eta, const double* Rd,
    double* dZ);
 int hs_zero_upper(hipStream_t s, double* A, int n);
 
@@ -179,8 +194,11 @@
 
 struct hs_dir_tail_args { int m, q, K; const int* n; const double* const* B; const double* const* H; const double* beta; const double* hl;
    const double* rhs2; const double* rp; const double* b; double* u1; const double* u2; double* dy; double* dyt; double* sc; double* red_ws;
-   const double* dinvm; const double* Lm; double eta, rg, sigmu, tau, kappa, etk; };
+   const double* dinvm; const double* Lm; double eta, rg, sigmu, tau, kappa, etk;
+   const double* dec; };
 int hs_ipm_dir_tail(hipStream_t st, const hs_dir_tail_args* a, int tail, int fuse_solve);
+int hs_ipm_decide_layout(hs_decide_pred* a);
+int hs_ipm_host_decisions_force(int on);
 int hs_ipm_after_solve2(hipStream_t st, int m, const double* rhs2, double* u2, double* wt, const double* u1, double* e2, double* e1, int fused);
 int hs_ipm_dz_combine(hipStream_t st, long long n2, double* dZ, const double* P2, const double* sc, double eta, const double* Rd);
 int hs_ipm_sc_dtau(void);
diff --git a/scip-sdp_amd/csrc/ipm.hip b/scip-sdp_amd/csrc/ipm.hip
--- a/scip-sdp_amd/csrc/ipm.hip
+++ b/scip-sdp_amd/csrc/ipm.hip
@@ -35,8 +35,10 @@
    SC_RATX,
    SC_RATZ,
    SC_DEN,
+   SC_DEC,
    SC_FIXED_END = 24
 };
+static_assert(SC_DEC + HS_DEC_LEN <= SC_FIXED_END, "the decision record's slots lie in front of the blocks' slots");
 #define SC_BLK(k, i) (SC_FIXED_END + 8 * (k) + (i))
 
 struct Block
@@ -1572,7 +1574,7 @@
 int hs_gen_dense(hipStream_t s, int n, int i0, int i1, long long seed, double* A);
 static int ensure_packed(hipsdp_solver* s);
 static int pass_A(hipsdp_solver* s, Block& B, const double* V, double* out, bool packed = false);
-static int pass_AT(hipsdp_solver* s, Block& B, const double* coef, double sa, const double* add, double* out);
+static int pass_AT(hipsdp_solver* s, Block& B, const double* coef, hs_dval sa, const double* add, double* out);
 
 extern "C" int hipsdp_gen_planted(hipsdp_solver* s, int n, int m, long long seed, const double* Xstar, const double* Zstar,
    const double* ystar, double* b_out)
@@ -1874,17 +1876,21 @@
    return HS_OK;
 }
 
-__global__ void k_h(int m, double eta, const double* __restrict__ AH, const double* __restrict__ rp, double* __restrict__ h)
-{
+__global__ void k_h(int m, hs_dval eta_, const double* __restrict__ AH, const double* __restrict__ rp, double* __restrict__ h)
+{
+   const double eta = hs_dget(eta_);
    const int i = blockIdx.x * blockDim.x + threadIdx.x;
    if ( i < m )
       h[i] = AH[1 + i] - eta * rp[i];
 }
 
-__global__ void k_finish_dir(int m, double eta, double rg, double sigmu, double tau, double kappa, double etk,
+__global__ void k_finish_dir(int m, double eta_, double rg, double sigmu_, double tau, double kappa, double etk_,
    const double* __restrict__ u1, const double* __restrict__ u2, double* __restrict__ dy, double* __restrict__ dyt,
-   double* __restrict__ sc)
-{
+   double* __restrict__ sc, const double* __restrict__ dec)
+{
+   const double eta = dec != NULL ? dec[HS_DEC_ETA] : eta_;
+   const double sigmu = dec != NULL ? dec[HS_DEC_SIGMU] : sigmu_;
+   const double etk = dec != NULL ? dec[HS_DEC_ETK] : etk_;
    const double den = sc[SC_S0] + kappa / tau + sc[SC_BUB];
    const double num = -eta * rg + (sigmu - tau * kappa - etk) / tau - sc[SC_BH] - eta * sc[SC_WRP] + sc[SC_BU1];
    const double dtau = num / den;
@@ -1943,7 +1949,7 @@
    if ( fuse_solve || tail )
    {
       hs_rb_finish F = {m, a->eta, a->rg, a->sigmu, a->tau, a->kappa, a->etk, a->u1, a->u2, a->dy, a->dyt, a->sc,
-         SC_S0, SC_BUB, SC_BH, SC_WRP, SC_BU1, SC_DTAU, SC_DKAPPA, SC_DEN};
+         SC_S0, SC_BUB, SC_BH, SC_WRP, SC_BU1, SC_DTAU, SC_DKAPPA, SC_DEN, a->dec};
       finished = hs_red_batch_finish(st, &F, sizeof(F)) == 1;
    }
    HS_CALL( hs_red_batch_end() );
@@ -1951,7 +1957,7 @@
    {
       HS_CALL( hs_red_batch_flush() );
       hipLaunchKernelGGL(k_finish_dir, g1d(m > 0 ? m : 1), dim3(256), 0, st, m, a->eta, a->rg, a->sigmu, a->tau, a->kappa, a->etk,
-         a->u1, a->u2, a->dy, a->dyt, a->sc);
+         a->u1, a->u2, a->dy, a->dyt, a->sc, a->dec);
       HS_LAUNCH_CHECK();
    }
    return HS_OK;
@@ -1984,6 +1990,11 @@
 }
 
 int hs_ipm_sc_dtau(void) { return SC_DTAU; }
+int hs_ipm_decide_layout(hs_decide_pred* a)
+{
+   a->blk0 = SC_FIXED_END; a->ratx = SC_RATX; a->ratz = SC_RATZ; a->dtau = SC_DTAU; a->dkappa = SC_DKAPPA;
+   return SC_DEC;
+}
 int hs_ipm_sc_len(int nblocks) { return SC_FIXED_END + 8 * (nblocks > 0 ? nblocks : 1) + 8; }
 
 static int gemm_on(hipStream_t st, int layA, int layB, int M, int N, int K, double alpha, const double* A, long long lda,
@@ -2359,10 +2370,18 @@
    return hs_gemv_n(s->stream, m1, (long long) B.n * B.n, B.A, (long long) B.n * B.n, 1, &V, out, m1, s->gemv_ws, s->gemv_ws_len);
 }
 
-static int pass_AT(hipsdp_solver* s, Block& B, const double* coef, double sa, const double* add, double* out)
+static int pass_AT(hipsdp_solver* s, Block& B, const double* coef, hs_dval sa_, const double* add, double* out)
 {
    const int m1 = s->m + 1;
    const long long n2 = (long long) B.n * B.n;
+   if ( sa_.p != NULL )
+   {
+      if ( B.sparse || passes_sharded(s, B) || B.Apk == NULL )
+         return HS_ERR_ARG;
+      HS_CALL( hs_gemv_t_ws(s->stream, m1, B.Lp, B.Apk, B.Lp, coef, 0.0, NULL, B.pkv + B.Lp, s->gemvt_ws, s->gemvt_ws_len) );
+      return hs_unpack_sym(s->stream, B.n, B.pkv + B.Lp, sa_, add, out);
+   }
+   const double sa = sa_.v;
    if ( B.sparse )
    {
       hipLaunchKernelGGL(k_sp_base, g1d(n2), dim3(256), 0, s->stream, n2, coef, B.A0, sa, add, out);
@@ -2504,10 +2523,14 @@
 static const int SOLVE_MODE = 3 | 4;
 
 static int direction(hipsdp_solver* s, double sigma, double eta, double mu, double rg, bool useE, double etk, int part = 0,
-   bool u1_solved = false, int split = 0)
+   bool u1_solved = false, int split = 0, const double* dec = NULL)
 {
    const int m = s->m, m1 = s->m + 1, q = s->q;
    const double sigmu = sigma * mu;
+   const hs_dval v_eta = dec != NULL ? hs_dval(dec + HS_DEC_ETA) : hs_dval(eta);
+   const hs_dval v_sigmu = dec != NULL ? hs_dval(dec + HS_DEC_SIGMU) : hs_dval(sigmu);
+   if ( dec != NULL && (!useE || part != 0 || split == 2 || !general_tail(s)) )
+      return HS_ERR_ARG;
    std::vector<double*> Hs;
    int fusedA = 0;
    BatchRegion region(s, part == 0 && batch_regions(s));
@@ -2521,19 +2544,29 @@
          HS_CALL( hs_dir_block_small(s->stream, n, eta, B.X, B.Rd, useE ? B.E : NULL, B.Zinv, sigmu, B.H) );
       else
       {
-         if ( useE )
-            HS_CALL( hs_copy(s->stream, B.G, B.E, n2) );
-         HS_CALL( gemm(s, HS_KC, HS_MC, n, n, n, eta, B.X, n, B.Rd, n, useE ? 1.0 : 0.0, B.G, n) );
+         if ( dec != NULL )
+         {
+            if ( !pack_with_dirmat(s, B) )
+               return HS_ERR_ARG;
+            HS_CALL( gemm(s, HS_KC, HS_MC, n, n, n, 1.0, B.X, n, B.Rd, n, 0.0, B.GZ, n) );
+            HS_CALL( hs_scaled_plus(s->stream, n2, v_eta, B.GZ, B.E, B.G) );
+         }
+         else
+         {
+            if ( useE )
+               HS_CALL( hs_copy(s->stream, B.G, B.E, n2) );
+            HS_CALL( gemm(s, HS_KC, HS_MC, n, n, n, eta, B.X, n, B.Rd, n, useE ? 1.0 : 0.0, B.G, n) );
+         }
          HS_CALL( gemm(s, HS_KC, HS_MC, n, n, n, 1.0, B.G, n, B.Zinv, n, 0.0, B.GZ, n) );
          if ( pack_with_dirmat(s, B) )
-            HS_CALL( hs_dirmat_pack(s->stream, n, sigmu, B.Zinv, B.X, B.GZ, B.H, B.pkv) );
+            HS_CALL( hs_dirmat_pack(s->stream, n, v_sigmu, B.Zinv, B.X, B.GZ, B.H, B.pkv) );
          else
-            HS_CALL( hs_dirmat(s->stream, n, sigmu, B.Zinv, B.X, B.GZ, B.H) );
+            HS_CALL( hs_dirmat(s->stream, n, v_sigmu, B.Zinv, B.X, B.GZ, B.H) );
       }
       Hs.push_back(B.H);
    }
    if ( q > 0 )
-      HS_CALL( hs_lp_dir(s->stream, q, sigmu, eta, s->x, s->z, s->rd, useE ? s->elp : NULL, s->hl) );
+      HS_CALL( hs_lp_dir(s->stream, q, v_sigmu, v_eta, s->x, s->z, s->rd, useE ? s->elp : NULL, s->hl) );
    fusedA = part == 1 ? 0 : apply_A_small(s, Hs.data(), s->hl, s->AH, 1, eta, s->rp, s->u1);
    if ( fusedA < 0 )
       return -fusedA;
@@ -2542,7 +2575,7 @@
    if ( fusedA == 0 && m > 0 )
    {
       HS_CALL( hs_red_batch_flush() );
-      hipLaunchKernelGGL(k_h, g1d(m), dim3(256), 0, s->stream, m, eta, s->AH, s->rp, s->u1);
+      hipLaunchKernelGGL(k_h, g1d(m), dim3(256), 0, s->stream, m, v_eta, s->AH, s->rp, s->u1);
       HS_LAUNCH_CHECK();
    }
    if ( part == 1 )
@@ -2562,7 +2595,7 @@
          bn.push_back(B.n); bB.push_back(B.B); bH.push_back(B.H);
       }
       const hs_dir_tail_args ta = {m, q, (int) s->blk.size(), bn.data(), bB.data(), bH.data(), s->beta, s->hl, s->rhs2, s->rp, s->b, s->u1, s->u2,
-         s->dy, s->dyt, s->sc, s->red_ws, s->dinvm, s->Lm, eta, rg, sigmu, s->tau, s->kappa, etk};
+         s->dy, s->dyt, s->sc, s->red_ws, s->dinvm, s->Lm, eta, rg, sigmu, s->tau, s->kappa, etk, dec};
       HS_CALL( hs_ipm_dir_tail(s->stream, &ta, general_tail(s) ? 1 : 0, fuse_solve ? 1 : 0) );
    }
    for (auto& B : s->blk)
@@ -2570,7 +2603,7 @@
       const int n = B.n;
       const long long n2 = (long long) n * n;
       if ( split == 0 )
-         HS_CALL( pass_AT(s, B, s->dyt, eta, B.Rd, B.dZ) );
+         HS_CALL( pass_AT(s, B, s->dyt, v_eta, B.Rd, B.dZ) );
       else
       {
          bool combined = false;
@@ -2584,12 +2617,14 @@
             if ( pack_with_dirmat(s, B) )
             {
                HS_CALL( hs_gemv_t_ws(s->stream, m1, B.Lp, B.Apk, B.Lp, s->cvec + m1, 0.0, NULL, B.pkv + B.Lp, s->gemvt_ws, s->gemvt_ws_len) );
-               HS_CALL( hs_unpack_dz_combine(s->stream, n, B.pkv + B.Lp, B.P2, s->sc, SC_DTAU, eta, B.Rd, B.dZ) );
+               HS_CALL( hs_unpack_dz_combine(s->stream, n, B.pkv + B.Lp, B.P2, s->sc, SC_DTAU, v_eta, B.Rd, B.dZ) );
                combined = true;
             }
             else
                HS_CALL( pass_AT(s, B, s->cvec + m1, 0.0, NULL, B.dZ) );
          }
+         if ( !combined && dec != NULL )
+            return HS_ERR_ARG;
          if ( !combined )
             HS_CALL( hs_ipm_dz_combine(s->stream, n2, B.dZ, B.P2, s->sc, eta, B.Rd) );
       }
@@ -2601,7 +2636,7 @@
             HS_CALL( hs_copy(s->stream, B.G, B.E, n2) );
          HS_CALL( gemm(s, HS_KC, HS_MC, n, n, n, 1.0, B.X, n, B.dZ, n, useE ? 1.0 : 0.0, B.G, n) );
          HS_CALL( gemm(s, HS_KC, HS_MC, n, n, n, 1.0, B.G, n, B.Zinv, n, 0.0, B.GZ, n) );
-         HS_CALL( hs_dirmat(s->stream, n, sigmu, B.Zinv, B.X, B.GZ, B.dX) );
+         HS_CALL( hs_dirmat(s->stream, n, v_sigmu, B.Zinv, B.X, B.GZ, B.dX) );
       }
    }
    if ( q > 0 )
@@ -2615,8 +2650,11 @@
       {
          const double* v = s->dyt;
          HS_CALL( hs_gemv_n(s->stream, q, m1, s->Dext, m1, 1, &v, s->tmpq, q, s->gemv_ws, s->gemv_ws_len) );
-         HS_CALL( hs_scale_add(s->stream, q, 1.0, s->tmpq, eta, s->rd, s->dz) );
-         HS_CALL( hs_lp_dir(s->stream, q, sigmu, 1.0, s->x, s->z, s->dz, useE ? s->elp : NULL, s->dx) );
+         if ( dec != NULL )
+            HS_CALL( hs_scale_add_d(s->stream, q, 1.0, s->tmpq, v_eta, s->rd, s->dz) );
+         else
+            HS_CALL( hs_scale_add(s->stream, q, 1.0, s->tmpq, eta, s->rd, s->dz) );
+         HS_CALL( hs_lp_dir(s->stream, q, v_sigmu, 1.0, s->x, s->z, s->dz, useE ? s->elp : NULL, s->dx) );
       }
    }
    return region.close();
@@ -3221,6 +3259,15 @@
    return HS_OK;
 }
 
+static int g_host_decisions = 0;
+static int g_device_decided = 0;
+int hs_ipm_host_decisions_force(int on)
+{
+   if ( on >= 0 )
+      g_host_decisions = on;
+   return g_device_decided;
+}
+
 struct GeneralSolve
 {
    hipsdp_solver* const s;
@@ -3267,6 +3314,8 @@
    bool predH_queued = false, predH_joined = false, split_dz = false;
    double dta = 0, dka = 0, sigma = 0, eta = 0, amax = 0, alpha = 0, dt = 0, dk = 0;
    double tau0 = 0, kappa0 = 0, applied = 0;
+   bool dev_pred = false;
+   bool time_pending = false;
 
    int halt(int why) { status = why; stop = true; return HS_OK; }
 
@@ -4057,10 +4106,60 @@
          HS_CALL( join2(s) );
       HS_CALL( direction(s, 0.0, 1.0, mu, rg, false, 0.0, predH_queued ? 2 : 0, predH_joined, split_dz ? 2 : 0) );
       HS_CALL( steplen_enqueue(s) );
+      dev_pred = device_decisions();
+      if ( dev_pred )
+      {
+         const hs_decide_pred dp = {K, SC_FIXED_END, SC_RATX, SC_RATZ, SC_DTAU, SC_DKAPPA, s->tau, s->kappa, sigma_floor, mu, s->sc,
+            s->sc + SC_DEC};
+         if ( hs_red_batch_decide_pred(s->stream, &dp) != 1 )
+            return HS_ERR_ARG;
+         ++g_device_decided;
+         return hs_red_batch_end();
+      }
       HS_CALL( read_scalars(s, hs, hflags) );
+      HS_CALL( assembly_book() );
+      if ( stop )
+         return HS_OK;
+      const double aa = fmin(1.0, steplen_host(s, hs));
+      dta = hs.v[SC_DTAU];
+      dka = hs.v[SC_DKAPPA];
+      if ( !std::isfinite(aa) || !std::isfinite(dta) )
+      {
+         if ( par.verbose )
+            printf("hipsdp: predictor not finite (alpha %g dtau %g)\n", aa, dta);
+         return halt(HIPSDP_STATUS_NUMERIC);
+      }
+      sigma = (1.0 - aa) * (1.0 - aa) * (1.0 - aa);
+      sigma = fmin(1.0, fmax(sigma_floor, sigma));
+      eta = 1.0 - sigma;
+      if ( par.verbose )
+         printf("hipsdp: predictor step %.17g sigma %.17g (host)\n", aa, sigma);
+      return HS_OK;
+   }
+
+   bool device_decisions() const
+   {
+      if ( g_host_decisions != 0 || !general_tail(s) || q > 0 )
+         return false;
+      for (auto& B : s->blk)
+         if ( !pack_with_dirmat(s, B) )
+            return false;
+      return true;
+   }
+
+   void assembly_time()
+   {
       float ms = 0.f;
-      if ( hipEventElapsedTime(&ms, s->ev0, s->ev1) == hipSuccess )
+      if ( time_pending && hipEventElapsedTime(&ms, s->ev0, s->ev1) == hipSuccess )
          schur_ms += ms;
+      time_pending = false;
+   }
+
+   int assembly_book()
+   {
+      time_pending = true;
+      if ( !dev_pred )
+         assembly_time();
       info->schur_calls++;
       for (auto& B : s->blk)
          if ( !gram_cached )
@@ -4069,20 +4168,9 @@
       {
          if ( par.verbose )
             printf("hipsdp: Cholesky failure flags Z=%d X=%d M=%d\n", hflags[0], hflags[1], hflags[2]);
+         assembly_time();
          return halt(HIPSDP_STATUS_NUMERIC);
       }
-      const double aa = fmin(1.0, steplen_host(s, hs));
-      dta = hs.v[SC_DTAU];
-      dka = hs.v[SC_DKAPPA];
-      if ( !std::isfinite(aa) || !std::isfinite(dta) )
-      {
-         if ( par.verbose )
-            printf("hipsdp: predictor not finite (alpha %g dtau %g)\n", aa, dta);
-         return halt(HIPSDP_STATUS_NUMERIC);
-      }
-      sigma = (1.0 - aa) * (1.0 - aa) * (1.0 - aa);
-      sigma = fmin(1.0, fmax(sigma_floor, sigma));
-      eta = 1.0 - sigma;
       return HS_OK;
    }
 
@@ -4095,11 +4183,29 @@
          BatchRegion region(s, batch_regions(s));
          if ( q > 0 )
             HS_CALL( hs_vec_mul(st, q, s->dx, s->dz, s->elp) );
-         HS_CALL( direction(s, sigma, eta, mu, rg, true, dta * dka, 0, false, split_dz ? 1 : 0) );
+         HS_CALL( direction(s, sigma, eta, mu, rg, true, dta * dka, 0, false, split_dz ? 1 : 0, dev_pred ? s->sc + SC_DEC : NULL) );
          HS_CALL( region.close() );
       }
       HS_CALL( steplen_enqueue(s) );
-      HS_CALL( read_scalars(s, hs, NULL) );
+      HS_CALL( read_scalars(s, hs, dev_pred ? hflags : NULL) );
+      if ( dev_pred )
+      {
+         const double* d = hs.v.data() + SC_DEC;
+         HS_CALL( assembly_book() );
+         if ( stop )
+            return HS_OK;
+         if ( d[HS_DEC_BAD] != 0.0 )
+         {
+            if ( par.verbose )
+               printf("hipsdp: predictor not finite (alpha %g)\n", d[HS_DEC_AA]);
+            assembly_time();
+            return halt(HIPSDP_STATUS_NUMERIC);
+         }
+         sigma = d[HS_DEC_SIGMA];
+         eta = d[HS_DEC_ETA];
+         if ( par.verbose )
+            printf("hipsdp: predictor step %.17g sigma %.17g (device)\n", d[HS_DEC_AA], sigma);
+      }
       amax = steplen_host(s, hs);
       alpha = fmin(1.0, gamma_eff * amax);
       dt = hs.v[SC_DTAU];
@@ -4108,6 +4214,7 @@
       {
          if ( par.verbose )
             printf("hipsdp: corrector not finite (alpha %g dtau %g dkappa %g)\n", alpha, dt, dk);
+         assembly_time();
          return halt(HIPSDP_STATUS_NUMERIC);
       }
       return HS_OK;
@@ -4115,6 +4222,7 @@
 
    int update()
    {
+      struct TakeTime { GeneralSolve* g; ~TakeTime() { g->assembly_time(); } } take_time = {this};
       phase_mark(s, PH_UPDATE);
       tau0 = s->tau;
       kappa0 = s->kappa;
@@ -4212,6 +4320,7 @@
                rd_scale = 1.0 - alpha * eta;
             }
             HS_CALL( enqueue_residuals() );
+            assembly_time();
             HS_CALL( read_back(hflags) );
             if ( hflags[0] == 0 && hflags[1] == 0 )
                break;
diff --git a/scip-sdp_amd/csrc/kernels.hip b/scip-sdp_amd/csrc/kernels.hip
--- a/scip-sdp_amd/csrc/kernels.hip
+++ b/scip-sdp_amd/csrc/kernels.hip
@@ -57,6 +57,29 @@
    }
 }
 
+__global__ void k_scale_add_d(long long n, double a, const double* __restrict__ x, hs_dval b_, const double* __restrict__ y,
+   double* __restrict__ out)
+{
+   const double b = hs_dget(b_);
+   for (long long i = (long long) blockIdx.x * blockDim.x + threadIdx.x; i < n; i += (long long) gridDim.x * blockDim.x)
+   {
+      double v = a * x[i];
+      v += b * y[i];
+      out[i] = v;
+   }
+}
+
+__global__ void k_scaled_plus(long long n, hs_dval c_, const double* __restrict__ t, const double* __restrict__ e, double* __restrict__ out)
+{
+#pragma clang fp contract(off)
+   const double c = hs_dget(c_);
+   for (long long i = (long long) blockIdx.x * blockDim.x + threadIdx.x; i < n; i += (long long) gridDim.x * blockDim.x)
+   {
+      const double v = c * t[i];
+      out[i] = v + e[i];
+   }
+}
+
 __global__ void k_mirror_lower(double* A, int n, long long lda)
 {
    const long long total = (long long) n * n;
@@ -128,8 +151,9 @@
    }
 }
 
-__global__ void k_unpack_sym(int n, const double* __restrict__ pk, double sa, const double* __restrict__ add, double* __restrict__ out)
-{
+__global__ void k_unpack_sym(int n, const double* __restrict__ pk, hs_dval sa_, const double* __restrict__ add, double* __restrict__ out)
+{
+   const double sa = hs_dget(sa_);
    const long long total = (long long) n * n;
    for (long long e = (long long) blockIdx.x * blockDim.x + threadIdx.x; e < total; e += (long long) gridDim.x * blockDim.x)
    {
@@ -157,8 +181,9 @@
 }
 
 __global__ void k_unpack_dz_combine(int n, const double* __restrict__ pk, const double* __restrict__ P2, const double* __restrict__ sc, int idtau,
-   double eta, const double* __restrict__ Rd, double* __restrict__ dZ)
-{
+   hs_dval eta_, const double* __restrict__ Rd, double* __restrict__ dZ)
+{
+   const double eta = hs_dget(eta_);
    const double dtau = sc[idtau];
    const long long total = (long long) n * n;
    for (long long e = (long long) blockIdx.x * blockDim.x + threadIdx.x; e < total; e += (long long) gridDim.x * blockDim.x)
@@ -170,9 +195,10 @@
    }
 }
 
-__global__ void k_dirmat_pack(int n, double s1, const double* __restrict__ Zinv, const double* __restrict__ X,
+__global__ void k_dirmat_pack(int n, hs_dval s1_, const double* __restrict__ Zinv, const double* __restrict__ X,
    const double* __restrict__ GZ, double* __restrict__ H, double* __restrict__ pk)
 {
+   const double s1 = hs_dget(s1_);
    const long long total = (long long) n * n;
    for (long long i = (long long) blockIdx.x * blockDim.x + threadIdx.x; i < total; i += (long long) gridDim.x * blockDim.x)
    {
@@ -214,9 +240,10 @@
    }
 }
 
-__global__ void k_dirmat(int n, double s1, const double* __restrict__ Zinv, const double* __restrict__ X,
+__global__ void k_dirmat(int n, hs_dval s1_, const double* __restrict__ Zinv, const double* __restrict__ X,
    const double* __restrict__ GZ, double* __restrict__ H)
 {
+   const double s1 = hs_dget(s1_);
    const long long total = (long long) n * n;
    for (long long i = (long long) blockIdx.x * blockDim.x + threadIdx.x; i < total; i += (long long) gridDim.x * blockDim.x)
    {
@@ -227,9 +254,10 @@
    }
 }
 
-__global__ void k_lp_dir(int q, double sigmu, double eta, const double* __restrict__ x, const double* __restrict__ z,
+__global__ void k_lp_dir(int q, hs_dval sigmu_, hs_dval eta_, const double* __restrict__ x, const double* __restrict__ z,
    const double* __restrict__ r, const double* __restrict__ elp, double* __restrict__ out)
 {
+   const double sigmu = hs_dget(sigmu_), eta = hs_dget(eta_);
    const int i = blockIdx.x * blockDim.x + threadIdx.x;
    if ( i < q )
    {
@@ -405,6 +433,25 @@
    }
 }
 
+int hs_scale_add_d(hipStream_t s, long long n, double a, const double* x, hs_dval b, const double* y, double* out)
+{
+   (void) hs_red_batch_flush();
+   if ( n <= 0 ) return HS_OK;
+   if ( y == NULL ) return HS_ERR_ARG;
+   hipLaunchKernelGGL(k_scale_add_d, dim3(grid_for(n, 256, 2048)), dim3(256), 0, s, n, a, x, b, y, out);
+   HS_LAUNCH_CHECK();
+   return HS_OK;
+}
+
+int hs_scaled_plus(hipStream_t s, long long n, hs_dval c, const double* t, const double* e, double* out)
+{
+   (void) hs_red_batch_flush();
+   if ( n <= 0 ) return HS_OK;
+   hipLaunchKernelGGL(k_scaled_plus, dim3(grid_for(n, 256, 2048)), dim3(256), 0, s, n, c, t, e, out);
+   HS_LAUNCH_CHECK();
+   return HS_OK;
+}
+
 int hs_trial_pair(hipStream_t s, long long n, double alpha, int first, const hs_trial_job* jobs)
 {
    (void) hs_red_batch_flush();
@@ -473,7 +520,7 @@
    return HS_OK;
 }
 
-int hs_unpack_sym(hipStream_t s, int n, const double* pk, double sa, const double* add, double* out)
+int hs_unpack_sym(hipStream_t s, int n, const double* pk, hs_dval sa, const double* add, double* out)
 {
    (void) hs_red_batch_flush();
    hipLaunchKernelGGL(k_unpack_sym, dim3(grid_for((long long) n * n, 256, 2048)), dim3(256), 0, s, n, pk, sa, add, out);
@@ -496,7 +543,7 @@
    return HS_OK;
 }
 
-int hs_unpack_dz_combine(hipStream_t s, int n, const double* pk, const double* P2, const double* sc, int idtau, double eta, const double* Rd,
+int hs_unpack_dz_combine(hipStream_t s, int n, const double* pk, const double* P2, const double* sc, int idtau, hs_dval eta, const double* Rd,
    double* dZ)
 {
    (void) hs_red_batch_flush();
@@ -672,7 +719,7 @@
    return HS_OK;
 }
 
-int hs_dirmat(hipStream_t s, int n, double s1, const double* Zinv, const double* X, const double* GZ, double* H)
+int hs_dirmat(hipStream_t s, int n, hs_dval s1, const double* Zinv, const double* X, const double* GZ, double* H)
 {
    (void) hs_red_batch_flush();
    if ( n <= 0 ) return HS_OK;
@@ -681,7 +728,7 @@
    return HS_OK;
 }
 
-int hs_dirmat_pack(hipStream_t s, int n, double s1, const double* Zinv, const double* X, const double* GZ, double* H, double* pk)
+int hs_dirmat_pack(hipStream_t s, int n, hs_dval s1, const double* Zinv, const double* X, const double* GZ, double* H, double* pk)
 {
    (void) hs_red_batch_flush();
    hipLaunchKernelGGL(k_dirmat_pack, dim3(grid_for((long long) n * n, 256, 2048)), dim3(256), 0, s, n, s1, Zinv, X, GZ, H, pk);
@@ -689,11 +736,13 @@
    return HS_OK;
 }
 
-int hs_lp_dir(hipStream_t s, int q, double sigmu, double eta, const double* x, const double* z, const double* r,
+int hs_lp_dir(hipStream_t s, int q, hs_dval sigmu, hs_dval eta, const double* x, const double* z, const double* r,
    const double* elp, double* out)
 {
    if ( q <= 0 ) return HS_OK;
-   if ( hs_rec_lp_dir(s, q, sigmu, eta, x, z, r, elp, out) )
+   if ( sigmu.p != NULL || eta.p != NULL )
+      (void) hs_red_batch_flush();
+   else if ( hs_rec_lp_dir(s, q, sigmu.v, eta.v, x, z, r, elp, out) )
       return HS_OK;
    hipLaunchKernelGGL(k_lp_dir, dim3((q + 255) / 256), dim3(256), 0, s, q, sigmu, eta, x, z, r, elp, out);
    HS_LAUNCH_CHECK();
@@ -831,11 +880,13 @@
 #define RB_MAKEEXT 114
 #define RB_GEMVT   115
 #define RB_LPROWS  116
+#define RB_DECPRED 118
 #define RB_APPLYA  117
 
 struct rb_desc { int kind; int accumulate; int i[6]; double d[4]; const void* p[10]; };
 struct rb_finish { int m; double eta, rg, sigmu, tau, kappa, etk; const double* u1; const double* u2; double* dy; double* dyt; double* sc;
-   int s0, bub, bh, wrp, bu1, dtau, dkappa, den; };
+   int s0, bub, bh, wrp, bu1, dtau, dkappa, den; const double* dec; };
+static_assert(sizeof(rb_finish) == sizeof(hs_rb_finish), "the caller's parameter block is copied into the record");
 struct rb_args { int cnt; rb_desc d[RB_MAX]; rb_finish fin; int pub_n; const double* pub_src; double* pub_dst;
    unsigned long long pub_seq; unsigned long long* pub_flag;
    unsigned long long* dbg; };
@@ -935,6 +986,48 @@
       r = OP::f(r, v[1]); r = OP::f(r, v[2]); r = OP::f(r, v[3]);
       *out = D.accumulate ? OP::f(*out, r) : r;
    }
+}
+
+__device__ __forceinline__ void d_decide_pred(const rb_desc& D)
+{
+#pragma clang fp contract(off)
+   const double* sc = (const double*) D.p[0];
+   double* dec = (double*) D.p[1];
+   const int nblk = D.i[0], blk0 = D.i[1];
+   const double tau = D.d[0], kappa = D.d[1], sigma_floor = D.d[2], mu = D.d[3];
+   double a = 1e300;
+   for (int k = 0; k < nblk; ++k)
+      for (int which = 0; which < 2; ++which)
+      {
+         const double theta = sc[blk0 + 8 * k + (which ? 4 : 1)];
+         const double resid = sc[blk0 + 8 * k + (which ? 5 : 2)];
+         const double lo = theta - resid;
+         if ( lo < 0.0 )
+            a = fmin(a, -1.0 / lo);
+      }
+   a = fmin(a, fmin(sc[D.i[2]], sc[D.i[3]]));
+   const double dtau = sc[D.i[4]], dkap = sc[D.i[5]];
+   if ( dtau < 0.0 ) a = fmin(a, -tau / dtau);
+   if ( dkap < 0.0 ) a = fmin(a, -kappa / dkap);
+   const double aa = fmin(1.0, a);
+   dec[HS_DEC_AA] = aa;
+   if ( !isfinite(aa) || !isfinite(dtau) )
+   {
+      dec[HS_DEC_SIGMA] = 1.0;
+      dec[HS_DEC_ETA] = 0.0;
+      dec[HS_DEC_SIGMU] = mu;
+      dec[HS_DEC_ETK] = 0.0;
+      dec[HS_DEC_BAD] = 1.0;
+      return;
+   }
+   const double om = 1.0 - aa;
+   double sigma = (om * om) * om;
+   sigma = fmin(1.0, fmax(sigma_floor, sigma));
+   dec[HS_DEC_SIGMA] = sigma;
+   dec[HS_DEC_ETA] = 1.0 - sigma;
+   dec[HS_DEC_SIGMU] = sigma * mu;
+   dec[HS_DEC_ETK] = dtau * dkap;
+   dec[HS_DEC_BAD] = 0.0;
 }
 
 __global__ void __launch_bounds__(256) k_red_batch(rb_args A)
@@ -1243,6 +1336,10 @@
          }
          break;
       }
+      case RB_DECPRED:
+         if ( threadIdx.x == 0 )
+            d_decide_pred(D);
+         break;
       case RB_SOLVE:
       {
          __shared__ double sL[64 * 65];
@@ -1381,14 +1478,19 @@
       default:
       {
          const rb_finish& F = A.fin;
-         const double den = F.sc[F.s0] + F.kappa / F.tau + F.sc[F.bub];
-         const double num = -F.eta * F.rg + (F.sigmu - F.tau * F.kappa - F.etk) / F.tau - F.sc[F.bh] - F.eta * F.sc[F.wrp] + F.sc[F.bu1];
+         double f_eta = F.dec != NULL ? F.dec[HS_DEC_ETA] : F.eta;
+         double f_sigmu = F.dec != NULL ? F.dec[HS_DEC_SIGMU] : F.sigmu;
+         double f_etk = F.dec != NULL ? F.dec[HS_DEC_ETK] : F.etk;
+         double f_rg = F.rg, f_tau = F.tau, f_kappa = F.kappa;
+         asm volatile("" : "+v"(f_eta), "+v"(f_sigmu), "+v"(f_etk), "+v"(f_rg), "+v"(f_tau), "+v"(f_kappa));
+         const double den = F.sc[F.s0] + f_kappa / f_tau + F.sc[F.bub];
+         const double num = -f_eta * f_rg + (f_sigmu - f_tau * f_kappa - f_etk) / f_tau - F.sc[F.bh] - f_eta * F.sc[F.wrp] + F.sc[F.bu1];
          const double dtau = num / den;
          __syncthreads();
          if ( threadIdx.x == 0 )
          {
             F.sc[F.dtau] = dtau;
-            F.sc[F.dkappa] = (F.sigmu - F.tau * F.kappa - F.etk - F.kappa * dtau) / F.tau;
+            F.sc[F.dkappa] = (f_sigmu - f_tau * f_kappa - f_etk - f_kappa * dtau) / f_tau;
             F.sc[F.den] = den;
             F.dyt[0] = -dtau;
          }
@@ -1625,6 +1727,21 @@
    rb_desc& D = g_rb.args.d[g_rb.args.cnt++];
    memset(&D, 0, sizeof(D));
    D.kind = RB_FINISH;
+   return 1;
+}
+
+int hs_red_batch_decide_pred(hipStream_t s, const hs_decide_pred* a)
+{
+   if ( !g_rb.open || s != g_rb.s )
+      return 0;
+   if ( g_rb.args.cnt == RB_MAX )
+      (void) rb_flush();
+   rb_desc& D = g_rb.args.d[g_rb.args.cnt++];
+   memset(&D, 0, sizeof(D));
+   D.kind = RB_DECPRED;
+   D.i[0] = a->nblk; D.i[1] = a->blk0; D.i[2] = a->ratx; D.i[3] = a->ratz; D.i[4] = a->dtau; D.i[5] = a->dkappa;
+   D.d[0] = a->tau; D.d[1] = a->kappa; D.d[2] = a->sigma_floor; D.d[3] = a->mu;
+   D.p[0] = a->sc; D.p[1] = a->dec;
    return 1;
 }
 
diff --git a/scip-sdp_amd/csrc/units.hip b/scip-sdp_amd/csrc/units.hip
--- a/scip-sdp_amd/csrc/units.hip
+++ b/scip-sdp_amd/csrc/units.hip
@@ -1046,6 +1046,48 @@
    HS_CALL( rc );
    HS_CALL( dS.down(sc, nsc) ); HS_CALL( dY.down(dy, m) );
    return dYt.down(dyt, m + 1);
+}
+
+extern "C" int hipsdp_host_decisions_force(int on)
+{
+   return hs_ipm_host_decisions_force(on);
+}
+
+extern "C" int hipsdp_decide_sc_len(int nblk) { return hs_ipm_sc_len(nblk); }
+extern "C" int hipsdp_decide_pred_layout(int* layout)
+{
+   if ( layout == NULL )
+      return HIPSDP_ERR_ARG;
+   hs_decide_pred a;
+   memset(&a, 0, sizeof(a));
+   layout[5] = hs_ipm_decide_layout(&a);
+   layout[0] = a.blk0; layout[1] = a.ratx; layout[2] = a.ratz; layout[3] = a.dtau; layout[4] = a.dkappa;
+   return HIPSDP_OK;
+}
+extern "C" int hipsdp_decide_pred_unit(int device, int nblk, const double* par, const double* sc, double* dec)
+{
+   if ( nblk < 1 || nblk > 64 || par == NULL || sc == NULL || dec == NULL )
+      return HIPSDP_ERR_ARG;
+   HS_CALL( pick_device(device) );
+   const int nsc = hs_ipm_sc_len(nblk);
+   DevBuf dS;
+   HS_CALL( dS.alloc(nsc) );
+   HS_CALL( dS.up(sc, nsc) );
+   hs_decide_pred a;
+   memset(&a, 0, sizeof(a));
+   const int off = hs_ipm_decide_layout(&a);
+   a.nblk = nblk; a.tau = par[0]; a.kappa = par[1]; a.sigma_floor = par[2]; a.mu = par[3]; a.sc = dS.p; a.dec = dS.p + off;
+   hs_red_batch_reset();
+   hs_red_batch_begin(0);
+   int rc = hs_red_batch_decide_pred(0, &a) == 1 ? HS_OK : HS_ERR_ARG;
+   if ( rc == HS_OK ) rc = hs_red_batch_end();
+   if ( rc == HS_OK && hipDeviceSynchronize() != hipSuccess ) rc = HS_ERR_HIP;
+   hs_red_batch_reset();
+   HS_CALL( rc );
+   std::vector<double> h((size_t) nsc);
+   HS_CALL( dS.down(h.data(), nsc) );
+   memcpy(dec, h.data() + off, HS_DEC_LEN * sizeof(double));
+   return HIPSDP_OK;
 }
 
 extern "C" int hipsdp_tail_dots_unit(int device, int m, int n, int fused, const double* a, const double* v, double* out)
```

New measurement: 13.35. -1.4%, worse.
